# liuQuan98/APR

Measured on AMD Instinct MI355X. Metric: point-cloud pairs/sec (120k-pt KITTI frame, FCGF encode+match+SVD), higher is better.
Workload: dtype f32

## Files before the change

apr_amd/_lib.py:

```python
from __future__ import annotations

import ctypes as C
import os

import torch

_HERE = os.path.dirname(os.path.abspath(__file__))
LIB_PATH = os.path.join(_HERE, "lib", "libapr_hip.so")

_p = C.c_void_p
_i32, _i64, _u64, _f32, _f64, _sz = C.c_int32, C.c_int64, C.c_uint64, C.c_float, C.c_double, C.c_size_t

class PairDesc(C.Structure):
    _fields_ = [("f0", C.c_void_p), ("n0", C.c_int64), ("f1", C.c_void_p), ("n1", C.c_int64),
                ("xyz0", C.c_void_p), ("xyz1", C.c_void_p), ("seed", C.c_uint64)]


class SpconvDesc(C.Structure):
    _fields_ = [("inp", C.c_void_p), ("ldi", C.c_int64), ("nbr", C.c_void_p), ("n_out", C.c_int64),
                ("K", C.c_int32), ("cin", C.c_int32), ("cout", C.c_int32), ("relu", C.c_int32),
                ("w_packed", C.c_void_p), ("scale", C.c_void_p), ("shift", C.c_void_p),
                ("residual", C.c_void_p), ("ldr", C.c_int64), ("out", C.c_void_p), ("ldo", C.c_int64),
                ("counters", C.c_void_p), ("plist", C.c_void_p), ("prod_scratch", C.c_void_p),
                ("plist_bytes", C.c_int64), ("w_bf3", C.c_void_p),
                ("os_pairs", C.c_void_p), ("os_rows", C.c_int64), ("os_build_bytes", C.c_int64),
                ("os_n_in", C.c_int64), ("l2norm", C.c_int32), ("ws3", C.c_int32)]


class ResunetLayer(C.Structure):
    _fields_ = [("K", C.c_int32), ("cin", C.c_int32), ("cout", C.c_int32), ("relu", C.c_int32),
                ("w_packed", C.c_void_p), ("w_bf3", C.c_void_p), ("scale", C.c_void_p), ("shift", C.c_void_p)]


class ResunetPlan(C.Structure):
    _fields_ = [("layer", ResunetLayer * 23), ("conv1_w", C.c_void_p), ("conv1_ks", C.c_int32), ("normalize", C.c_int32),
                ("ws_conv", C.c_uint32), ("ws_block", C.c_uint32), ("os_block", C.c_uint32),
                ("ws3", C.c_int32), ("ws3_cin128", C.c_int32), ("os_min_rows", C.c_int32), ("occ_kernel_map", C.c_int32),
                ("ws3_max_rows_128", C.c_int64)]


class LevelMap(C.Structure):
    _fields_ = [("coords", C.c_void_p), ("keys", C.c_void_p), ("vals", C.c_void_p), ("cap", C.c_int64), ("n", C.c_int64)]


class Pyramid(C.Structure):
    _fields_ = [("lv", LevelMap * 4), ("first", C.c_void_p), ("pts", C.c_void_p), ("header", C.c_void_p),
                ("header_ints", C.c_int32), ("compact", C.c_int32), ("compact_rows", C.c_int64),
                ("counters", C.c_void_p), ("n_counter_slots", C.c_int32)]


class GcnLayer(C.Structure):
    _fields_ = [("kind", C.c_int32), ("k", C.c_int32), ("heads", C.c_int32),
                ("eps1", C.c_float), ("eps2", C.c_float), ("eps3", C.c_float),
                ("w1", C.c_void_p), ("w2", C.c_void_p), ("w3", C.c_void_p), ("b1", C.c_void_p), ("b2", C.c_void_p),
                ("wq", C.c_void_p), ("wk", C.c_void_p), ("wv", C.c_void_p), ("wm", C.c_void_p),
                ("bq", C.c_void_p), ("bk", C.c_void_p), ("bv", C.c_void_p), ("bm", C.c_void_p)]


class GcnDesc(C.Structure):
    _fields_ = [("n_layers", C.c_int32), ("c", C.c_int32), ("layer", GcnLayer * 8)]


PROTOTYPES = {
    "apr_col_sums": (C.c_int, [_p, _i64, _i64, _i32, _p, _p, _sz, _p]),
    "apr_mha_train_forward": (C.c_int, [_p, _p, _p, _i32, _i32, _i32, _i32, _i32, _p, _p, _p]),
    "apr_mha_train_backward": (C.c_int, [_p, _p, _p, _p, _p, _i32, _i32, _i32, _i32, _i32, _p, _p, _p, _p, _p]),
    "apr_edge_features_backward": (C.c_int, [_p, _i32, _i32, _i32, _p, _i64, _p, _p]),
    "apr_gcn_scratch_bytes": (_sz, [_p, _i32, _i32]),
    "apr_gcn_forward": (C.c_int, [_p, _p, _i32, _p, _i32, _p, _i64, _p, _i64, _p, _i64, _p, _i64, _p, _sz, _p]),
    "apr_voxel_pyramid_scratch_bytes": (_sz, [_i64, _i32]),
    "apr_voxel_pyramid": (C.c_int, [_p, _p, _i32, _f32, _p, _sz, _p, _p]),
    "apr_resunet_encode_supported": (C.c_int, [_p, _p, _p]),
    "apr_resunet_encode_scratch_bytes": (_sz, [_p, _p, _p]),
    "apr_resunet_encode": (C.c_int, [_p, _p, _p, _p, _i32, _p, _sz, _p, _i64, _p]),
    "apr_last_error": (C.c_char_p, []),
    "apr_version": (C.c_int, []),
    "apr_device_count": (C.c_int, []),
    "apr_struct_sizes": (_i32, [_p, _i32]),
    "apr_ransac_set_screen": (C.c_int, [_i32]),
    "apr_ransac_set_option": (C.c_int, [_i32, _i32]),
    "apr_ransac_sampling_launches": (C.c_int, [_p]),
    "apr_event_wait": (C.c_int, [_p, _i32]),
    "apr_event_wait_timeout": (C.c_int, [_p, _i32, _i64]),
    "apr_hash_capacity": (_i64, [_i64]),
    "apr_map_scratch_bytes": (_sz, [_i64]),
    "apr_voxelize": (C.c_int, [_p, _i64, _f32, _i32, _p, _p]),
    "apr_map_build": (C.c_int, [_p, _i64, _p, _i32, _p, _p, _i64, _p, _p, _p, _p, _p, _sz, _p]),
    "apr_kernel_map_transpose": (C.c_int, [_p, _i64, _i32, _i64, _p, _p]),
    "apr_voxelize_segments": (C.c_int, [_p, _i64, C.c_float, _p, _i32, _p, _p]),
    "apr_segment_counts": (C.c_int, [_p, _p, _p, _i32, _p, _p]),
    "apr_kernel_map_same": (C.c_int, [_p, _i64, _p, _p, _i64, _i32, _i32, _p, _p]),
    "apr_kernel_map": (C.c_int, [_p, _i64, _p, _p, _p, _i64, _i32, _i32, _p, _p]),
    "apr_spconv_packed_size": (_i64, [_i32, _i32, _i32]),
    "apr_spconv_pack_weights": (C.c_int, [_p, _i32, _i32, _i32, _p, _p]),
    "apr_spconv_fwd": (C.c_int, [_p, _i64, _p, _i64, _i32, _i32, _i32, _p, _p, _p, _p, _i64, _i32, _p, _i64, _p]),
    "apr_pairlist_counter_ints": (_i32, []),
    "apr_pairlist_bytes": (_sz, [_i64, _i32]),
    "apr_pairlist_build": (C.c_int, [_p, _i64, _i32, _p, _p, _sz, _p]),
    "apr_pairlist3_bytes": (_sz, [_i64]),
    "apr_pairlist3_build": (C.c_int, [_p, _i64, _i32, _p, _p, _sz, _p]),
    "apr_spconv_ws3_supported": (C.c_int, [_i32, _i32, _i32]),
    "apr_spconv_ws3_fwd_bf3": (C.c_int, [_p, _i64, _p, _p, _i64, _i32, _i32, _p, _p, _p, _p, _i64, _i32, _p, _i64, _p, _p]),
    "apr_spconv_ws_fwd": (C.c_int, [_p, _i64, _p, _p, _i64, _i32, _i32, _i32, _p, _p, _p, _p, _i64, _i32, _p, _i64, _p, _p]),
    "apr_spconv_packed_bf3_bytes": (_i64, [_i32, _i32, _i32]),
    "apr_spconv_pack_weights_bf3": (C.c_int, [_p, _i32, _i32, _i32, _p, _p]),
    "apr_spconv_pack_weights_bf3_ex": (C.c_int, [_p, _i32, _i32, _i32, _i32, _i32, _p, _p]),
    "apr_spconv_ws_fwd_bf3": (C.c_int, [_p, _i64, _p, _p, _i64, _i32, _i32, _i32, _p, _p, _p, _p, _p, _i64, _i32, _p, _i64,
                                        _p, _p]),
    "apr_spconv_wgrad_scratch_bytes": (_sz, [_i64, _i32, _i32, _i32]),
    "apr_spconv_wgrad": (C.c_int, [_p, _i64, _p, _i64, _p, _i64, _i32, _i32, _i32, _p, _p, _sz, _p]),
    "apr_spconv_wgrad_same_level": (C.c_int, [_p, _i64, _p, _i64, _p, _i64, _i32, _i32, _i32, _p, _p, _sz, _p]),
    "apr_spconv_fwd_batch": (C.c_int, [_p, _i32, _p]),
    "apr_spconv_fwd_batch_timed": (C.c_int, [_p, _i32, _p, _p]),
    "apr_bn_stats": (C.c_int, [_p, _i64, _i64, _i32, _p, _p, _p, _sz, _p]),
    "apr_norm_params": (C.c_int, [_p, _i64, _i64, _i32, _f32, _p, _p, _p, _sz, _p]),
    "apr_bn_stats_scratch_bytes": (_sz, [_i64, _i32]),
    "apr_instance_norm_act": (C.c_int, [_p, _i64, _i64, _i32, _f32, _p, _i64, _i32, _f32, _p, _i64, _p, _sz, _p]),
    "apr_spconv_os_tile_rows": (_i32, [_i64, _i32, _i32]),
    "apr_spconv_os_pairs_bytes": (_sz, [_i64, _i32, _i32]),
    "apr_spconv_os_pairs_build": (C.c_int, [_p, _i64, _i64, _i32, _i32, _p, _sz, _p]),
    "apr_spconv_os_trace": (C.c_int, [_p, _i32]),
    "apr_spconv_os_set_debug": (C.c_int, [_i32]),
    "apr_spconv_os_fwd": (C.c_int, [_p, _i64, _p, _i64, _i32, _i32, _i32, _i32, _p, _p, _p, _p, _i64, _i32, _p, _i64, _p]),
    "apr_norm_backward_scratch_bytes": (_sz, [_i64, _i32]),
    "apr_norm_backward": (C.c_int, [_p, _i64, _p, _i64, _i64, _i32, _p, _p, _p, _p, _i64, _p, _p, _p, _sz, _p]),
    "apr_bn_train_fwd": (C.c_int, [_p, _i64, _i64, _i32, _p, _p, C.c_float, C.c_float, _p, _p, _p, _i64, _i32, _p, _i64, _p, _p,
                                   _p, _p, _i32, _p, _sz, _p]),
    "apr_bn_train_bwd": (C.c_int, [_p, _i64, _p, _i64, _p, _i64, _i64, _i32, _p, _p, _p, _i32, _p, _i64, _p, _i64, _p, _p,
                                   _p, _i32, _p, _sz, _p]),
    "apr_weights_flip_transpose": (C.c_int, [_p, _i32, _i32, _i32, _i32, _p, _p]),
    "apr_dense_gemm_bf3": (C.c_int, [_p, _i64, _i64, _i32, _i32, _p, _p, _p, _p, _i64, _i32, _p, _i64, _p]),
    "apr_dense_rows_bf3_ok": (_i32, [_i32, _i32]),
    "apr_dense_rows_bf3_route": (_i32, [_i64, _i32, _i32]),
    "apr_dense_rows_bf3": (C.c_int, [_p, _i64, _i64, _i32, _i32, _p, _p, _p, _p, _i64, _i32, _i32, _p, _i64, _p]),
    "apr_dense_gemm_bf3_norm_scratch_bytes": (_sz, [_i64, _i32, _i32]),
    "apr_dense_gemm_bf3_norm_act": (C.c_int, [_p, _i64, _i64, _i32, _i32, _p, _f32, _p, _i64, _i32, _f32, _p, _i64, _p, _i32, _p,
                                              _sz, _p]),
    "apr_weighted_choice_round": (C.c_int64, [_p, _i64, _p, _i64, _i64, _p, _i64, _p, _p, _i32]),
    "apr_instance_norm_act_seg": (C.c_int, [_p, _i64, _i64, _i32, _f32, _p, _i64, _i32, _f32, _p, _i64, _p, _i32, _p, _sz, _p]),
    "apr_affine_act": (C.c_int, [_p, _i64, _i64, _i32, _p, _p, _p, _i64, _i32, _f32, _p, _i64, _p]),
    "apr_act_backward": (C.c_int, [_p, _i64, _p, _i64, _i64, _i32, _i32, _f32, _p, _i64, _p]),
    "apr_l2_normalize": (C.c_int, [_p, _i64, _i64, _i32, _p, _i64, _p]),
    "apr_l2_normalize_backward": (C.c_int, [_p, _i64, _p, _i64, _i64, _i32, _p, _i64, _p]),
    "apr_feature_nn": (C.c_int, [_p, _i64, _p, _i64, _i32, _p, _p]),
    "apr_feature_nn_fast_scratch_bytes": (_sz, [_i64, _i64, _i32]),
    "apr_feature_nn_fast": (C.c_int, [_p, _i64, _p, _i64, _i32, _p, _p, _sz, _p]),
    "apr_nn_unpack": (C.c_int, [_p, _i64, _p, _p, _p]),
    "apr_ransac_scratch_bytes": (_sz, [_i64, _i64]),
    "apr_ransac_pose": (C.c_int, [_p, _i64, _p, _i64, _p, _f64, _f64, _i64, _u64, _p, _sz, _p, _p]),
    "apr_ransac_geometric_scratch_bytes": (_sz, [_i64, _i64, _i64]),
    "apr_ransac_pose_geometric": (C.c_int, [_p, _i64, _p, _i64, _p, _f64, _f64, _i64, _i64, _u64, _p, _sz, _p, _p]),
    "apr_ransac_raw_bytes": (_sz, []),
    "apr_ransac_pose_geometric_async": (C.c_int, [_p, _i64, _p, _i64, _p, _f64, _f64, _i64, _i64, _u64, _p, _sz, _p, _p]),
    "apr_ransac_decode": (C.c_int, [_p, _p]),
    "apr_irls_pose": (C.c_int, [_p, _p, _p, _i64, _p, _p, _sz, _p]),
    "apr_match_pose_batch_scratch_bytes": (_sz, [_i32, _i64, _i64, _i32, _i64]),
    "apr_match_pose_batch": (C.c_int, [_p, _i32, _i32, C.c_double, C.c_double, _i64, _p, _sz, _p, _p]),
    "apr_match_pose_batch_slot_bytes": (_sz, [_i32]),
    "apr_match_pose_set_lanes": (C.c_int, [_i32]),
    "apr_match_pose_batch_enqueue": (C.c_int, [_p, _i32, _i32, C.c_double, C.c_double, _i64, _p, _sz, _p, _p]),
    "apr_match_pose_batch_finish": (C.c_int, [_p, _i32, _i32, C.c_double, C.c_double, _i64, _p, _sz, _p, _p, _p]),
    "apr_irls_scratch_bytes": (_sz, [_i64]),
    "apr_valid_pair": (C.c_int, [_p, _i64, _p, _i64, _p, _p, _i64, _i64, _p, _p, _f32, _p, _i64, _i64, _p, _sz, _p]),
    "apr_valid_pair_scratch_bytes": (_sz, [_i64]),
    "apr_contrastive_reduce": (C.c_int, [_p, _p, _i32, _i32, _p, _p, _p, _p, _p, _p, _p, _i32, _i64, _f32, _f32, _p, _p]),
    "apr_grid_subsample_scratch_bytes": (_sz, [_i64]),
    "apr_grid_subsample": (C.c_int, [_p, _i64, _p, _i32, _f32, _p, _i32, _p, _p, _p, _p, _sz, _p]),
    "apr_grid_subsample_async": (C.c_int, [_p, _i64, _p, _i32, _f32, _p, _i32, _p, _p, _p, _p, _sz, _p]),
    "apr_voxel_down_sample_scratch_bytes": (_sz, [_i64]),
    "apr_voxel_down_sample": (C.c_int, [_p, _i64, _p, _i32, _f64, _p, _p, _p, _p, _p, _p, _p, _sz, _p]),
    "apr_sample_augment": (C.c_int, [_p, _p, _i64, _f64, _p, _f64, _p, _p, _p]),
    "apr_cloud_mean": (C.c_int, [_p, _i64, _p, _p]),
    "apr_radius_scratch_bytes": (_sz, [_i64, _i64]),
    "apr_radius_neighbors_async": (C.c_int, [_p, _i64, _p, _i64, _p, _p, _i32, _f32, _i32, _p, _i64, _p, _p, _sz, _p]),
    "apr_radius_neighbors_regrid_async": (C.c_int, [_p, _i64, _p, _i64, _p, _p, _i32, _f32, _i32, _p, _i64, _p, _p, _sz, _p]),
    "apr_radius_neighbors": (C.c_int, [_p, _i64, _p, _i64, _p, _p, _i32, _f32, _i32, _p, _i64, _p, _p, _sz, _p]),
    "apr_knn": (C.c_int, [_p, _i32, _i32, _i32, _p, _p]),
    "apr_row_sums": (C.c_int, [_p, _i64, _i64, _i32, _p, _p]),
    "apr_kpconv_weighted": (C.c_int, [_p, _i64, _p, _i64, _p, _i32, _p, _i64, _i32, _p, _i32, _f32, _p, _p, _i64, _p]),
    "apr_kpconv_dfeat": (C.c_int, [_p, _i64, _p, _i64, _p, _i32, _p, _i64, _i32, _p, _i32, _f32, _p, _p, _i64, _p]),
    "apr_kpconv_dfeat_contrib": (C.c_int, [_p, _i64, _p, _i64, _p, _i32, _p, _i64, _i32, _p, _i32, _f32, _p, _p, _p]),
    "apr_reverse_table_scratch_bytes": (_sz, [_i64, _i32, _i64]),
    "apr_reverse_table_build": (C.c_int, [_p, _i64, _i32, _i64, _p, _p, _p, _sz, _p]),
    "apr_reverse_gather": (C.c_int, [_p, _i32, _p, _p, _i64, _p, _i64, _p]),
    "apr_reverse_gather_range": (C.c_int, [_p, _i32, _p, _p, _i64, _i64, _i64, _i32, _p, _i64, _p]),
    "apr_gather_pool": (C.c_int, [_p, _i64, _i64, _i32, _p, _i32, _i64, _i32, _p, _i64, _p]),
    "apr_gather_pool_argmax": (C.c_int, [_p, _i64, _i64, _i32, _p, _i32, _i64, _p, _i64, _p, _p]),
    "apr_gather_pool_backward": (C.c_int, [_p, _i64, _i32, _p, _p, _i64, _i32, _p, _i32, _p, _i64, _p]),
    "apr_edge_features": (C.c_int, [_p, _i64, _i32, _i32, _p, _i32, _p, _p]),
    "apr_group_max": (C.c_int, [_p, _i64, _i32, _i32, _i32, _p, _p, _f32, _p, _i64, _p]),
    "apr_coords_bbox": (C.c_int, [_p, _i64, _p, _p]),
    "apr_kp_resnet_scratch_bytes": (_sz, [_p]),
    "apr_kp_resnet_block": (C.c_int, [_p, _p]),
    "apr_voxelize_frames": (C.c_int, [_p, _p, _i32, _f32, _p, _p, _p]),
    "apr_gather_frame_points": (C.c_int, [_p, _p, _i32, _p, _p, _i64, _p, _p]),
    "apr_pack_i32": (C.c_int, [_p, _p, _i32, _p, _p, _i64, _p]),
    "apr_fill_bytes": (C.c_int, [_p, _i32, _sz, _p]),
    "apr_kernel_map_transpose_prefilled": (C.c_int, [_p, _i64, _i32, _i64, _p, _p]),
    "apr_occ_conv_scratch_bytes": (_sz, [_p, _i32]),
    "apr_occ_conv_pays": (C.c_int, [_p, _i32, _i64]),
    "apr_occ_conv": (C.c_int, [_p, _i64, _p, _i32, _p, _i32, _p, _p, _p, _i64, _i32, _p, _i64, _p, _sz, _p]),
    "apr_kernel_map_occ": (C.c_int, [_p, _i64, _p, _p, _p, _i64, _i32, _i32, _p, _i32, _p, _p, _p]),
    "apr_mha": (C.c_int, [_p, _p, _p, _i32, _i32, _i32, _i32, _p, _p]),
    "apr_mha_headmajor": (C.c_int, [_p, _p, _p, _i32, _i32, _i32, _i32, _p, _p]),
    "apr_softmax_matvec": (C.c_int, [_p, _p, _p, _i32, _i32, _i32, _f32, _p, _p]),
    "apr_softmax_matvec_bt": (C.c_int, [_p, _p, _p, _i32, _i32, _i32, _f32, _p, _p]),
    "apr_softmax_matvec_mfma": (C.c_int, [_p, _p, _p, _i32, _i32, _i32, _f32, _p, _p]),
    "apr_score_head": (C.c_int, [_p, _i64, _i64, _p, _p]),
    "apr_transform_points": (C.c_int, [_p, _i64, _p, _p, _p]),
    "apr_crop_scratch_bytes": (_sz, [_i64]),
    "apr_crop_to_radius": (C.c_int, [_p, _i64, _p, _i64, _p, _p, _p, _sz, _p]),
    "apr_chamfer_sum": (C.c_int, [_p, _i64, _p, _i64, _p, _p, _sz, _p]),
    "apr_nn3_scratch_bytes": (_sz, [_i64, _i64]),
    "apr_nn3": (C.c_int, [_p, _i64, _p, _i64, C.c_float, _p, _p, _p, _sz, _p]),
    "apr_nn3_batch": (C.c_int, [_p, _p, _p, _p, _i32, C.c_float, _p, _p, _p, _p, _sz, _p]),
    "apr_overlap_labels": (C.c_int, [_p, _i64, _i64, _i64, _p, _p, _p, _p, _p]),
    "apr_weighted_bce_scratch_bytes": (_sz, []),
    "apr_weighted_bce_forward": (C.c_int, [_p, _p, _i64, _p, _p, _p, _sz, _p]),
    "apr_weighted_bce_backward": (C.c_int, [_p, _p, _i64, _p, _p, _p, _p, _p, _p]),
    "apr_gathered_argmax": (C.c_int, [_p, _p, _p, _i64, _p, _p, _p, _i64, _i32, _p, _p, _p]),
    "apr_saliency_labels": (C.c_int, [_p, _p, _p, _p, _p, _p, _p, _p, _p, _p, _i64, _i64, _f32, _p, _p, _p, _p, _p]),
    "apr_circle_select": (C.c_int, [_p, _i64, _p, _i64, _p, _i64, _p, _p, _f32, _p, _p, _p]),
    "apr_circle_gather": (C.c_int, [_p, _p, _p, _p, _i32, _p, _p, _p, _p, _i32, _p, _p, _p, _p, _p, _p, _p, _p, _p]),
    "apr_circle_forward": (C.c_int, [_p, _p, _p, _i32, _p, _p, _p, _i32, _p, _p, _p, _p, _p, _p, _p, _p]),
    "apr_circle_backward": (C.c_int, [_p, _p, _p, _i32, _p, _p, _p, _i32, _p, _p, _p, _p, _p, _p, _p, _p, _p, _p, _p]),
    "apr_circle_scatter": (C.c_int, [_p, _p, _i32, _i32, _p, _i64, _p]),
    "apr_icp_scratch_bytes": (_sz, [_i64, _i64, _i32]),
    "apr_icp_batch": (C.c_int, [_p, _p, _p, _p, _i32, _p, _i32, _p, _f64, _i32, _f64, _f64, _p, _p, _p, _sz, _p]),
    "apr_mutual_select": (C.c_int, [_p, _p, _i64, _p, _p, _i64, _p, _p, _p]),
    "apr_inlier_ratio": (C.c_int, [_p, _i64, _p, _i64, _p, _p, _p, _p, _p, _i64, _f32, _p, _p, _p, _p]),
    "apr_dense_argmax": (C.c_int, [_p, _i64, _i64, _p, _p, _p]),
    "apr_ransac_pairs_geometric_scratch_bytes": (_sz, [_i64, _i64, _i64, _i64, _i64]),
    "apr_ransac_pose_pairs_geometric": (C.c_int, [_p, _i64, _p, _i64, _p, _i64, _f64, _i64, _i64, _u64, _p, _sz, _p, _p]),
    "apr_information_scratch_bytes": (_sz, [_i64, _i64, _i32]),
    "apr_information_batch": (C.c_int, [_p, _p, _p, _p, _i32, _p, _i32, _p, _i64, _f64, _p, _p, _p, _p, _sz, _p]),
    "apr_posegraph_optimize": (C.c_int, [_p, _p, _i32, _p, _p, _i64, _p, _p, _f64, _f64, _f64, _p, _p, _p, _p, _p, _p]),
}

class KpResnetDesc(C.Structure):
    _fields_ = [("x", _p), ("ldx", _i64), ("n_in", _i64),
                ("in_dim", _i32), ("mid", _i32), ("out_dim", _i32), ("strided", _i32),
                ("q_pts", _p), ("s_pts", _p), ("n_out", _i64),
                ("nbr", _p), ("H", _i32), ("n_kp", _i32),
                ("kernel_points", _p), ("extent", _f32), ("eps", _f32), ("slope", _f32), ("nseg", _i32),
                ("w_unary1", _p), ("w_kpconv", _p), ("w_unary2", _p), ("w_shortcut", _p),
                ("seg_in", _p), ("seg_out", _p),
                ("out", _p), ("ldo", _i64),
                ("scratch", _p), ("scratch_bytes", _sz)]


_lib = None


class AprHipError(RuntimeError):
    pass


def load():
    global _lib
    if _lib is not None:
        return _lib
    if not os.path.exists(LIB_PATH):
        raise AprHipError(
            f"{LIB_PATH} is missing: build it with `python -m apr_amd.build` "
            "(hipcc --offload-arch=gfx950). There is no CPU fallback.")
    lib = C.CDLL(LIB_PATH)
    for name, (res, args) in PROTOTYPES.items():
        fn = getattr(lib, name)
        fn.restype = res
        fn.argtypes = args
    _lib = lib
    return lib


def check(rc: int):
    if rc != 0:
        msg = load().apr_last_error().decode()
        raise AprHipError(f"libapr_hip error {rc}: {msg}")


def ptr(t):
    if t is None:
        return None
    return C.c_void_p(t.data_ptr())


def stream():
    return C.c_void_p(torch._C._cuda_getCurrentRawStream(torch.cuda.current_device()))


def require_gpu_tensor(t, dtype, name):
    if not t.is_cuda:
        raise AprHipError(f"{name}: expected a GPU tensor (the HIP path has no CPU fallback)")
    if t.dtype != dtype:
        raise AprHipError(f"{name}: expected dtype {dtype}, got {t.dtype}")
    if not t.is_contiguous():
        raise AprHipError(f"{name}: tensor must be contiguous")
    return t
```

apr_amd/csrc/common.h:

```cpp
#pragma once
#include <hip/hip_runtime.h>
#include <stdint.h>
#include <stdio.h>
#include <stdlib.h>
#include <string.h>

#include "../../include/apr_hip.h"

static inline int env_int(const char* name, int dflt) {
  const char* v = getenv(name);
  return v ? atoi(v) : dflt;
}

#define APR_API extern "C" __attribute__((visibility("default")))

void apr_set_error(const char* fmt, ...);

#define APR_CHECK_ARG(cond, ...)      \
  do {                                \
    if (!(cond)) {                    \
      apr_set_error(__VA_ARGS__);     \
      return APR_EINVAL;              \
    }                                 \
  } while (0)

#define APR_HIP(call)                                                            \
  do {                                                                           \
    hipError_t e_ = (call);                                                      \
    if (e_ != hipSuccess) {                                                      \
      apr_set_error("%s:%d %s -> %s", __FILE__, __LINE__, #call, hipGetErrorString(e_)); \
      return APR_EHIP;                                                           \
    }                                                                            \
  } while (0)

#define APR_LAUNCH_CHECK() APR_HIP(hipGetLastError())

static inline int64_t cdiv64(int64_t a, int64_t b) { return (a + b - 1) / b; }

__host__ __device__ static inline size_t apr_align256(size_t x) { return (x + 255) & ~(size_t)255; }

struct AprArena {
  char* base;
  size_t off = 0;
  explicit AprArena(void* scratch) : base((char*)apr_align256((size_t)scratch)) {}
  template <typename T>
  T* take(size_t count) {
    T* p = base ? (T*)(base + off) : nullptr;
    off += apr_align256(count * sizeof(T));
    return p;
  }
  size_t bytes() const { return off + 256; }
  bool fits(size_t scratch_bytes) const { return scratch_bytes >= bytes(); }
};

int apr_internal_nn_brute(const float* f0, int64_t n0, const float* f1, int64_t n1, int32_t c, uint64_t* best,
                          const unsigned* run_if, void* stream);

int apr_internal_fill(void* ptr, int32_t byte_value, size_t bytes, hipStream_t st);

bool apr_internal_dense_ok(int64_t M, int32_t cin, int32_t cout);
bool apr_internal_dense_rows_route(int64_t M, int32_t cin, int32_t cout);
int apr_internal_dense_gemm(const float* in, int64_t ldi, int64_t M, int32_t cin, int32_t cout, const float* wp,
                            const float* scale, const float* shift, const float* residual, int64_t ldr, int32_t relu,
                            float* out, int64_t ldo, hipStream_t st);

int apr_internal_norm_apply_partials(const float* x, int64_t ldx, int32_t c, const int64_t* seg_row0, const int* seg_blk0,
                                     int32_t nseg, const double* partial, float eps, const float* residual, int64_t ldr,
                                     int32_t act_mode, float negative_slope, float* y, int64_t ldy, hipStream_t st);

#ifdef __HIPCC__
__device__ inline int apr_wave_incl_scan(int x) {
  x += __builtin_amdgcn_update_dpp(0, x, 0x111, 0xf, 0xf, true);
  x += __builtin_amdgcn_update_dpp(0, x, 0x112, 0xf, 0xf, true);
  x += __builtin_amdgcn_update_dpp(0, x, 0x114, 0xf, 0xf, true);
  x += __builtin_amdgcn_update_dpp(0, x, 0x118, 0xf, 0xf, true);
  x += __builtin_amdgcn_update_dpp(0, x, 0x142, 0xa, 0xf, true);
  x += __builtin_amdgcn_update_dpp(0, x, 0x143, 0xc, 0xf, true);
  return x;
}
#endif

#define APR_KEY_EMPTY 0xFFFFFFFFFFFFFFFFull
#define APR_AXIS_BIAS (1 << 17)
#define APR_AXIS_RANGE (1 << 18)

__host__ __device__ static inline bool apr_key_in_range(int b, int x, int y, int z) {
  return (unsigned)b < 1023u && (unsigned)(x + APR_AXIS_BIAS) < (unsigned)APR_AXIS_RANGE &&
         (unsigned)(y + APR_AXIS_BIAS) < (unsigned)APR_AXIS_RANGE &&
         (unsigned)(z + APR_AXIS_BIAS) < (unsigned)APR_AXIS_RANGE;
}

__host__ __device__ static inline uint64_t apr_pack_key(int b, int x, int y, int z) {
  return ((((uint64_t)(unsigned)b << 18 | (uint64_t)(unsigned)(x + APR_AXIS_BIAS)) << 18 |
           (uint64_t)(unsigned)(y + APR_AXIS_BIAS))
          << 18) |
         (uint64_t)(unsigned)(z + APR_AXIS_BIAS);
}

__host__ __device__ static inline uint32_t apr_hash_u64(uint64_t k) {
  k ^= k >> 33;
  k *= 0xff51afd7ed558ccdull;
  k ^= k >> 33;
  k *= 0xc4ceb9fe1a85ec53ull;
  k ^= k >> 33;
  return (uint32_t)k;
}

__host__ __device__ static inline int apr_floor_to(int v, int m) {
  int q = v / m;
  if ((v % m) != 0 && v < 0) --q;
  return q * m;
}

struct AprSearchGrid {
  const unsigned long long* keys;
  const int* vals;
  uint32_t mask;
  const int* start;
  const int* sorted;
  const float* mins;
  float cell;
  const int4* cell_coords;
  const int* n_cells;
  const int* status;
};
#define APR_GRID_MARGIN_CELLS 40960
size_t apr_internal_grid_bytes(int64_t n);
int apr_internal_search_grid(const float* pts, int64_t n, float cell, void* scratch, AprSearchGrid* out,
                             hipStream_t st);
int apr_internal_search_grid_batch(const float* pts, int64_t n, const int32_t* lengths_host, int32_t nb, float cell, void* scratch,
                                   AprSearchGrid* out, hipStream_t st);
struct AprCellBuckets {
  int4* coords;
  const int* starts;
  const float* mins;
  const int4* cell_coords;
  const int* n_cells;
  const int* status;
  const int* start;
  int* sorted;
  int* big_count;
  int* big_list;
  int* spare;
};
int apr_internal_buckets_begin(const float* pts, int64_t n, const int32_t* lengths_host, int32_t nb, void* scratch,
                               AprCellBuckets* out, hipStream_t st);
int apr_internal_buckets_finish(int64_t n, void* scratch, int64_t* first, hipStream_t st);
int apr_internal_icp_pack(const float* tgt, int64_t m, AprSearchGrid g, float4* rows, hipStream_t st);

__device__ static inline int apr_table_lookup(const unsigned long long* __restrict__ keys,
                                              const int* __restrict__ vals, uint32_t mask,
                                              unsigned long long key) {
  uint32_t slot = apr_hash_u64(key) & mask;
  for (uint32_t probe = 0; probe <= mask; ++probe) {
    unsigned long long k = keys[slot];
    if (k == key) return vals[slot];
    if (k == APR_KEY_EMPTY) return -1;
    slot = (slot + 1) & mask;
  }
  return -1;
}
```

apr_amd/csrc/encoder.hip:

```cpp
#include "common.h"

namespace {

constexpr int kLevels = 4, kStages = 7, kMaps = 10, kMaxLists = 24;

inline bool ws_shape_ok(int K, int cin, int cout) { return K <= 27 && cin % 64 == 0 && cin <= 512 && cout % 64 == 0; }

struct ListSlot {
  int map, kind, rows;
  void* blob;
  size_t bytes;
  int32_t* counters;
  bool built;
};

struct Enc {
  const apr_resunet_plan& P;
  const apr_level_map* lv;
  const int32_t* bbox;
  AprArena arena;
  const bool dry;
  hipStream_t st;
  int rc = APR_OK;

  int32_t* kmap[kMaps] = {};
  ListSlot lists[kMaxLists];
  int nlists = 0, ncounter = 0;
  int32_t* counters = nullptr;
  int n_counter_slots = 0;
  void* occ = nullptr;
  size_t occ_bytes = 0;
  int32_t* tpool[3] = {};
  bool tpool_ready = false;
  float* prod = nullptr;
  size_t prod_bytes = 0;

  apr_spconv_desc descs[4];
  int ndesc = 0;

  Enc(const apr_resunet_plan& p, const apr_level_map* l, const int32_t* b, void* scratch, hipStream_t s)
      : P(p), lv(l), bbox(b), arena(scratch), dry(scratch == nullptr), st(s) {}

  float* rows(int64_t n, int c) { return arena.take<float>((size_t)n * c); }
  size_t need() const { return arena.bytes() + apr_align256(prod_bytes); }
  bool ok() const { return rc == APR_OK; }
  void run(int r) {
    if (rc == APR_OK && r != APR_OK) rc = r;
  }

  int64_t map_rows(int m) const { return m < 4 ? lv[m].n : m < 7 ? lv[m - 4 + 1].n : lv[m - 7].n; }
  int64_t map_in_rows(int m) const { return m < 4 ? lv[m].n : m < 7 ? lv[m - 4].n : lv[m - 7 + 1].n; }

  int32_t* kernel_map(int m) {
    if (kmap[m] || (dry && kmap_sized[m])) return kmap[m];
    kmap_sized[m] = true;
    const int64_t n_out = map_rows(m);
    if (m >= 7) {
      const int l = m - 7;
      int32_t* fwd = kernel_map(4 + l);
      if (!tpool_ready) {
        size_t ints = 0;
        for (int a = 0; a < 3; ++a) ints += (size_t)lv[a].n * 27;
        ints = (ints + 63) / 64 * 64 + 64;
        int32_t* buf = arena.take<int32_t>(ints);
        size_t pos = 0;
        for (int a = 0; a < 3; ++a) {
          tpool[a] = dry ? nullptr : buf + pos;
          pos += (size_t)lv[a].n * 27;
        }
        if (!dry) run(apr_fill_bytes(buf, 0xFF, ints * 4, st));
        tpool_ready = true;
      }
      kmap[m] = tpool[l];
      if (!dry) run(apr_kernel_map_transpose_prefilled(fwd, lv[l + 1].n, 27, lv[l].n, kmap[m], st));
      return kmap[m];
    }
    kmap[m] = arena.take<int32_t>((size_t)n_out * 27);
    if (dry) return kmap[m];
    const int lin = m < 4 ? m : m - 4, lout = m < 4 ? m : m - 4 + 1;
    const apr_level_map& in = lv[lin];
    const apr_level_map& outm = lv[lout];
    if (lin == 0 && P.occ_kernel_map && occ)
      run(apr_kernel_map_occ(outm.coords, outm.n, nullptr, in.keys, in.vals, in.cap, 3, 1, bbox, P.conv1_ks, occ, kmap[m], st));
    else
      run(apr_kernel_map(outm.coords, outm.n, nullptr, in.keys, in.vals, in.cap, 3, 1 << lin, kmap[m], st));
    return kmap[m];
  }
  bool kmap_sized[kMaps] = {};

  ListSlot* find_list(int m, int kind, int rws) {
    for (int i = 0; i < nlists; ++i)
      if (lists[i].map == m && lists[i].kind == kind && lists[i].rows == rws) return &lists[i];
    return nullptr;
  }

  ListSlot* ws_list(const apr_resunet_layer& L, int m, bool same_level) {
    bool tri = P.ws3 && L.w_bf3 && apr_spconv_ws3_supported(L.K, L.cin, L.cout);
    if (tri && L.cin == 128 && ((same_level && map_rows(m) > P.ws3_max_rows_128) || !P.ws3_cin128)) tri = false;
    const int kind = tri ? 1 : 0;
    ListSlot* s = find_list(m, kind, 0);
    if (s) return s;
    if (nlists >= kMaxLists) {
      apr_set_error("apr_resunet_encode: more than %d pair lists", kMaxLists);
      run(APR_EINVAL);
      return nullptr;
    }
    s = &lists[nlists++];
    s->map = m;
    s->kind = kind;
    s->rows = 0;
    s->bytes = tri ? apr_pairlist3_bytes(map_rows(m)) : apr_pairlist_bytes(map_rows(m), 27);
    s->blob = arena.take<char>(s->bytes);
    s->built = false;
    s->counters = nullptr;
    if (!dry) {
      if (ncounter >= n_counter_slots) {
        apr_set_error("apr_resunet_encode: more than %d pair lists need a counter block", n_counter_slots);
        run(APR_EINVAL);
        return nullptr;
      }
      s->counters = counters + (size_t)ncounter * apr_pairlist_counter_ints();
    }
    ++ncounter;
    return s;
  }

  ListSlot* os_list(const apr_resunet_layer& L, int m) {
    const int64_t n_out = map_rows(m), n_in = map_in_rows(m);
    const int rws = n_in < (1ll << 23) ? apr_spconv_os_tile_rows(n_out, L.cin, L.cout) : 0;
    if (rws <= 0) return nullptr;
    ListSlot* s = find_list(m, 2, rws);
    if (s) return s;
    if (nlists >= kMaxLists) {
      apr_set_error("apr_resunet_encode: more than %d pair lists", kMaxLists);
      run(APR_EINVAL);
      return nullptr;
    }
    s = &lists[nlists++];
    s->map = m;
    s->kind = 2;
    s->rows = rws;
    s->bytes = apr_spconv_os_pairs_bytes(n_out, 27, rws);
    s->blob = arena.take<char>(s->bytes);
    s->built = false;
    s->counters = nullptr;
    return s;
  }

  float* prod_rows(size_t floats) {
    if (dry) {
      if (floats * 4 > prod_bytes) prod_bytes = floats * 4;
      return nullptr;
    }
    return prod;
  }

  void conv(const apr_resunet_layer& L, const float* in, int64_t ldi, int m, int64_t n_out, ListSlot* list, const float* residual,
            int64_t ldr, float* out, int64_t ldo, bool l2norm) {
    if (!ok()) return;
    int32_t* nbr = m >= 0 ? kernel_map(m) : nullptr;
    apr_spconv_desc d;
    memset(&d, 0, sizeof(d));
    d.in = in; d.ldi = ldi; d.nbr = nbr; d.n_out = n_out;
    d.K = L.K; d.cin = L.cin; d.cout = L.cout; d.relu = L.relu;
    d.w_packed = L.w_packed; d.scale = L.scale; d.shift = L.shift;
    d.residual = residual; d.ldr = residual ? ldr : 0;
    d.out = out; d.ldo = ldo;
    d.l2norm = l2norm ? 1 : 0;
    if (list && list->kind == 2 && L.w_bf3 && m >= 0) {
      d.os_pairs = list->blob; d.os_rows = list->rows; d.os_n_in = map_in_rows(m); d.w_bf3 = L.w_bf3;
      if (!list->built) {
        d.os_build_bytes = (int64_t)list->bytes;
        list->built = true;
      }
    } else if (list && list->kind != 2 && m >= 0 && ws_shape_ok(L.K, L.cin, L.cout)) {
      const bool is3 = list->kind == 1;
      d.prod_scratch = prod_rows((size_t)n_out * (is3 ? 9 : 27) * L.cout);
      d.counters = list->counters; d.plist = list->blob; d.ws3 = is3 ? 1 : 0;
      d.w_bf3 = L.w_bf3;
      if (!list->built) {
        d.plist_bytes = (int64_t)list->bytes;
        list->built = true;
      }
    } else if (m < 0 && L.K == 1 && L.w_bf3 && ((L.cin % 64 == 0 && L.cout % 64 == 0) || apr_dense_rows_bf3_ok(L.cin, L.cout)) &&
               ldi % 4 == 0 && ldo % 4 == 0 &&
               (dry || (((uintptr_t)in | (uintptr_t)out) % 16 == 0 && (!residual || (ldr % 4 == 0 && (uintptr_t)residual % 16 == 0)) &&
                        (!L.scale || (uintptr_t)L.scale % 16 == 0) && (!L.shift || (uintptr_t)L.shift % 16 == 0)))) {
      d.w_bf3 = L.w_bf3;
    }
    if (!dry) descs[ndesc++] = d;
  }
  void flush() {
    if (!dry && ok() && ndesc > 0) run(apr_spconv_fwd_batch(descs, ndesc, st));
    ndesc = 0;
  }

  void walk(float* out, int64_t ldo) {
    const apr_resunet_layer* L = P.layer;
    const int64_t n[4] = {lv[0].n, lv[1].n, lv[2].n, lv[3].n};
    occ_bytes = apr_occ_conv_scratch_bytes(bbox, P.conv1_ks);
    occ = arena.take<char>(occ_bytes + 256);
    if (!counters) {
      n_counter_slots = 16;
      counters = arena.take<int32_t>((size_t)n_counter_slots * apr_pairlist_counter_ints());
      if (!dry) run(apr_fill_bytes(counters, 0, (size_t)n_counter_slots * apr_pairlist_counter_ints() * 4, st));
    }
    if (!dry) prod = (float*)arena.take<char>(prod_bytes_live);

    const int ch1 = L[0].cout, ch2 = L[3].cout, ch3 = L[6].cout, ch4 = L[9].cout;
    const int tr4 = L[12].cout, tr3 = L[15].cout, tr2 = L[18].cout;
    const int w1 = tr2 + ch1, w2 = tr3 + ch2, w3 = tr4 + ch3;
    float* cat1 = rows(n[0], w1);
    float* cat2 = rows(n[1], w2);
    float* cat3 = rows(n[2], w3);
    float* s8 = rows(n[3], ch4);
    int64_t amax = 0;
    {
      const int64_t c[kStages] = {n[0] * ch1, n[1] * ch2, n[2] * ch3, n[3] * ch4, n[2] * tr4, n[1] * tr3, n[0] * tr2};
      for (int s = 0; s < kStages; ++s) amax = c[s] > amax ? c[s] : amax;
    }
    float* A = arena.take<float>((size_t)amax);
    float* H = arena.take<float>((size_t)amax);
    float* h1 = rows(n[0], L[21].cout);

    struct StageIo {
      const float* in; int64_t ldi; int cmap, bmap, lout; float* out; int64_t ldo;
    };
    const StageIo io[kStages] = {
        {nullptr, 0, -1, 0, 0, cat1 + tr2, w1},
        {cat1 + tr2, w1, 4, 1, 1, cat2 + tr3, w2},
        {cat2 + tr3, w2, 5, 2, 2, cat3 + tr4, w3},
        {cat3 + tr4, w3, 6, 3, 3, s8, ch4},
        {s8, ch4, 9, 2, 2, cat3, w3},
        {cat3, w3, 8, 1, 1, cat2, w2},
        {cat2, w2, 7, 0, 0, cat1, w1},
    };
    for (int s = 0; s < kStages && ok(); ++s) {
      const apr_resunet_layer &C = L[3 * s], &B1 = L[3 * s + 1], &B2 = L[3 * s + 2];
      const StageIo& q = io[s];
      const int64_t n_out = n[q.lout];
      if (s == 0) {
        if (!dry)
          run(apr_occ_conv(lv[0].coords, n_out, bbox, P.conv1_ks, P.conv1_w, C.cout, C.scale, C.shift, nullptr, 0, C.relu, A,
                           C.cout, occ, occ_bytes + 256, st));
      } else {
        ListSlot* cl = ((P.ws_conv >> s) & 1u) && ws_shape_ok(C.K, C.cin, C.cout) ? ws_list(C, q.cmap, false) : nullptr;
        conv(C, q.in, q.ldi, q.cmap, n_out, cl, nullptr, 0, A, C.cout, false);
      }
      ListSlot* bl = nullptr;
      if (((P.os_block >> s) & 1u) && B1.cin == 64 && B1.w_bf3 && n_out >= P.os_min_rows) bl = os_list(B1, q.bmap);
      if (!bl && ((P.ws_block >> s) & 1u) && ws_shape_ok(B1.K, B1.cin, B1.cout)) bl = ws_list(B1, q.bmap, true);
      conv(B1, A, B1.cin, q.bmap, n_out, bl, nullptr, 0, H, B1.cout, false);
      conv(B2, H, B2.cin, q.bmap, n_out, bl, A, B1.cin, q.out, q.ldo, false);
      flush();
    }
    conv(L[21], cat1, w1, -1, n[0], nullptr, nullptr, 0, h1, L[21].cout, false);
    conv(L[22], h1, L[21].cout, -1, n[0], nullptr, nullptr, 0, out, ldo, P.normalize != 0);
    flush();
  }
  size_t prod_bytes_live = 0;
};

bool plan_ok(const apr_resunet_plan* p, const apr_level_map* lv, const int32_t* bbox) {
  if (!p || !lv || !bbox || !p->conv1_w) return false;
  for (int l = 0; l < kLevels; ++l)
    if (lv[l].n <= 0 || !lv[l].coords || !lv[l].keys || !lv[l].vals || lv[l].cap <= 0 || (lv[l].cap & (lv[l].cap - 1))) return false;
  for (int i = 0; i < 23; ++i)
    if (!p->layer[i].w_packed || p->layer[i].cin <= 0 || p->layer[i].cout <= 0) return false;
  for (int i = 1; i < 21; ++i)
    if (p->layer[i].K != 27) return false;
  if (p->layer[21].K != 1 || p->layer[22].K != 1) return false;
  const apr_resunet_layer* L = p->layer;
  for (int s = 0; s < kStages; ++s)
    if (L[3 * s + 1].cin != L[3 * s].cout || L[3 * s + 1].cout != L[3 * s].cout || L[3 * s + 2].cin != L[3 * s].cout ||
        L[3 * s + 2].cout != L[3 * s].cout)
      return false;
  if (L[3].cin != L[0].cout || L[6].cin != L[3].cout || L[9].cin != L[6].cout || L[12].cin != L[9].cout ||
      L[15].cin != L[12].cout + L[6].cout || L[18].cin != L[15].cout + L[3].cout || L[21].cin != L[18].cout + L[0].cout ||
      L[22].cin != L[21].cout)
    return false;
  if (L[0].cin != 1 || L[0].K != p->conv1_ks * p->conv1_ks * p->conv1_ks || L[0].cout % 8 != 0) return false;
  if (p->conv1_ks != 3 && p->conv1_ks != 5 && p->conv1_ks != 7) return false;
  return true;
}

}

APR_API int apr_resunet_encode_supported(const apr_resunet_plan* plan, const apr_level_map* lv, const int32_t* bbox_host) {
  if (!plan_ok(plan, lv, bbox_host)) return 0;
  return apr_occ_conv_pays(bbox_host, plan->conv1_ks, lv[0].n) ? 1 : 0;
}

APR_API size_t apr_resunet_encode_scratch_bytes(const apr_resunet_plan* plan, const apr_level_map* lv, const int32_t* bbox_host) {
  if (!apr_resunet_encode_supported(plan, lv, bbox_host)) return 0;
  Enc e(*plan, lv, bbox_host, nullptr, nullptr);
  e.walk(nullptr, plan->layer[22].cout);
  return e.need();
}

APR_API int apr_resunet_encode(const apr_resunet_plan* plan, const apr_level_map* lv, const int32_t* bbox_host, int32_t* counters,
                               int32_t n_counter_slots, void* scratch, size_t scratch_bytes, float* out, int64_t ldo,
                               void* stream) {
  APR_CHECK_ARG(apr_resunet_encode_supported(plan, lv, bbox_host),
                "apr_resunet_encode: plan / maps / box not covered (apr_resunet_encode_supported)");
  APR_CHECK_ARG(scratch && out && ldo >= plan->layer[22].cout && (!counters || n_counter_slots > 0),
                "apr_resunet_encode: bad arguments");
  Enc dry(*plan, lv, bbox_host, nullptr, nullptr);
  dry.walk(nullptr, ldo);
  APR_CHECK_ARG(scratch_bytes >= dry.need(), "apr_resunet_encode: scratch too small");
  Enc e(*plan, lv, bbox_host, scratch, (hipStream_t)stream);
  e.counters = counters;
  e.n_counter_slots = counters ? n_counter_slots : 0;
  e.prod_bytes_live = dry.prod_bytes;
  e.walk(out, ldo);
  return e.rc;
}

namespace {

struct MapBufs {
  uint64_t* keys; int32_t* vals; int64_t cap; int32_t* coords; int64_t* first; int32_t *n_dev, *status; void* scratch;
  size_t scratch_bytes; int64_t rows;
};

MapBufs take_map(AprArena& f, int64_t rows, bool want_first, int32_t* hdr_slot, void* shared_scratch, size_t shared_bytes) {
  MapBufs m;
  m.rows = rows;
  m.cap = apr_hash_capacity(rows);
  m.keys = f.take<uint64_t>((size_t)m.cap);
  m.vals = f.take<int32_t>((size_t)m.cap);
  m.coords = f.take<int32_t>((size_t)rows * 4);
  m.first = want_first ? f.take<int64_t>((size_t)rows) : nullptr;
  m.scratch_bytes = shared_bytes;
  m.scratch = shared_scratch;
  m.n_dev = hdr_slot;
  m.status = hdr_slot ? hdr_slot + 1 : nullptr;
  return m;
}

inline int64_t compact_rows_for(int64_t n_points) { return n_points > 4 * 65536 ? (n_points / 4 > 65536 ? n_points / 4 : 65536) : 0; }

int front_walk(AprArena& f, const float* const* frames, const int64_t* offs, int32_t nseg, float vs, apr_pyramid* out,
               hipStream_t st) {
  const int64_t N = offs ? offs[nseg] : 0;
  const int64_t R = compact_rows_for(N);
  const int hints = 10 + nseg + 8;
  const bool dry = f.base == nullptr;
  int32_t* hdr = f.take<int32_t>((size_t)hints);
  int32_t* counters = f.take<int32_t>((size_t)16 * apr_pairlist_counter_ints());
  int32_t* raw = f.take<int32_t>((size_t)N * 4);
  int64_t* offs_dev = f.take<int64_t>((size_t)(nseg + 1));
  float* pts = f.take<float>((size_t)N * 3);
  const size_t sbytes = apr_map_scratch_bytes(N);
  void* const sc = f.take<char>(sbytes);
  MapBufs dedup = take_map(f, N, true, dry ? nullptr : hdr + (R ? 8 : 0), sc, sbytes);
  MapBufs lvl[4];
  if (R) lvl[0] = take_map(f, R, false, dry ? nullptr : hdr, sc, sbytes);
  else lvl[0] = dedup;
  const int64_t rows = R ? R : N;
  for (int l = 1; l < 4; ++l) lvl[l] = take_map(f, rows, false, dry ? nullptr : hdr + 2 * l, sc, sbytes);
  if (dry) return APR_OK;

  int rc;
  const size_t clear = (size_t)((char*)counters - (char*)hdr) + (size_t)16 * apr_pairlist_counter_ints() * 4;
  if ((rc = apr_pack_i32(nullptr, nullptr, 0, nullptr, hdr, (int64_t)(clear / 4), st)) != APR_OK) return rc;
  if ((rc = apr_voxelize_frames(frames, offs, nseg, vs, raw, offs_dev, st)) != APR_OK) return rc;
  if ((rc = apr_map_build(raw, N, nullptr, 0, dedup.keys, dedup.vals, dedup.cap, dedup.coords, dedup.first, dedup.n_dev,
                          dedup.status, dedup.scratch, dedup.scratch_bytes, st)) != APR_OK)
    return rc;
  if ((rc = apr_segment_counts(dedup.first, dedup.n_dev, offs_dev, nseg, hdr + 10, st)) != APR_OK) return rc;
  if ((rc = apr_coords_bbox(raw, N, hdr + 10 + nseg, st)) != APR_OK) return rc;
  if ((rc = apr_gather_frame_points(frames, offs, nseg, dedup.first, dedup.n_dev, N, pts, st)) != APR_OK) return rc;
  if (R &&
      (rc = apr_map_build(dedup.coords, R, dedup.n_dev, 0, lvl[0].keys, lvl[0].vals, lvl[0].cap, lvl[0].coords, nullptr,
                          lvl[0].n_dev, lvl[0].status, lvl[0].scratch, lvl[0].scratch_bytes, st)) != APR_OK)
    return rc;
  for (int l = 1; l < 4; ++l)
    if ((rc = apr_map_build(lvl[l - 1].coords, rows, lvl[l - 1].n_dev, 1 << l, lvl[l].keys, lvl[l].vals, lvl[l].cap, lvl[l].coords,
                            nullptr, lvl[l].n_dev, lvl[l].status, lvl[l].scratch, lvl[l].scratch_bytes, st)) != APR_OK)
      return rc;
  for (int l = 0; l < 4; ++l) {
    out->lv[l].coords = lvl[l].coords; out->lv[l].keys = lvl[l].keys; out->lv[l].vals = lvl[l].vals;
    out->lv[l].cap = lvl[l].cap; out->lv[l].n = lvl[l].rows;
  }
  out->first = dedup.first;
  out->pts = pts;
  out->header = hdr;
  out->header_ints = hints;
  out->compact = R ? 1 : 0;
  out->compact_rows = R;
  out->counters = counters;
  out->n_counter_slots = 16;
  return APR_OK;
}

}

APR_API size_t apr_voxel_pyramid_scratch_bytes(int64_t n_points, int32_t nseg) {
  if (n_points <= 0 || nseg <= 0 || nseg > APR_MAX_FRAMES) return 0;
  AprArena f(nullptr);
  int64_t offs[APR_MAX_FRAMES + 1] = {};
  offs[nseg] = n_points;
  (void)front_walk(f, nullptr, offs, nseg, 1.f, nullptr, nullptr);
  return f.bytes();
}

APR_API int apr_voxel_pyramid(const float* const* frames_host, const int64_t* offsets_host, int32_t nseg, float voxel_size,
                              void* arena, size_t arena_bytes, apr_pyramid* out, void* stream) {
  APR_CHECK_ARG(frames_host && offsets_host && nseg >= 1 && nseg <= APR_MAX_FRAMES && arena && out && voxel_size > 0.f,
                "apr_voxel_pyramid: bad arguments (1 .. %d frames)", APR_MAX_FRAMES);
  APR_CHECK_ARG(offsets_host[0] == 0 && offsets_host[nseg] > 0, "apr_voxel_pyramid: offsets must run 0 .. total points > 0");
  APR_CHECK_ARG(arena_bytes >= apr_voxel_pyramid_scratch_bytes(offsets_host[nseg], nseg), "apr_voxel_pyramid: arena too small");
  AprArena f(arena);
  return front_walk(f, frames_host, offsets_host, nseg, voxel_size, out, (hipStream_t)stream);
}
```

apr_amd/csrc/hash.hip:

```cpp
#include "common.h"

namespace {

constexpr int kBlock = 256;

__global__ void k_voxelize(const float* __restrict__ xyz, int64_t n, float vs, int batch,
                           int4* __restrict__ coords) {
  int64_t i = (int64_t)blockIdx.x * blockDim.x + threadIdx.x;
  if (i >= n) return;
  float x = xyz[3 * i + 0] / vs, y = xyz[3 * i + 1] / vs, z = xyz[3 * i + 2] / vs;
  coords[i] = make_int4(batch, (int)floorf(x), (int)floorf(y), (int)floorf(z));
}

__global__ void k_voxelize_segments(const float* __restrict__ xyz, int64_t n, float vs,
                                    const long long* __restrict__ offsets, int nseg, int4* __restrict__ coords) {
  int64_t i = (int64_t)blockIdx.x * blockDim.x + threadIdx.x;
  if (i >= n) return;
  int b = 0;
  while (b + 1 < nseg && i >= offsets[b + 1]) ++b;
  float x = xyz[3 * i + 0] / vs, y = xyz[3 * i + 1] / vs, z = xyz[3 * i + 2] / vs;
  coords[i] = make_int4(b, (int)floorf(x), (int)floorf(y), (int)floorf(z));
}

__device__ inline int4 load_coord(const int4* coords, int64_t i, int floor_to) {
  int4 c = coords[i];
  if (floor_to > 0) {
    c.y = apr_floor_to(c.y, floor_to);
    c.z = apr_floor_to(c.z, floor_to);
    c.w = apr_floor_to(c.w, floor_to);
  }
  return c;
}

__global__ void k_insert(const int4* __restrict__ coords, int64_t n, const int* __restrict__ n_dev,
                         int floor_to, unsigned long long* __restrict__ keys, int* __restrict__ vals,
                         uint32_t mask, int* __restrict__ slot_of, int* __restrict__ status) {
  const int64_t i = (int64_t)blockIdx.x * blockDim.x + threadIdx.x;
  const int lane = threadIdx.x & 63;
  if (n_dev) n = min((long long)n, (long long)*n_dev);
  const bool live = i < n;
  unsigned long long key = APR_KEY_EMPTY;
  bool ok = false;
  if (live) {
    const int4 c = load_coord(coords, i, floor_to);
    ok = apr_key_in_range(c.x, c.y, c.z, c.w);
    if (ok) key = apr_pack_key(c.x, c.y, c.z, c.w);
    else *status = 1;
  }
  const unsigned long long prev = __shfl_up(key, 1);
  const bool head = lane == 0 || key != prev || !ok;
  const unsigned long long heads = __ballot(head);
  const int leader = 63 - __clzll((long long)(heads & ((2ull << lane) - 1ull)));
  int slot = -1;
  if (head && ok) {
    uint32_t sl = apr_hash_u64(key) & mask;
    for (uint32_t probe = 0; probe <= mask; ++probe) {
      unsigned long long p = keys[sl];
      if (p != key) {
        if (p != APR_KEY_EMPTY) {
          sl = (sl + 1) & mask;
          continue;
        }
        p = atomicCAS(&keys[sl], APR_KEY_EMPTY, key);
        if (p != APR_KEY_EMPTY && p != key) {
          sl = (sl + 1) & mask;
          continue;
        }
      }
      atomicMin(&vals[sl], (int)i);
      slot = (int)sl;
      break;
    }
    if (slot < 0) *status = 2;
  }
  slot = __shfl(slot, leader);
  if (live) slot_of[i] = ok ? slot : -1;
}

__global__ void k_flag_count(const int* __restrict__ vals, const int* __restrict__ slot_of,
                             int64_t n, const int* __restrict__ n_dev, uint8_t* __restrict__ flags,
                             int* __restrict__ block_counts) {
  __shared__ int wave_cnt[kBlock / 64];
  int64_t i = (int64_t)blockIdx.x * blockDim.x + threadIdx.x;
  if (n_dev) n = min((long long)n, (long long)*n_dev);
  bool f = false;
  if (i < n) {
    int s = slot_of[i];
    f = (s >= 0) && (vals[s] == (int)i);
    flags[i] = f;
  }
  unsigned long long b = __ballot(f);
  if ((threadIdx.x & 63) == 0) wave_cnt[threadIdx.x >> 6] = __popcll(b);
  __syncthreads();
  if (threadIdx.x == 0) {
    int s = 0;
    for (int w = 0; w < kBlock / 64; ++w) s += wave_cnt[w];
    block_counts[blockIdx.x] = s;
  }
}

__global__ void k_scan_blocks(const int* __restrict__ counts, int nblk, int* __restrict__ offsets,
                              int* __restrict__ n_out) {
  __shared__ int wave_sum[16];
  __shared__ int carry_s;
  if (threadIdx.x == 0) carry_s = 0;
  __syncthreads();
  const int lane = threadIdx.x & 63, wave = threadIdx.x >> 6;
  for (int base = 0; base < nblk; base += blockDim.x) {
    int idx = base + threadIdx.x;
    int v = idx < nblk ? counts[idx] : 0;
    int incl = v;
    for (int d = 1; d < 64; d <<= 1) {
      int t = __shfl_up(incl, d);
      if (lane >= d) incl += t;
    }
    if (lane == 63) wave_sum[wave] = incl;
    __syncthreads();
    int woff = 0;
    for (int w = 0; w < wave; ++w) woff += wave_sum[w];
    int carry = carry_s;
    if (idx < nblk) offsets[idx] = carry + woff + incl - v;
    __syncthreads();
    if (threadIdx.x == blockDim.x - 1) carry_s = carry + woff + incl;
    __syncthreads();
  }
  if (threadIdx.x == 0) *n_out = carry_s;
}

__global__ void k_compact(const int4* __restrict__ coords, int64_t n, const int* __restrict__ n_dev,
                          int floor_to, const uint8_t* __restrict__ flags,
                          const int* __restrict__ block_offsets, const int* __restrict__ slot_of,
                          int* __restrict__ vals, int4* __restrict__ out_coords,
                          long long* __restrict__ out_first) {
  __shared__ int wave_cnt[kBlock / 64];
  int64_t i = (int64_t)blockIdx.x * blockDim.x + threadIdx.x;
  if (n_dev) n = min((long long)n, (long long)*n_dev);
  bool f = (i < n) && flags[i];
  unsigned long long b = __ballot(f);
  const int lane = threadIdx.x & 63, wave = threadIdx.x >> 6;
  if (lane == 0) wave_cnt[wave] = __popcll(b);
  __syncthreads();
  if (!f) return;
  int pos = block_offsets[blockIdx.x] + __popcll(b & ((1ull << lane) - 1ull));
  for (int w = 0; w < wave; ++w) pos += wave_cnt[w];
  out_coords[pos] = load_coord(coords, i, floor_to);
  if (out_first) out_first[pos] = (long long)i;
  vals[slot_of[i]] = pos;
}

__device__ inline int table_lookup(const unsigned long long* __restrict__ keys,
                                   const int* __restrict__ vals, uint32_t mask,
                                   unsigned long long key) {
  uint32_t slot = apr_hash_u64(key) & mask;
  for (uint32_t probe = 0; probe <= mask; ++probe) {
    unsigned long long k = keys[slot];
    if (k == key) return vals[slot];
    if (k == APR_KEY_EMPTY) return -1;
    slot = (slot + 1) & mask;
  }
  return -1;
}

__global__ void k_table_init(unsigned long long* __restrict__ keys, int* __restrict__ vals, int64_t cap,
                             int* __restrict__ status, int* __restrict__ n_out) {
  const int64_t i = (int64_t)blockIdx.x * blockDim.x + threadIdx.x;
  if (i < cap) {
    keys[i] = ~0ull;
    vals[i] = 0x7F7F7F7F;
  }
  if (i == 0) {
    *status = 0;
    if (n_out) *n_out = 0;
  }
}

__global__ void k_segment_counts(const long long* __restrict__ first, const int* __restrict__ n_dev,
                                 const long long* __restrict__ offsets, int nseg, int* __restrict__ counts) {
  const int b = blockIdx.x * blockDim.x + threadIdx.x;
  if (b >= nseg) return;
  const int n = *n_dev;
  auto lower = [&](long long v) {
    int lo = 0, hi = n;
    while (lo < hi) {
      const int mid = (lo + hi) >> 1;
      if (first[mid] < v) lo = mid + 1; else hi = mid;
    }
    return lo;
  };
  counts[b] = lower(offsets[b + 1]) - lower(offsets[b]);
}

__global__ void k_kernel_map(const int4* __restrict__ out_coords, int64_t n_out,
                             const int* __restrict__ n_out_dev,
                             const unsigned long long* __restrict__ keys,
                             const int* __restrict__ vals, uint32_t mask, int ks, int scale,
                             int* __restrict__ nbr) {
  const int K = ks * ks * ks, h = ks / 2;
  int64_t total = n_out * K;
  if (n_out_dev) total = (int64_t)min((long long)n_out, (long long)*n_out_dev) * K;
  for (int64_t t = (int64_t)blockIdx.x * blockDim.x + threadIdx.x; t < total;
       t += (int64_t)gridDim.x * blockDim.x) {
    int64_t j = t / K;
    int o = (int)(t - j * K);
    int ox = o % ks - h, oy = (o / ks) % ks - h, oz = o / (ks * ks) - h;
    int4 c = out_coords[j];
    int x = c.y + ox * scale, y = c.z + oy * scale, z = c.w + oz * scale;
    int r = -1;
    if (apr_key_in_range(c.x, x, y, z)) r = table_lookup(keys, vals, mask, apr_pack_key(c.x, x, y, z));
    nbr[t] = r;
  }
}

__global__ void k_kernel_map_sym(const int4* __restrict__ coords, int64_t n, const unsigned long long* __restrict__ keys,
                                 const int* __restrict__ vals, uint32_t mask, int ks, int scale,
                                 int* __restrict__ nbr) {
  const int K = ks * ks * ks, h = ks / 2, half = K / 2;
  const int64_t total = n * (half + 1);
  for (int64_t t = (int64_t)blockIdx.x * blockDim.x + threadIdx.x; t < total;
       t += (int64_t)gridDim.x * blockDim.x) {
    const int64_t j = t / (half + 1);
    const int o = (int)(t - j * (half + 1));
    if (o == half) {
      nbr[j * K + o] = (int)j;
      continue;
    }
    const int ox = o % ks - h, oy = (o / ks) % ks - h, oz = o / (ks * ks) - h;
    const int4 c = coords[j];
    const int x = c.y + ox * scale, y = c.z + oy * scale, z = c.w + oz * scale;
    int r = -1;
    if (apr_key_in_range(c.x, x, y, z)) r = table_lookup(keys, vals, mask, apr_pack_key(c.x, x, y, z));
    nbr[j * K + o] = r;
    if (r >= 0) nbr[(int64_t)r * K + (K - 1 - o)] = (int)j;
  }
}

__global__ void k_fill_upper(int* __restrict__ nbr, int64_t n, int K, int half) {
  const int64_t total = n * half;
  for (int64_t t = (int64_t)blockIdx.x * blockDim.x + threadIdx.x; t < total; t += (int64_t)gridDim.x * blockDim.x) {
    const int64_t j = t / half;
    nbr[j * K + half + 1 + (int)(t - j * half)] = -1;
  }
}

__global__ void k_map_transpose(const int* __restrict__ nbr, int64_t total, int K, int* __restrict__ nbr_t) {
  const int64_t t = (int64_t)blockIdx.x * blockDim.x + threadIdx.x;
  if (t >= total) return;
  const int i = nbr[t];
  if (i >= 0) nbr_t[(int64_t)i * K + (int)(t % K)] = (int)(t / K);
}

constexpr int kMaxFrames = APR_MAX_FRAMES;
struct FrameTable {
  const float* ptr[kMaxFrames];
  long long off[kMaxFrames + 1];
  int nseg;
};

__device__ inline int frame_of(const FrameTable& ft, long long i) {
  int b = 0;
  while (b + 1 < ft.nseg && i >= ft.off[b + 1]) ++b;
  return b;
}

__global__ void k_voxelize_frames(FrameTable ft, int64_t n, float vs, int4* __restrict__ coords,
                                  long long* __restrict__ offsets_out) {
  int64_t i = (int64_t)blockIdx.x * blockDim.x + threadIdx.x;
  if (blockIdx.x == 0 && threadIdx.x <= ft.nseg && offsets_out) offsets_out[threadIdx.x] = ft.off[threadIdx.x];
  if (i >= n) return;
  const int b = frame_of(ft, i);
  const float* p = ft.ptr[b] + 3 * (i - ft.off[b]);
  float x = p[0] / vs, y = p[1] / vs, z = p[2] / vs;
  coords[i] = make_int4(b, (int)floorf(x), (int)floorf(y), (int)floorf(z));
}

__global__ void k_gather_frame_points(FrameTable ft, const long long* __restrict__ first, const int* __restrict__ n_dev,
                                      float* __restrict__ pts) {
  const int64_t r = (int64_t)blockIdx.x * blockDim.x + threadIdx.x;
  if (r >= *n_dev) return;
  const long long i = first[r];
  const int b = frame_of(ft, i);
  const float* p = ft.ptr[b] + 3 * (i - ft.off[b]);
  pts[3 * r + 0] = p[0];
  pts[3 * r + 1] = p[1];
  pts[3 * r + 2] = p[2];
}

constexpr int kMaxPack = APR_MAX_PACK;
struct PackTable {
  const int* src[kMaxPack];
  int begin[kMaxPack + 1];
  int nsrc;
};
__global__ void k_pack_i32(PackTable pt, int* __restrict__ dst, int* __restrict__ zero_ptr, long long zero_words) {
  for (int s = 0; s < pt.nsrc; ++s) {
    const int n = pt.begin[s + 1] - pt.begin[s];
    for (int e = blockIdx.x * blockDim.x + threadIdx.x; e < n; e += gridDim.x * blockDim.x) dst[pt.begin[s] + e] = pt.src[s][e];
  }
  for (long long e = (long long)blockIdx.x * blockDim.x + threadIdx.x; e < zero_words; e += (long long)gridDim.x * blockDim.x)
    zero_ptr[e] = 0;
}

}

APR_API int64_t apr_hash_capacity(int64_t n) {
  int64_t cap = 1024;
  while (cap < 2 * n) cap <<= 1;
  return cap;
}

namespace {
struct MapScratch {
  int* slot_of;
  uint8_t* flags;
  int *blk_cnt, *blk_off;
};
MapScratch walk_map(AprArena& a, int64_t n) {
  const size_t nblk = (size_t)cdiv64(n > 0 ? n : 1, kBlock);
  MapScratch m;
  m.slot_of = a.take<int>(n);
  m.flags = a.take<uint8_t>(n);
  m.blk_cnt = a.take<int>(nblk);
  m.blk_off = a.take<int>(nblk);
  return m;
}
}

APR_API size_t apr_map_scratch_bytes(int64_t n) {
  AprArena a(nullptr);
  walk_map(a, n);
  return a.bytes();
}

APR_API int apr_voxelize(const float* xyz, int64_t n, float voxel_size, int32_t batch,
                         int32_t* coords, void* stream) {
  APR_CHECK_ARG(n >= 0 && voxel_size > 0.f, "apr_voxelize: bad n=%lld or voxel_size", (long long)n);
  APR_CHECK_ARG(batch >= 0 && batch < 1023, "apr_voxelize: batch index %d outside [0,1023)", batch);
  if (n == 0) return APR_OK;
  hipLaunchKernelGGL(k_voxelize, dim3((unsigned)cdiv64(n, kBlock)), dim3(kBlock), 0, (hipStream_t)stream,
                     xyz, n, voxel_size, batch, (int4*)coords);
  APR_LAUNCH_CHECK();
  return APR_OK;
}

APR_API int apr_map_build(const int32_t* coords_in, int64_t n, const int32_t* n_dev, int32_t floor_to,
                          uint64_t* keys,
                          int32_t* vals, int64_t cap, int32_t* out_coords, int64_t* out_first,
                          int32_t* n_out, int32_t* status, void* scratch, size_t scratch_bytes,
                          void* stream) {
  hipStream_t st = (hipStream_t)stream;
  APR_CHECK_ARG(n >= 0 && n < (1ll << 31), "apr_map_build: n=%lld out of range", (long long)n);
  APR_CHECK_ARG(cap >= 2 * n && (cap & (cap - 1)) == 0, "apr_map_build: cap=%lld must be a power of two >= 2n",
                (long long)cap);
  AprArena arena(scratch);
  const MapScratch m = walk_map(arena, n);
  APR_CHECK_ARG(arena.fits(scratch_bytes), "apr_map_build: scratch too small");
  APR_CHECK_ARG(floor_to >= 0, "apr_map_build: floor_to < 0");
  hipLaunchKernelGGL(k_table_init, dim3((unsigned)cdiv64(cap, 256)), dim3(256), 0, st, (unsigned long long*)keys, vals,
                     cap, status, n == 0 ? n_out : (int*)nullptr);
  if (n == 0) {
    APR_LAUNCH_CHECK();
    return APR_OK;
  }
  const int nblk = (int)cdiv64(n, kBlock);
  const uint32_t mask = (uint32_t)(cap - 1);
  hipLaunchKernelGGL(k_insert, dim3(nblk), dim3(kBlock), 0, st, (const int4*)coords_in, n, n_dev,
                     floor_to, (unsigned long long*)keys, vals, mask, m.slot_of, status);
  hipLaunchKernelGGL(k_flag_count, dim3(nblk), dim3(kBlock), 0, st, vals, m.slot_of, n, n_dev, m.flags, m.blk_cnt);
  hipLaunchKernelGGL(k_scan_blocks, dim3(1), dim3(1024), 0, st, m.blk_cnt, nblk, m.blk_off, n_out);
  hipLaunchKernelGGL(k_compact, dim3(nblk), dim3(kBlock), 0, st, (const int4*)coords_in, n, n_dev, floor_to,
                     m.flags, m.blk_off, m.slot_of, vals, (int4*)out_coords, (long long*)out_first);
  APR_LAUNCH_CHECK();
  return APR_OK;
}

static int map_transpose(const int32_t* nbr, int64_t n_out, int32_t K, int64_t n_in, int32_t* nbr_t, bool prefilled,
                         void* stream) {
  APR_CHECK_ARG(n_out >= 0 && n_in >= 0 && K >= 1 && (nbr || n_out == 0) && (nbr_t || n_in == 0),
                "apr_kernel_map_transpose: bad arguments");
  hipStream_t st = (hipStream_t)stream;
  if (n_in > 0 && !prefilled) {
    if (int rcf = apr_internal_fill(nbr_t, 0xFF, (size_t)n_in * K * 4, st)) return rcf;
  }
  if (n_out > 0)
    hipLaunchKernelGGL(k_map_transpose, dim3((unsigned)cdiv64(n_out * K, kBlock)), dim3(kBlock), 0, st, nbr,
                       n_out * (int64_t)K, K, nbr_t);
  APR_LAUNCH_CHECK();
  return APR_OK;
}

APR_API int apr_kernel_map_transpose(const int32_t* nbr, int64_t n_out, int32_t K, int64_t n_in, int32_t* nbr_t,
                                     void* stream) {
  return map_transpose(nbr, n_out, K, n_in, nbr_t, false, stream);
}

APR_API int apr_kernel_map_transpose_prefilled(const int32_t* nbr, int64_t n_out, int32_t K, int64_t n_in, int32_t* nbr_t,
                                               void* stream) {
  return map_transpose(nbr, n_out, K, n_in, nbr_t, true, stream);
}

static __global__ __launch_bounds__(256) void k_fill_bytes(unsigned char* __restrict__ p, unsigned v32, unsigned long long head,
                                              unsigned long long n16, unsigned long long tail) {
  uint4* const q = (uint4*)(p + head);
  const uint4 v = make_uint4(v32, v32, v32, v32);
  for (unsigned long long i = (unsigned long long)blockIdx.x * blockDim.x + threadIdx.x; i < n16;
       i += (unsigned long long)gridDim.x * blockDim.x)
    q[i] = v;
  if (blockIdx.x == 0) {
    if (threadIdx.x < head) p[threadIdx.x] = (unsigned char)v32;
    if (threadIdx.x < tail) p[head + n16 * 16 + threadIdx.x] = (unsigned char)v32;
  }
}

int apr_internal_fill(void* ptr, int32_t byte_value, size_t bytes, hipStream_t st) {
  static const int s_kernel = env_int("APR_FILL_KERNEL", 1);
  if (bytes == 0) return APR_OK;
  if (!s_kernel) {
    APR_HIP(hipMemsetAsync(ptr, byte_value, bytes, st));
    return APR_OK;
  }
  const unsigned b = (unsigned)byte_value & 0xFFu;
  const unsigned v32 = b * 0x01010101u;
  size_t head = (16 - ((uintptr_t)ptr & 15)) & 15;
  if (head > bytes) head = bytes;
  const size_t n16 = (bytes - head) / 16, tail = bytes - head - n16 * 16;
  int64_t nblk = cdiv64((int64_t)n16, 256 * 8);
  nblk = nblk < 1 ? 1 : (nblk > 2048 ? 2048 : nblk);
  hipLaunchKernelGGL(k_fill_bytes, dim3((unsigned)nblk), dim3(256), 0, st, (unsigned char*)ptr, v32, (unsigned long long)head,
                     (unsigned long long)n16, (unsigned long long)tail);
  APR_LAUNCH_CHECK();
  return APR_OK;
}

APR_API int apr_fill_bytes(void* ptr, int32_t byte_value, size_t bytes, void* stream) {
  APR_CHECK_ARG(ptr || bytes == 0, "apr_fill_bytes: null pointer");
  return apr_internal_fill(ptr, byte_value, bytes, (hipStream_t)stream);
}

APR_API int apr_voxelize_segments(const float* xyz, int64_t n, float voxel_size, const int64_t* offsets, int32_t nseg,
                                  int32_t* coords, void* stream) {
  APR_CHECK_ARG(n >= 0 && voxel_size > 0.f && nseg >= 1 && nseg <= 1023 && offsets, "apr_voxelize_segments: bad arguments");
  if (n == 0) return APR_OK;
  hipLaunchKernelGGL(k_voxelize_segments, dim3((unsigned)cdiv64(n, kBlock)), dim3(kBlock), 0, (hipStream_t)stream, xyz, n,
                     voxel_size, (const long long*)offsets, nseg, (int4*)coords);
  APR_LAUNCH_CHECK();
  return APR_OK;
}


static int fill_frame_table(FrameTable& ft, const float* const* frames, const int64_t* offsets, int32_t nseg) {
  APR_CHECK_ARG(frames && offsets && nseg >= 1 && nseg <= kMaxFrames, "frame table: 1 <= frames <= %d", kMaxFrames);
  APR_CHECK_ARG(offsets[0] == 0, "frame table: offsets[0] must be 0");
  for (int b = 0; b < nseg; ++b) {
    APR_CHECK_ARG(offsets[b + 1] >= offsets[b] && (frames[b] || offsets[b + 1] == offsets[b]), "frame table: bad frame %d", b);
    ft.ptr[b] = frames[b];
    ft.off[b] = offsets[b];
  }
  ft.off[nseg] = offsets[nseg];
  ft.nseg = nseg;
  return APR_OK;
}

APR_API int apr_voxelize_frames(const float* const* frames_host, const int64_t* offsets_host, int32_t nseg, float voxel_size,
                                int32_t* coords, int64_t* offsets_dev, void* stream) {
  FrameTable ft;
  if (int rc = fill_frame_table(ft, frames_host, offsets_host, nseg)) return rc;
  APR_CHECK_ARG(voxel_size > 0.f && coords, "apr_voxelize_frames: bad arguments");
  const int64_t n = offsets_host[nseg];
  hipLaunchKernelGGL(k_voxelize_frames, dim3((unsigned)(n > 0 ? cdiv64(n, kBlock) : 1)), dim3(kBlock), 0, (hipStream_t)stream, ft,
                     n, voxel_size, (int4*)coords, (long long*)offsets_dev);
  APR_LAUNCH_CHECK();
  return APR_OK;
}

APR_API int apr_gather_frame_points(const float* const* frames_host, const int64_t* offsets_host, int32_t nseg,
                                    const int64_t* first, const int32_t* n_dev, int64_t n_max, float* pts, void* stream) {
  FrameTable ft;
  if (int rc = fill_frame_table(ft, frames_host, offsets_host, nseg)) return rc;
  APR_CHECK_ARG(first && n_dev && pts && n_max >= 0, "apr_gather_frame_points: bad arguments");
  if (n_max == 0) return APR_OK;
  hipLaunchKernelGGL(k_gather_frame_points, dim3((unsigned)cdiv64(n_max, kBlock)), dim3(kBlock), 0, (hipStream_t)stream, ft,
                     (const long long*)first, n_dev, pts);
  APR_LAUNCH_CHECK();
  return APR_OK;
}

APR_API int apr_pack_i32(const int32_t* const* srcs_host, const int32_t* counts_host, int32_t nsrc, int32_t* dst,
                         int32_t* zero_ptr, int64_t zero_words, void* stream) {
  APR_CHECK_ARG(nsrc >= 0 && nsrc <= kMaxPack && (nsrc == 0 || (srcs_host && counts_host && dst)) && zero_words >= 0 &&
                    (zero_words == 0 || zero_ptr),
                "apr_pack_i32: bad arguments (at most %d sources)", kMaxPack);
  PackTable pt;
  pt.nsrc = nsrc;
  pt.begin[0] = 0;
  int64_t words = 0;
  for (int s = 0; s < nsrc; ++s) {
    APR_CHECK_ARG(counts_host[s] >= 0 && (srcs_host[s] || counts_host[s] == 0), "apr_pack_i32: bad source %d", s);
    pt.src[s] = srcs_host[s];
    words += counts_host[s];
    APR_CHECK_ARG(words < (1 << 30), "apr_pack_i32: too many words");
    pt.begin[s + 1] = (int)words;
  }
  if (nsrc == 0 && zero_words == 0) return APR_OK;
  int64_t nblk = cdiv64(zero_words > words ? zero_words : words, 256 * 8);
  nblk = nblk < 1 ? 1 : (nblk > 64 ? 64 : nblk);
  hipLaunchKernelGGL(k_pack_i32, dim3((unsigned)nblk), dim3(256), 0, (hipStream_t)stream, pt, dst, zero_ptr, (long long)zero_words);
  APR_LAUNCH_CHECK();
  return APR_OK;
}

APR_API int apr_segment_counts(const int64_t* first, const int32_t* n_dev, const int64_t* offsets, int32_t nseg,
                               int32_t* counts, void* stream) {
  APR_CHECK_ARG(nseg >= 0 && first && n_dev && offsets && counts, "apr_segment_counts: bad arguments");
  if (nseg == 0) return APR_OK;
  hipLaunchKernelGGL(k_segment_counts, dim3((unsigned)cdiv64(nseg, 64)), dim3(64), 0, (hipStream_t)stream,
                     (const long long*)first, n_dev, (const long long*)offsets, nseg, counts);
  APR_LAUNCH_CHECK();
  return APR_OK;
}

APR_API int apr_kernel_map_same(const int32_t* coords, int64_t n, const uint64_t* keys, const int32_t* vals, int64_t cap,
                                int32_t kernel_size, int32_t scale, int32_t* nbr, void* stream) {
  APR_CHECK_ARG(kernel_size >= 3 && (kernel_size & 1) && kernel_size <= 7,
                "apr_kernel_map_same: kernel_size=%d must be odd, 3 ... 7", kernel_size);
  APR_CHECK_ARG((cap & (cap - 1)) == 0 && cap > 0, "apr_kernel_map_same: cap must be a power of two");
  APR_CHECK_ARG(n >= 0 && n < (1ll << 31), "apr_kernel_map_same: bad n");
  if (n == 0) return APR_OK;
  hipStream_t st = (hipStream_t)stream;
  const int K = kernel_size * kernel_size * kernel_size, half = K / 2;
  int64_t fblk = cdiv64(n * half, kBlock);
  if (fblk > 16384) fblk = 16384;
  hipLaunchKernelGGL(k_fill_upper, dim3((unsigned)fblk), dim3(kBlock), 0, st, nbr, n, K, half);
  int64_t nblk = cdiv64(n * (half + 1), kBlock);
  if (nblk > 65536) nblk = 65536;
  hipLaunchKernelGGL(k_kernel_map_sym, dim3((unsigned)nblk), dim3(kBlock), 0, st, (const int4*)coords, n,
                     (const unsigned long long*)keys, vals, (uint32_t)(cap - 1), kernel_size, scale, nbr);
  APR_LAUNCH_CHECK();
  return APR_OK;
}

APR_API int apr_kernel_map(const int32_t* out_coords, int64_t n_out, const int32_t* n_out_dev,
                           const uint64_t* in_keys, const int32_t* in_vals, int64_t cap,
                           int32_t kernel_size, int32_t scale, int32_t* nbr, void* stream) {
  APR_CHECK_ARG(kernel_size >= 1 && (kernel_size & 1) && kernel_size <= 7,
                "apr_kernel_map: kernel_size=%d must be odd and <= 7", kernel_size);
  APR_CHECK_ARG((cap & (cap - 1)) == 0 && cap > 0, "apr_kernel_map: cap must be a power of two");
  APR_CHECK_ARG(n_out >= 0, "apr_kernel_map: n_out < 0");
  if (n_out == 0) return APR_OK;
  const int K = kernel_size * kernel_size * kernel_size;
  int64_t total = n_out * K;
  int64_t nblk = cdiv64(total, kBlock);
  if (nblk > 65536) nblk = 65536;
  hipLaunchKernelGGL(k_kernel_map, dim3((unsigned)nblk), dim3(kBlock), 0, (hipStream_t)stream,
                     (const int4*)out_coords, n_out, n_out_dev, (const unsigned long long*)in_keys, in_vals,
                     (uint32_t)(cap - 1), kernel_size, scale, nbr);
  APR_LAUNCH_CHECK();
  return APR_OK;
}
```

apr_amd/csrc/occ.hip:

```cpp
#include <climits>

#include "common.h"

namespace {

struct OccGrid {
  int minx, miny, minz;
  int dy, dz, wx;
  int nx, nb;
};

__device__ inline bool occ_inside(const OccGrid& g, const int4& c, int h) {
  const int x = c.y - g.minx, y = c.z - g.miny, z = c.w - g.minz;
  return c.x >= 0 && c.x < g.nb && x >= h && x < g.nx - h && y >= h && y < g.dy - h && z >= h && z < g.dz - h;
}

__device__ inline int64_t occ_word(const OccGrid& g, int b, int x, int y, int z) {
  return (((int64_t)b * g.dz + (z - g.minz)) * g.dy + (y - g.miny)) * g.wx + ((x - g.minx) >> 5);
}

__global__ void k_bbox_init(int* __restrict__ bbox) {
  if (threadIdx.x < 3) bbox[threadIdx.x] = INT_MAX;
  else if (threadIdx.x < 7) bbox[threadIdx.x] = INT_MIN;
  else if (threadIdx.x == 7) bbox[7] = 0;
}

constexpr int kBboxThreads = 1024, kBboxBlocks = 128;
__global__ __launch_bounds__(kBboxThreads) void k_bbox(const int4* __restrict__ coords, int64_t n, int* __restrict__ bbox) {
  __shared__ int s_red[kBboxThreads / 64][8];
  int lo[3] = {INT_MAX, INT_MAX, INT_MAX}, hi[4] = {INT_MIN, INT_MIN, INT_MIN, INT_MIN};
  for (int64_t i = (int64_t)blockIdx.x * blockDim.x + threadIdx.x; i < n; i += (int64_t)gridDim.x * blockDim.x) {
    const int4 c = coords[i];
    lo[0] = min(lo[0], c.y); lo[1] = min(lo[1], c.z); lo[2] = min(lo[2], c.w);
    hi[0] = max(hi[0], c.y); hi[1] = max(hi[1], c.z); hi[2] = max(hi[2], c.w); hi[3] = max(hi[3], c.x);
  }
#pragma unroll
  for (int d = 32; d >= 1; d >>= 1) {
#pragma unroll
    for (int a = 0; a < 3; ++a) lo[a] = min(lo[a], __shfl_xor(lo[a], d));
#pragma unroll
    for (int a = 0; a < 4; ++a) hi[a] = max(hi[a], __shfl_xor(hi[a], d));
  }
  const int wave = threadIdx.x >> 6;
  if ((threadIdx.x & 63) == 0) {
#pragma unroll
    for (int a = 0; a < 3; ++a) s_red[wave][a] = lo[a];
#pragma unroll
    for (int a = 0; a < 4; ++a) s_red[wave][3 + a] = hi[a];
  }
  __syncthreads();
  if (threadIdx.x < 7) {
    const int a = threadIdx.x;
    int v = s_red[0][a];
    for (int w = 1; w < kBboxThreads / 64; ++w) v = a < 3 ? min(v, s_red[w][a]) : max(v, s_red[w][a]);
    if (a < 3) atomicMin(&bbox[a], v);
    else atomicMax(&bbox[a], v);
  }
}

__global__ void k_occ_set(const int4* __restrict__ coords, int n, OccGrid g, int h, unsigned* __restrict__ bm) {
  const int i = blockIdx.x * blockDim.x + threadIdx.x;
  if (i >= n) return;
  const int4 c = coords[i];
  if (!occ_inside(g, c, h)) return;
  atomicOr(&bm[occ_word(g, c.x, c.y, c.z, c.w)], 1u << ((c.y - g.minx) & 31));
}

template <int KS>
__global__ __launch_bounds__(256) void k_occ_conv(const int4* __restrict__ coords, int n, OccGrid g,
                                                  const unsigned* __restrict__ bm, const float* __restrict__ w,
                                                  int cout, const float* __restrict__ scale,
                                                  const float* __restrict__ shift, const float* __restrict__ residual,
                                                  int64_t ldr, int relu, float* __restrict__ out, int64_t ldo) {
  constexpr int H = KS / 2, K = KS * KS * KS, MW = (K + 31) / 32;
  __shared__ unsigned s_mask[64][MW + 1];
  const int tid = threadIdx.x;
  const int r = tid >> 2, cg = tid & 3;
  const int row = blockIdx.x * 64 + r;
  for (int t = tid; t < 64 * (MW + 1); t += 256) (&s_mask[0][0])[t] = 0u;
  __syncthreads();
  bool inside = false;
  if (row < n) {
    const int4 c = coords[row];
    inside = occ_inside(g, c, H);
  }
  if (inside) {
    const int4 c = coords[row];
    const int x0 = c.y - H - g.minx;
    const int sh = x0 & 31;
    const unsigned* base = bm + occ_word(g, c.x, c.y - H, c.z, c.w);
    for (int p = cg; p < KS * KS; p += 4) {
      const int oy = p % KS - H, oz = p / KS - H;
      const unsigned* q = base + ((int64_t)oz * g.dy + oy) * g.wx;
      const unsigned long long win = (unsigned long long)q[0] | ((unsigned long long)q[1] << 32);
      const unsigned bits = (unsigned)(win >> sh) & ((1u << KS) - 1u);
      if (bits) {
        const int k0 = KS * p;
        atomicOr(&s_mask[r][k0 >> 5], bits << (k0 & 31));
        if ((k0 & 31) + KS > 32) atomicOr(&s_mask[r][(k0 >> 5) + 1], bits >> (32 - (k0 & 31)));
      }
    }
  }
  __syncthreads();
  if (row >= n) return;
  if (!inside) {
    for (int c = cg; c < cout; c += 4) out[(int64_t)row * ldo + c] = __int_as_float(0x7fc00000);
    return;
  }
  typedef float f32x4 __attribute__((ext_vector_type(4)));
  for (int c0 = cg * 8; c0 < cout; c0 += 32) {
    float acc[8] = {0.f, 0.f, 0.f, 0.f, 0.f, 0.f, 0.f, 0.f};
#pragma unroll
    for (int mw = 0; mw < MW; ++mw) {
      unsigned m = s_mask[r][mw];
      while (m) {
        const int k = mw * 32 + __ffs((int)m) - 1;
        m &= m - 1;
        const f32x4 w0 = *reinterpret_cast<const f32x4*>(w + (int64_t)k * cout + c0);
        const f32x4 w1 = *reinterpret_cast<const f32x4*>(w + (int64_t)k * cout + c0 + 4);
        acc[0] += w0[0]; acc[1] += w0[1]; acc[2] += w0[2]; acc[3] += w0[3];
        acc[4] += w1[0]; acc[5] += w1[1]; acc[6] += w1[2]; acc[7] += w1[3];
      }
    }
#pragma unroll
    for (int i = 0; i < 8; ++i) {
      const int c = c0 + i;
      float v = acc[i] * (scale ? scale[c] : 1.f) + (shift ? shift[c] : 0.f);
      if (residual) v += residual[(int64_t)row * ldr + c];
      if (relu) v = fmaxf(v, 0.f);
      out[(int64_t)row * ldo + c] = v;
    }
  }
}

struct OccLayout {
  OccGrid g;
  int64_t words;
  bool ok;
};

OccLayout occ_layout(const int32_t* bbox, int32_t ks) {
  OccLayout L;
  L.ok = false;
  L.words = 0;
  const int h = ks / 2;
  for (int a = 0; a < 3; ++a)
    if (bbox[3 + a] < bbox[a]) return L;
  if (bbox[6] < 0) return L;
  const int64_t dx = (int64_t)bbox[3] - bbox[0] + 1 + 2 * h, dy = (int64_t)bbox[4] - bbox[1] + 1 + 2 * h,
                dz = (int64_t)bbox[5] - bbox[2] + 1 + 2 * h;
  const int64_t wx = (dx + 31) / 32 + 1;
  const int64_t words = ((int64_t)bbox[6] + 1) * dz * dy * wx;
  if (dx > (1 << 24) || dy > (1 << 24) || dz > (1 << 24) || words > (1ll << 29)) return L;
  L.g.minx = bbox[0] - h;
  L.g.miny = bbox[1] - h;
  L.g.minz = bbox[2] - h;
  L.g.dy = (int)dy;
  L.g.dz = (int)dz;
  L.g.wx = (int)wx;
  L.g.nx = (int)dx;
  L.g.nb = bbox[6] + 1;
  L.words = words;
  L.ok = true;
  return L;
}

__global__ void k_kernel_map_occ(const int4* __restrict__ out_coords, int64_t n_out, const int* __restrict__ n_out_dev,
                                 const unsigned long long* __restrict__ keys, const int* __restrict__ vals, uint32_t mask,
                                 int ks, int scale, OccGrid g, int pad, const unsigned* __restrict__ bm, int* __restrict__ nbr) {
  const int K = ks * ks * ks, h = ks / 2;
  int64_t total = n_out * K;
  if (n_out_dev) total = (int64_t)min((long long)n_out, (long long)*n_out_dev) * K;
  for (int64_t t = (int64_t)blockIdx.x * blockDim.x + threadIdx.x; t < total; t += (int64_t)gridDim.x * blockDim.x) {
    const int64_t j = t / K;
    const int o = (int)(t - j * K);
    const int ox = o % ks - h, oy = (o / ks) % ks - h, oz = o / (ks * ks) - h;
    const int4 c = out_coords[j];
    const int x = c.y + ox * scale, y = c.z + oy * scale, z = c.w + oz * scale;
    int r = -1;
    if (apr_key_in_range(c.x, x, y, z)) {
      const int4 cell = make_int4(c.x, x, y, z);
      const bool maybe = !occ_inside(g, cell, pad) || ((bm[occ_word(g, c.x, x, y, z)] >> ((x - g.minx) & 31)) & 1u);
      if (maybe) r = apr_table_lookup(keys, vals, mask, apr_pack_key(c.x, x, y, z));
    }
    nbr[t] = r;
  }
}

}

APR_API int apr_kernel_map_occ(const int32_t* out_coords, int64_t n_out, const int32_t* n_out_dev, const uint64_t* in_keys,
                               const int32_t* in_vals, int64_t cap, int32_t kernel_size, int32_t scale,
                               const int32_t* bbox_host, int32_t bitmap_kernel_size, const void* occ_scratch, int32_t* nbr,
                               void* stream) {
  APR_CHECK_ARG(kernel_size >= 1 && (kernel_size & 1) && kernel_size <= 7, "apr_kernel_map_occ: kernel_size=%d must be odd and <= 7",
                kernel_size);
  APR_CHECK_ARG((cap & (cap - 1)) == 0 && cap > 0 && n_out >= 0 && bbox_host && occ_scratch && nbr,
                "apr_kernel_map_occ: bad arguments");
  if (n_out == 0) return APR_OK;
  const OccLayout L = occ_layout(bbox_host, bitmap_kernel_size);
  APR_CHECK_ARG(L.ok, "apr_kernel_map_occ: empty or oversized bounding box");
  const unsigned* bm = (const unsigned*)(((uintptr_t)occ_scratch + 255) & ~(uintptr_t)255);
  const int K = kernel_size * kernel_size * kernel_size;
  int64_t nblk = cdiv64(n_out * K, 256);
  if (nblk > 65536) nblk = 65536;
  hipLaunchKernelGGL(k_kernel_map_occ, dim3((unsigned)nblk), dim3(256), 0, (hipStream_t)stream, (const int4*)out_coords, n_out,
                     n_out_dev, (const unsigned long long*)in_keys, in_vals, (uint32_t)(cap - 1), kernel_size, scale, L.g,
                     bitmap_kernel_size / 2, bm, nbr);
  APR_LAUNCH_CHECK();
  return APR_OK;
}

APR_API int apr_coords_bbox(const int32_t* coords, int64_t n, int32_t* bbox_dev, void* stream) {
  APR_CHECK_ARG(n >= 0 && bbox_dev && (n == 0 || coords), "apr_coords_bbox: bad arguments");
  hipStream_t st = (hipStream_t)stream;
  hipLaunchKernelGGL(k_bbox_init, dim3(1), dim3(64), 0, st, bbox_dev);
  if (n > 0) {
    int64_t nblk = cdiv64(n, kBboxThreads * 4);
    if (nblk > kBboxBlocks) nblk = kBboxBlocks;
    hipLaunchKernelGGL(k_bbox, dim3((unsigned)nblk), dim3(kBboxThreads), 0, st, (const int4*)coords, n, bbox_dev);
  }
  APR_LAUNCH_CHECK();
  return APR_OK;
}

APR_API size_t apr_occ_conv_scratch_bytes(const int32_t* bbox_host, int32_t kernel_size) {
  if (!bbox_host || kernel_size < 1 || !(kernel_size & 1)) return 0;
  const OccLayout L = occ_layout(bbox_host, kernel_size);
  return L.ok ? (size_t)L.words * 4 + 256 : 0;
}

APR_API int apr_occ_conv_pays(const int32_t* bbox_host, int32_t kernel_size, int64_t n) {
  const size_t b = apr_occ_conv_scratch_bytes(bbox_host, kernel_size);
  return b > 0 && n > 0 && b <= (size_t)n * 1024 + ((size_t)4 << 20);
}

APR_API int apr_occ_conv(const int32_t* coords, int64_t n, const int32_t* bbox_host, int32_t kernel_size,
                         const float* w, int32_t cout, const float* scale, const float* shift, const float* residual,
                         int64_t ldr, int32_t relu, float* out, int64_t ldo, void* scratch, size_t scratch_bytes,
                         void* stream) {
  APR_CHECK_ARG(n >= 0 && n < (1ll << 31) && bbox_host && w && out && scratch, "apr_occ_conv: bad arguments");
  APR_CHECK_ARG(kernel_size == 3 || kernel_size == 5 || kernel_size == 7, "apr_occ_conv: kernel_size %d, supported: 3, 5, 7",
                kernel_size);
  APR_CHECK_ARG(cout > 0 && cout % 8 == 0 && ldo >= cout && (!residual || ldr >= cout), "apr_occ_conv: cout %% 8 != 0 or short rows");
  APR_CHECK_ARG((((uintptr_t)w) & 15) == 0, "apr_occ_conv: weights must be 16-byte aligned");
  if (n == 0) return APR_OK;
  const OccLayout L = occ_layout(bbox_host, kernel_size);
  APR_CHECK_ARG(L.ok, "apr_occ_conv: empty or oversized bounding box");
  APR_CHECK_ARG(scratch_bytes >= (size_t)L.words * 4 + 256, "apr_occ_conv: scratch too small");
  hipStream_t st = (hipStream_t)stream;
  unsigned* bm = (unsigned*)(((uintptr_t)scratch + 255) & ~(uintptr_t)255);
  if (int rcf = apr_internal_fill(bm, 0, (size_t)L.words * 4, st)) return rcf;
  hipLaunchKernelGGL(k_occ_set, dim3((unsigned)cdiv64(n, 256)), dim3(256), 0, st, (const int4*)coords, (int)n, L.g,
                     kernel_size / 2, bm);
  const dim3 grid((unsigned)cdiv64(n, 64));
  if (kernel_size == 3)
    hipLaunchKernelGGL(k_occ_conv<3>, grid, dim3(256), 0, st, (const int4*)coords, (int)n, L.g, bm, w, cout, scale, shift,
                       residual, ldr, relu, out, ldo);
  else if (kernel_size == 5)
    hipLaunchKernelGGL(k_occ_conv<5>, grid, dim3(256), 0, st, (const int4*)coords, (int)n, L.g, bm, w, cout, scale, shift,
                       residual, ldr, relu, out, ldo);
  else
    hipLaunchKernelGGL(k_occ_conv<7>, grid, dim3(256), 0, st, (const int4*)coords, (int)n, L.g, bm, w, cout, scale, shift,
                       residual, ldr, relu, out, ldo);
  APR_LAUNCH_CHECK();
  return APR_OK;
}
```

apr_amd/ops.py:

```python
from __future__ import annotations

import ctypes as C
import os

import numpy as np
import torch

from . import _lib
from ._lib import check, ptr, stream


def _lib_():
    return _lib.load()


def _f32(t, name):
    if not t.is_cuda or t.dtype != torch.float32:
        raise _lib.AprHipError(f"{name}: need a float32 GPU tensor (no CPU fallback), got {t.dtype} on {t.device}")
    return t


def _rows(t, name):
    _f32(t, name)
    if t.dim() != 2 or (t.shape[1] > 1 and t.stride(1) != 1):
# ... 1017 lines not shown
    @staticmethod
    def backward(ctx, dy):
        (x,) = ctx.saved_tensors
        dy = dy.contiguous()
        n, c = x.shape
        dx = torch.empty_like(x)
        check(_lib_().apr_l2_normalize_backward(ptr(x), c, ptr(dy), c, n, c, ptr(dx), c, stream()))
        return dx



def feature_nn(f0, f1, return_distance=False, impl=None):
    f0 = _f32(f0, "feature_nn.f0").contiguous()
    f1 = _f32(f1, "feature_nn.f1").contiguous()
    if f0.shape[1] != f1.shape[1]:
        raise _lib.AprHipError("feature_nn: channel mismatch")
    n0, c = f0.shape
    n1 = f1.shape[0]
    lib = _lib_()
    best = torch.empty(n0, dtype=torch.int64, device=f0.device)
    if impl is None:
        impl = os.environ.get("APR_NN_IMPL", "fast")
    if impl not in ("brute", "fast"):
        raise _lib.AprHipError(f"feature_nn: unknown impl {impl!r}")
    if impl == "fast" and c in (32, 64, 128):
        sb = int(lib.apr_feature_nn_fast_scratch_bytes(n0, n1, c))
        scratch = torch.empty(sb, dtype=torch.uint8, device=f0.device)
        check(lib.apr_feature_nn_fast(ptr(f0), n0, ptr(f1), n1, c, ptr(best), ptr(scratch), sb, stream()))
    else:
        check(lib.apr_feature_nn(ptr(f0), n0, ptr(f1), n1, c, ptr(best), stream()))
    idx = torch.empty(n0, dtype=torch.int64, device=f0.device)
    d2 = torch.empty(n0, dtype=torch.float32, device=f0.device) if return_distance else None
    check(lib.apr_nn_unpack(ptr(best), n0, ptr(idx), ptr(d2), stream()))
    return (idx, d2) if return_distance else idx



def _dev(t, dtype, name):
    if not torch.is_tensor(t) or not t.is_cuda or t.dtype != dtype:
        raise _lib.AprHipError(f"{name}: need a {dtype} GPU tensor (no CPU fallback), got "
                               f"{getattr(t, 'dtype', type(t))} on {getattr(t, 'device', 'the host')}")
    return t.contiguous()


def overlap_labels(correspondence, n_src, n_tgt):
    corr = _dev(correspondence, torch.int64, "overlap_labels.correspondence")
    dev = corr.device
    gt = torch.empty(n_src + n_tgt, dtype=torch.float32, device=dev)
    src_idx = torch.empty(n_src, dtype=torch.int32, device=dev)
    tgt_idx = torch.empty(n_tgt, dtype=torch.int32, device=dev)
    counts = torch.empty(3, dtype=torch.int32, device=dev)
    check(_lib_().apr_overlap_labels(ptr(corr), corr.shape[0], n_src, n_tgt, ptr(gt), ptr(src_idx), ptr(tgt_idx), ptr(counts),
                                     stream()))
    return gt, src_idx, tgt_idx, counts


def weighted_bce(pred, gt, n_dev=None):
    pred, gt = _dev(pred, torch.float32, "weighted_bce.pred"), _dev(gt, torch.float32, "weighted_bce.gt")
    if pred.dim() != 1 or pred.shape != gt.shape:
        raise _lib.AprHipError("weighted_bce: prediction and gt must be vectors of one length")
    lib = _lib_()
    sb = int(lib.apr_weighted_bce_scratch_bytes())
    scratch = torch.empty(sb, dtype=torch.uint8, device=pred.device)
    out = torch.empty(8, dtype=torch.float32, device=pred.device)
    check(lib.apr_weighted_bce_forward(ptr(pred), ptr(gt), pred.shape[0], ptr(n_dev), ptr(out), ptr(scratch), sb, stream()))
    return out


def weighted_bce_backward(pred, gt, out8, grad_out, n_dev=None, scatter_pos=None, dpred=None):
    pred, gt = _dev(pred, torch.float32, "weighted_bce_backward.pred"), _dev(gt, torch.float32, "weighted_bce_backward.gt")
    out8, grad_out = _dev(out8, torch.float32, "weighted_bce_backward.out8"), _dev(grad_out, torch.float32, "weighted_bce_backward.grad_out")
    if dpred is None:
        dpred = torch.zeros_like(pred)
    check(_lib_().apr_weighted_bce_backward(ptr(pred), ptr(gt), pred.shape[0], ptr(n_dev), ptr(out8), ptr(grad_out),
                                            ptr(scatter_pos), ptr(dpred), stream()))
    return dpred


def gathered_argmax(a, a_idx, na_dev, b, b_idx, nb_dev):
    a, b = _dev(a, torch.float32, "gathered_argmax.a"), _dev(b, torch.float32, "gathered_argmax.b")
    a_idx, b_idx = _dev(a_idx, torch.int32, "gathered_argmax.a_idx"), _dev(b_idx, torch.int32, "gathered_argmax.b_idx")
    if a.dim() != 2 or b.dim() != 2 or a.shape[1] != b.shape[1]:
        raise _lib.AprHipError("gathered_argmax: channel mismatch")
    row_arg = torch.zeros(a_idx.shape[0], dtype=torch.int32, device=a.device)
    col_arg = torch.zeros(b_idx.shape[0], dtype=torch.int32, device=a.device)
    check(_lib_().apr_gathered_argmax(ptr(a), ptr(a_idx), ptr(na_dev), a_idx.shape[0], ptr(b), ptr(b_idx), ptr(nb_dev),
                                      b_idx.shape[0], a.shape[1], ptr(row_arg), ptr(col_arg), stream()))
    return row_arg, col_arg


def saliency_labels(src_pcd, tgt_pcd, rot, trans, src_idx, tgt_idx, counts, row_arg, col_arg, scores_saliency, radius):
    src_pcd, tgt_pcd = _dev(src_pcd, torch.float32, "saliency_labels.src_pcd"), _dev(tgt_pcd, torch.float32, "saliency_labels.tgt_pcd")
    rot, trans = _dev(rot, torch.float32, "saliency_labels.rot"), _dev(trans, torch.float32, "saliency_labels.trans")
    scores_saliency = _dev(scores_saliency, torch.float32, "saliency_labels.scores_saliency")
    for name, t in (("src_idx", src_idx), ("tgt_idx", tgt_idx), ("counts", counts), ("row_arg", row_arg), ("col_arg", col_arg)):
        _dev(t, torch.int32, "saliency_labels." + name)
    n_src, n_tgt = src_pcd.shape[0], tgt_pcd.shape[0]
    if scores_saliency.shape[0] != n_src + n_tgt or src_idx.shape[0] != n_src or tgt_idx.shape[0] != n_tgt:
        raise _lib.AprHipError("saliency_labels: vector lengths do not match the clouds")
    dev = src_pcd.device
    labels = torch.zeros(n_src + n_tgt, dtype=torch.float32, device=dev)
    sel = torch.full((n_src + n_tgt,), 0.5, dtype=torch.float32, device=dev)
    pos = torch.zeros(n_src + n_tgt, dtype=torch.int32, device=dev)
    dist = torch.zeros(n_src + n_tgt, dtype=torch.float32, device=dev)
    check(_lib_().apr_saliency_labels(ptr(src_pcd), ptr(tgt_pcd), ptr(rot), ptr(trans), ptr(src_idx), ptr(tgt_idx),
                                      ptr(counts), ptr(row_arg), ptr(col_arg), ptr(scores_saliency), n_src, n_tgt,
                                      float(radius), ptr(labels), ptr(sel), ptr(pos), ptr(dist), stream()))
    return labels, sel, pos, dist


def circle_select(correspondence, src_pcd, tgt_pcd, rot, trans, thresh):
    corr = _dev(correspondence, torch.int64, "circle_select.correspondence")
    src_pcd, tgt_pcd = _dev(src_pcd, torch.float32, "circle_select.src_pcd"), _dev(tgt_pcd, torch.float32, "circle_select.tgt_pcd")
    rot, trans = _dev(rot, torch.float32, "circle_select.rot"), _dev(trans, torch.float32, "circle_select.trans")
    filt = torch.empty(max(int(corr.shape[0]), 1), dtype=torch.int32, device=corr.device)
    count = torch.empty(1, dtype=torch.int32, device=corr.device)
    check(_lib_().apr_circle_select(ptr(corr), corr.shape[0], ptr(src_pcd), src_pcd.shape[0], ptr(tgt_pcd), tgt_pcd.shape[0],
                                    ptr(rot), ptr(trans), float(thresh), ptr(filt), ptr(count), stream()))
    return filt, count


def circle_gather(correspondence, filt, count, choice, src_pcd, tgt_pcd, src_feats, tgt_feats, rot, trans):
    correspondence, choice = _dev(correspondence, torch.int64, "circle_gather.correspondence"), _dev(choice, torch.int64, "circle_gather.choice")
    filt, count = _dev(filt, torch.int32, "circle_gather.filt"), _dev(count, torch.int32, "circle_gather.count")
    src_pcd, tgt_pcd = _dev(src_pcd, torch.float32, "circle_gather.src_pcd"), _dev(tgt_pcd, torch.float32, "circle_gather.tgt_pcd")
    src_feats, tgt_feats = _dev(src_feats, torch.float32, "circle_gather.src_feats"), _dev(tgt_feats, torch.float32, "circle_gather.tgt_feats")
    rot, trans = _dev(rot, torch.float32, "circle_gather.rot"), _dev(trans, torch.float32, "circle_gather.trans")
    P, D, dev = int(choice.shape[0]), int(src_feats.shape[1]), src_feats.device
    g = {"a_row": torch.empty(P, dtype=torch.int32, device=dev), "b_row": torch.empty(P, dtype=torch.int32, device=dev),
         "a_pts": torch.empty((P, 3), dtype=torch.float32, device=dev), "b_pts": torch.empty((P, 3), dtype=torch.float32, device=dev),
         "a_feats": torch.empty((P, D), dtype=torch.float32, device=dev),
         "b_feats": torch.empty((P, D), dtype=torch.float32, device=dev)}
    check(_lib_().apr_circle_gather(ptr(correspondence), ptr(filt), ptr(count), ptr(choice), P, ptr(src_pcd), ptr(tgt_pcd),
                                    ptr(src_feats), ptr(tgt_feats), D, ptr(rot), ptr(trans), ptr(g["a_row"]), ptr(g["b_row"]),
                                    ptr(g["a_pts"]), ptr(g["b_pts"]), ptr(g["a_feats"]), ptr(g["b_feats"]), stream()))
    return g


def _circle_params(params):
    return (C.c_float * 7)(*[float(v) for v in params])


def circle_forward(params, anchors=None, coords_dist=None, feats_dist=None):
    g = anchors or {}
    for name, t in list(g.items()) + [("coords_dist", coords_dist), ("feats_dist", feats_dist)]:
        if t is not None and name in ("a_row", "b_row", "a_pts", "b_pts", "a_feats", "b_feats", "coords_dist", "feats_dist"):
            _dev(t, torch.int32 if name.endswith("_row") else torch.float32, "circle_forward." + name)
    if anchors is None and (coords_dist is None or feats_dist is None or coords_dist.shape != feats_dist.shape):
        raise _lib.AprHipError("circle_forward: give the anchors or two distance matrices of one shape")
    if anchors is not None:
        na = nb = int(g["a_row"].shape[0])
        dev = g["a_row"].device
    else:
        na, nb = (int(v) for v in coords_dist.shape)
        dev = coords_dist.device
    st_a = torch.empty((na, 8), dtype=torch.float32, device=dev)
    st_b = torch.empty((nb, 8), dtype=torch.float32, device=dev)
    out = torch.empty(4, dtype=torch.float32, device=dev)
    nn = torch.empty(na, dtype=torch.int32, device=dev)
    check(_lib_().apr_circle_forward(ptr(g.get("a_feats")), ptr(g.get("a_pts")), ptr(g.get("a_row")), na, ptr(g.get("b_feats")),
                                     ptr(g.get("b_pts")), ptr(g.get("b_row")), nb, ptr(coords_dist), ptr(feats_dist),
                                     _circle_params(params), ptr(st_a), ptr(st_b), ptr(out), ptr(nn), stream()))
    return out, st_a, st_b, nn


def circle_backward(params, st_a, st_b, out4, grad_out, anchors=None, coords_dist=None, feats_dist=None):
    g = anchors or {}
    for name, t in (("st_a", st_a), ("st_b", st_b), ("out4", out4), ("grad_out", grad_out)):
        _dev(t, torch.float32, "circle_backward." + name)
    grad_out = grad_out.contiguous()
    na, nb = int(st_a.shape[0]), int(st_b.shape[0])
    d_a = d_b = d_fd = None
    if anchors is not None:
        d_a, d_b = torch.empty_like(g["a_feats"]), torch.empty_like(g["b_feats"])
    else:
        d_fd = torch.empty_like(feats_dist)
    check(_lib_().apr_circle_backward(ptr(g.get("a_feats")), ptr(g.get("a_pts")), ptr(g.get("a_row")), na, ptr(g.get("b_feats")),
                                      ptr(g.get("b_pts")), ptr(g.get("b_row")), nb, ptr(coords_dist), ptr(feats_dist),
                                      _circle_params(params), ptr(st_a), ptr(st_b), ptr(out4), ptr(grad_out), ptr(d_a), ptr(d_b),
                                      ptr(d_fd), stream()))
    return (d_a, d_b) if anchors is not None else d_fd


def circle_scatter(d_anchor, row, n_rows):
    d_anchor, row = _dev(d_anchor, torch.float32, "circle_scatter.d_anchor"), _dev(row, torch.int32, "circle_scatter.row")
    P, D = d_anchor.shape
    out = torch.zeros((n_rows, D), dtype=torch.float32, device=d_anchor.device)
    check(_lib_().apr_circle_scatter(ptr(d_anchor), ptr(row), P, D, ptr(out), n_rows, stream()))
    return out


def ransac_pose(xyz0, xyz1, corr, max_dist, edge_ratio=0.9, max_iter=4000000, seed=0):
    xyz0 = _f32(xyz0, "ransac.xyz0").contiguous()
    xyz1 = _f32(xyz1, "ransac.xyz1").contiguous()
    if corr.dtype != torch.int64 or not corr.is_cuda:
        raise _lib.AprHipError("ransac_pose: corr must be an int64 GPU tensor")
    corr = corr.contiguous()
    n0, n1 = xyz0.shape[0], xyz1.shape[0]
    if corr.shape[0] != n0:
        raise _lib.AprHipError("ransac_pose: one correspondence per source point expected")
    lib = _lib_()
    sb = int(lib.apr_ransac_scratch_bytes(n0, int(max_iter)))
    scratch = torch.empty(sb, dtype=torch.uint8, device=xyz0.device)
    res = (C.c_double * 20)()
    check(lib.apr_ransac_pose(ptr(xyz0), n0, ptr(xyz1), n1, ptr(corr), float(max_dist), float(edge_ratio),
                              int(max_iter), int(seed) & 0xFFFFFFFFFFFFFFFF, ptr(scratch), sb, res, stream()))
    r = np.array(list(res), dtype=np.float64)
    T = r[:16].reshape(4, 4).copy()
    info = dict(inliers=int(r[16]), rmse=float(r[17]), best_iteration=int(r[18]), n_valid=int(r[19]),
                fitness=float(r[16]) / max(n0, 1))
    return T, info


def match_pose_batch(feats0, feats1, pts0, pts1, max_dist, edge_ratio=0.9, max_iter=4000000, seeds=None):
    B = len(feats0)
    if not (B == len(feats1) == len(pts0) == len(pts1)) or B == 0:
        raise _lib.AprHipError("match_pose_batch: need the same (non-zero) number of entries in every list")
    if seeds is None:
        seeds = range(B)
    lib = _lib_()
    descs = (_lib.PairDesc * B)()
    keep = []
    c = feats0[0].shape[1]
    n0m = n1m = 0
    for i in range(B):
        f0 = _f32(feats0[i], "match_pose_batch.feats0").contiguous()
        f1 = _f32(feats1[i], "match_pose_batch.feats1").contiguous()
        p0 = _f32(pts0[i], "match_pose_batch.pts0").contiguous()
        p1 = _f32(pts1[i], "match_pose_batch.pts1").contiguous()
        if f0.shape[1] != c or f1.shape[1] != c or p0.shape != (f0.shape[0], 3) or p1.shape != (f1.shape[0], 3):
            raise _lib.AprHipError("match_pose_batch: inconsistent shapes in pair %d" % i)
        keep += [f0, f1, p0, p1]
        d = descs[i]
        d.f0, d.n0, d.f1, d.n1 = f0.data_ptr(), f0.shape[0], f1.data_ptr(), f1.shape[0]
        d.xyz0, d.xyz1, d.seed = p0.data_ptr(), p1.data_ptr(), int(seeds[i]) & 0xFFFFFFFFFFFFFFFF
        n0m, n1m = max(n0m, f0.shape[0]), max(n1m, f1.shape[0])
    sb = int(lib.apr_match_pose_batch_scratch_bytes(B, n0m, n1m, c, int(max_iter)))
    scratch = torch.empty(sb, dtype=torch.uint8, device=keep[0].device)
    res = (C.c_double * (20 * B))()
    check(lib.apr_match_pose_batch(descs, B, c, float(max_dist), float(edge_ratio), int(max_iter), ptr(scratch), sb, res,
                                   stream()))
    r = np.array(list(res), dtype=np.float64).reshape(B, 20)
    out = []
    for i in range(B):
        n0 = descs[i].n0
        out.append((r[i, :16].reshape(4, 4).copy(),
                    dict(inliers=int(r[i, 16]), rmse=float(r[i, 17]), best_iteration=int(r[i, 18]),
                         n_valid=int(r[i, 19]), fitness=float(r[i, 16]) / max(n0, 1))))
    return out


def coords_bbox(coords):
    if coords.dtype != torch.int32 or coords.dim() != 2 or coords.shape[1] != 4 or not coords.is_contiguous():
        raise _lib.AprHipError("coords_bbox: coords must be contiguous int32 [n, 4]")
    bbox = torch.empty(8, dtype=torch.int32, device=coords.device)
    check(_lib_().apr_coords_bbox(ptr(coords), coords.shape[0], ptr(bbox), stream()))
    return bbox


def occ_conv_supported(bbox, kernel_size, cout, n=None):
    if bbox is None or kernel_size not in (3, 5, 7) or cout % 8 != 0:
        return False
    box = (C.c_int32 * 8)(*[int(v) for v in bbox])
    if n is not None:
        return bool(_lib_().apr_occ_conv_pays(box, int(kernel_size), int(n)))
    return int(_lib_().apr_occ_conv_scratch_bytes(box, int(kernel_size))) > 0


def occ_conv(coords, n, bbox, kernel_size, w, scale=None, shift=None, relu=False, residual=None, out=None, keep=None):
    lib = _lib_()
    w = _f32(w, "occ_conv.w").contiguous()
    K, cout = w.shape
    if K != kernel_size ** 3:
        raise _lib.AprHipError("occ_conv: w must be [kernel_size^3, cout]")
    box = (C.c_int32 * 8)(*[int(v) for v in bbox])
    sb = int(lib.apr_occ_conv_scratch_bytes(box, int(kernel_size)))
    if sb == 0:
        raise _lib.AprHipError("occ_conv: empty or oversized bounding box (use occ_conv_supported)")
    if out is None:
        out = torch.empty((n, cout), dtype=torch.float32, device=coords.device)
    out, ldo = _rows(out, "occ_conv.out")
    ldr = 0
    if residual is not None:
        residual, ldr = _rows(residual, "occ_conv.residual")
    scratch = torch.empty(sb, dtype=torch.uint8, device=coords.device)
    check(lib.apr_occ_conv(ptr(coords), int(n), box, int(kernel_size), ptr(w), cout, ptr(scale), ptr(shift), ptr(residual),
                           ldr, int(bool(relu)), ptr(out), ldo, ptr(scratch), sb, stream()))
    if keep is not None:
        keep.append((scratch, tuple(int(v) for v in bbox), int(kernel_size), int(n), coords.data_ptr()))
    return out


def kernel_map_occ(out_map: CoordMap, in_map: CoordMap, kernel_size: int, scale: int, occ) -> torch.Tensor:
    scratch, bbox, bks = occ[:3]
    if len(occ) < 5 or in_map.n is None or occ[3] != in_map.n or occ[4] != in_map.coords.data_ptr():
        return kernel_map(out_map, in_map, kernel_size, scale)
    nbr = torch.empty((out_map.n, kernel_size ** 3), dtype=torch.int32, device=out_map.coords.device)
    box = (C.c_int32 * 8)(*bbox)
    check(_lib_().apr_kernel_map_occ(ptr(out_map.coords), out_map.n, None, ptr(in_map.keys), ptr(in_map.vals), in_map.cap,
                                     int(kernel_size), int(scale), box, int(bks), ptr(scratch), ptr(nbr), stream()))
    return nbr


def set_ransac_screen(mode):
    check(_lib_().apr_ransac_set_screen(-1 if mode is None else int(bool(mode))))


_RANSAC_OPTIONS = {"screen": 0, "count": 1, "prune": 2, "force_rounds": 3}


def set_ransac_option(name, value):
    check(_lib_().apr_ransac_set_option(_RANSAC_OPTIONS[name], -1 if value is None else int(bool(value))))


class ransac_options:

    def __init__(self, **kw):
        self.kw = kw

    def __enter__(self):
        for k, v in self.kw.items():
            set_ransac_option(k, v)

    def __exit__(self, *exc):
        for k in self.kw:
            set_ransac_option(k, None)


def ransac_sampling_launches():
    out = (C.c_int64 * 2)()
    check(_lib_().apr_ransac_sampling_launches(out))
    return int(out[0]), int(out[1])


def set_match_lanes(lanes):
    check(_lib_().apr_match_pose_set_lanes(int(lanes)))


def match_pose_batch_async(feats0, feats1, pts0, pts1, max_dist, edge_ratio=0.9, max_iter=4000000, seeds=None):
    B = len(feats0)
    if not (B == len(feats1) == len(pts0) == len(pts1)) or B == 0:
        raise _lib.AprHipError("match_pose_batch: need the same (non-zero) number of entries in every list")
    if seeds is None:
        seeds = range(B)
    lib = _lib_()
    descs = (_lib.PairDesc * B)()
    keep = []
    c = feats0[0].shape[1]
    n0m = n1m = 0
    for i in range(B):
        f0 = _f32(feats0[i], "match_pose_batch.feats0").contiguous()
        f1 = _f32(feats1[i], "match_pose_batch.feats1").contiguous()
        p0 = _f32(pts0[i], "match_pose_batch.pts0").contiguous()
        p1 = _f32(pts1[i], "match_pose_batch.pts1").contiguous()
        if f0.shape[1] != c or f1.shape[1] != c or p0.shape != (f0.shape[0], 3) or p1.shape != (f1.shape[0], 3):
            raise _lib.AprHipError("match_pose_batch: inconsistent shapes in pair %d" % i)
        keep += [f0, f1, p0, p1]
        d = descs[i]
        d.f0, d.n0, d.f1, d.n1 = f0.data_ptr(), f0.shape[0], f1.data_ptr(), f1.shape[0]
        d.xyz0, d.xyz1, d.seed = p0.data_ptr(), p1.data_ptr(), int(seeds[i]) & 0xFFFFFFFFFFFFFFFF
        n0m, n1m = max(n0m, f0.shape[0]), max(n1m, f1.shape[0])
    sb = int(lib.apr_match_pose_batch_scratch_bytes(B, n0m, n1m, c, int(max_iter)))
    scratch = torch.empty(sb, dtype=torch.uint8, device=keep[0].device)
    slots = torch.empty(int(lib.apr_match_pose_batch_slot_bytes(B)), dtype=torch.uint8, pin_memory=True)
    st = stream()
    check(lib.apr_match_pose_batch_enqueue(descs, B, c, float(max_dist), float(edge_ratio), int(max_iter), ptr(scratch),
                                           sb, C.c_void_p(slots.data_ptr()), st))
    pf = PendingFetch.__new__(PendingFetch)
    pf._host = slots
    pf.event = fetch_event()
    pf.event.record()
    pf._keep = (keep, scratch, descs)

    def then(_):
        res = (C.c_double * (20 * B))()
        check(lib.apr_match_pose_batch_finish(descs, B, c, float(max_dist), float(edge_ratio), int(max_iter),
                                              ptr(scratch), sb, C.c_void_p(slots.data_ptr()), res, st))
        r = np.array(list(res), dtype=np.float64).reshape(B, 20)
        return [(r[i, :16].reshape(4, 4).copy(),
                 dict(inliers=int(r[i, 16]), rmse=float(r[i, 17]), best_iteration=int(r[i, 18]), n_valid=int(r[i, 19]),
                      fitness=float(r[i, 16]) / max(descs[i].n0, 1))) for i in range(B)]

    pf._then = then
    return pf


def ransac_pose_geometric(xyz0, xyz1, corr, max_dist, edge_ratio=0.9, max_iter=50000, max_validation=1000, seed=0):
    xyz0 = _f32(xyz0, "ransac.xyz0").contiguous()
    xyz1 = _f32(xyz1, "ransac.xyz1").contiguous()
    if corr.dtype != torch.int64 or not corr.is_cuda or corr.shape[0] != xyz0.shape[0]:
        raise _lib.AprHipError("ransac_pose_geometric: corr must be an int64 GPU tensor, one entry per source point")
    corr = corr.contiguous()
    n0, n1 = xyz0.shape[0], xyz1.shape[0]
    lib = _lib_()
    sb = int(lib.apr_ransac_geometric_scratch_bytes(n0, n1, int(max_iter)))
    scratch = torch.empty(sb, dtype=torch.uint8, device=xyz0.device)
    res = (C.c_double * 20)()
    check(lib.apr_ransac_pose_geometric(ptr(xyz0), n0, ptr(xyz1), n1, ptr(corr), float(max_dist), float(edge_ratio),
                                        int(max_iter), int(max_validation), int(seed) & 0xFFFFFFFFFFFFFFFF,
                                        ptr(scratch), sb, res, stream()))
    r = np.array(list(res), dtype=np.float64)
    info = dict(inliers=int(r[16]), rmse=float(r[17]), best_iteration=int(r[18]), n_valid=int(r[19]),
                fitness=float(r[16]) / max(n0, 1))
    return r[:16].reshape(4, 4).copy(), info


MUTUAL_FEATURE_WIDTH = 32


def score_argmax(a, b):
    a, b = _dev(a, torch.float32, "score_argmax.a"), _dev(b, torch.float32, "score_argmax.b")
    if a.dim() != 2 or b.dim() != 2 or a.shape[1] != b.shape[1]:
        raise _lib.AprHipError("score_argmax: need two [n, d] matrices of one width")
    if a.shape[1] != MUTUAL_FEATURE_WIDTH:
        raise _lib.AprHipError(f"score_argmax: feature width {a.shape[1]} is not covered (the arg-max kernel is limited to "
                               f"d = {MUTUAL_FEATURE_WIDTH})")
    if a.shape[0] == 0 or b.shape[0] == 0:
        raise _lib.AprHipError("score_argmax: empty cloud")
    dev = a.device
    ia = torch.arange(a.shape[0], dtype=torch.int32, device=dev)
    ib = torch.arange(b.shape[0], dtype=torch.int32, device=dev)
    n = torch.tensor([a.shape[0], b.shape[0]], dtype=torch.int32, device=dev)
    return gathered_argmax(a, ia, n[0:1], b, ib, n[1:2])


def dense_argmax(scores):
    scores = _dev(scores, torch.float32, "dense_argmax.scores")
    if scores.dim() != 2 or scores.shape[0] == 0 or scores.shape[1] == 0:
        raise _lib.AprHipError("dense_argmax: need a non-empty [n, m] matrix")
    n, m = scores.shape
    row_arg = torch.empty(n, dtype=torch.int32, device=scores.device)
    col_arg = torch.empty(m, dtype=torch.int32, device=scores.device)
    check(_lib_().apr_dense_argmax(ptr(scores), n, m, ptr(row_arg), ptr(col_arg), stream()))
    return row_arg, col_arg


def mutual_select(row_arg, col_arg, n_src_dev=None, n_tgt_dev=None):
    row_arg, col_arg = _dev(row_arg, torch.int32, "mutual_select.row_arg"), _dev(col_arg, torch.int32, "mutual_select.col_arg")
    if row_arg.dim() != 1 or col_arg.dim() != 1 or row_arg.shape[0] == 0 or col_arg.shape[0] == 0:
        raise _lib.AprHipError("mutual_select: need two non-empty vectors")
    for name, t in (("n_src_dev", n_src_dev), ("n_tgt_dev", n_tgt_dev)):
        if t is not None:
            _dev(t, torch.int32, "mutual_select." + name)
    n_src, n_tgt = row_arg.shape[0], col_arg.shape[0]
    pairs = torch.zeros((min(n_src, n_tgt), 2), dtype=torch.int32, device=row_arg.device)
    count = torch.zeros(1, dtype=torch.int32, device=row_arg.device)
    check(_lib_().apr_mutual_select(ptr(row_arg), ptr(n_src_dev), n_src, ptr(col_arg), ptr(n_tgt_dev), n_tgt, ptr(pairs),
                                    ptr(count), stream()))
    return pairs, count


def inlier_ratio(src_pcd, tgt_pcd, rot, trans, row_arg, pairs, count, threshold):
    src_pcd, tgt_pcd = _dev(src_pcd, torch.float32, "inlier_ratio.src_pcd"), _dev(tgt_pcd, torch.float32, "inlier_ratio.tgt_pcd")
    rot, trans = _dev(rot, torch.float32, "inlier_ratio.rot"), _dev(trans, torch.float32, "inlier_ratio.trans")
    row_arg, pairs = _dev(row_arg, torch.int32, "inlier_ratio.row_arg"), _dev(pairs, torch.int32, "inlier_ratio.pairs")
    count = _dev(count, torch.int32, "inlier_ratio.count")
    if src_pcd.dim() != 2 or src_pcd.shape[1] != 3 or tgt_pcd.dim() != 2 or tgt_pcd.shape[1] != 3:
        raise _lib.AprHipError("inlier_ratio: the clouds must be [n, 3]")
    if rot.numel() != 9 or trans.numel() != 3 or row_arg.shape[0] != src_pcd.shape[0] or pairs.dim() != 2 or pairs.shape[1] != 2:
        raise _lib.AprHipError("inlier_ratio: need rot [3,3], trans [3,1], one row_arg per source point and pairs [k, 2]")
    n_src, n_tgt, cap = src_pcd.shape[0], tgt_pcd.shape[0], pairs.shape[0]
    dev = src_pcd.device
    dist_wo = torch.empty(n_src, dtype=torch.float32, device=dev)
    dist_w = torch.zeros(cap, dtype=torch.float32, device=dev)
    out = torch.empty(8, dtype=torch.float32, device=dev)
    check(_lib_().apr_inlier_ratio(ptr(src_pcd), n_src, ptr(tgt_pcd), n_tgt, ptr(rot), ptr(trans), ptr(row_arg), ptr(pairs),
                                   ptr(count), cap, float(threshold), ptr(dist_wo), ptr(dist_w), ptr(out), stream()))
    return dist_wo, dist_w, out


def ransac_pose_pairs_geometric(xyz0, xyz1, pairs, n_pairs, max_dist, max_iter=50000, max_validation=1000, seed=0):
    xyz0 = _f32(xyz0, "ransac_pairs.xyz0").contiguous()
    xyz1 = _f32(xyz1, "ransac_pairs.xyz1").contiguous()
    pairs = _dev(pairs, torch.int32, "ransac_pairs.pairs")
    n_pairs = int(n_pairs)
    if pairs.dim() != 2 or pairs.shape[1] != 2 or not 0 <= n_pairs <= pairs.shape[0]:
        raise _lib.AprHipError("ransac_pose_pairs_geometric: pairs must be int32 [k, 2] with 0 <= n_pairs <= k")
    n0, n1 = xyz0.shape[0], xyz1.shape[0]
    lib = _lib_()
    sb = int(lib.apr_ransac_pairs_geometric_scratch_bytes(n0, n1, n_pairs, int(max_iter), int(max_validation)))
    scratch = torch.empty(max(sb, 256), dtype=torch.uint8, device=xyz0.device)
    res = (C.c_double * 20)()
    check(lib.apr_ransac_pose_pairs_geometric(ptr(xyz0), n0, ptr(xyz1), n1, ptr(pairs), n_pairs, float(max_dist),
                                              int(max_iter), int(max_validation), int(seed) & 0xFFFFFFFFFFFFFFFF,
                                              ptr(scratch), sb, res, stream()))
    r = np.array(list(res), dtype=np.float64)
    info = dict(inliers=int(r[16]), rmse=float(r[17]), best_iteration=int(r[18]), n_valid=int(r[19]),
                fitness=float(r[16]) / max(n0, 1), n_pairs=n_pairs)
    return r[:16].reshape(4, 4).copy(), info


def ransac_pose_geometric_async(xyz0, xyz1, corr, max_dist, edge_ratio=0.9, max_iter=50000, max_validation=1000, seed=0):
    xyz0 = _f32(xyz0, "ransac.xyz0").contiguous()
    xyz1 = _f32(xyz1, "ransac.xyz1").contiguous()
    if corr.dtype != torch.int64 or not corr.is_cuda or corr.shape[0] != xyz0.shape[0]:
        raise _lib.AprHipError("ransac_pose_geometric: corr must be an int64 GPU tensor, one entry per source point")
    corr = corr.contiguous()
    n0, n1 = xyz0.shape[0], xyz1.shape[0]
    lib = _lib_()
    sb = int(lib.apr_ransac_geometric_scratch_bytes(n0, n1, int(max_iter)))
    scratch = torch.empty(sb, dtype=torch.uint8, device=xyz0.device)
    raw = torch.empty(int(lib.apr_ransac_raw_bytes()), dtype=torch.uint8, device=xyz0.device)
    check(lib.apr_ransac_pose_geometric_async(ptr(xyz0), n0, ptr(xyz1), n1, ptr(corr), float(max_dist),
                                              float(edge_ratio), int(max_iter), int(max_validation),
                                              int(seed) & 0xFFFFFFFFFFFFFFFF, ptr(scratch), sb, ptr(raw), stream()))
    return raw


def ransac_decode(raw_host, n0):
    res = (C.c_double * 20)()
    raw_host = np.ascontiguousarray(raw_host)
    check(_lib_().apr_ransac_decode(raw_host.ctypes.data, res))
    r = np.array(list(res), dtype=np.float64)
    info = dict(inliers=int(r[16]), rmse=float(r[17]), best_iteration=int(r[18]), n_valid=int(r[19]),
                fitness=float(r[16]) / max(n0, 1))
    return r[:16].reshape(4, 4).copy(), info


def irls_pose(pts0, pts1, weight=None):
    pts0 = _f32(pts0, "irls.pts0").contiguous()
    pts1 = _f32(pts1, "irls.pts1").contiguous()
    n = pts0.shape[0]
    if weight is not None:
        weight = _f32(weight, "irls.weight").contiguous().view(-1)
    lib = _lib_()
    sb = int(lib.apr_irls_scratch_bytes(n))
    scratch = torch.empty(sb, dtype=torch.uint8, device=pts0.device)
    T = (C.c_float * 16)()
    check(lib.apr_irls_pose(ptr(pts0), ptr(pts1), ptr(weight), n, T, ptr(scratch), sb, stream()))
    return torch.tensor(list(T), dtype=torch.float32).view(4, 4)


VALID_RECORD_FLOATS = 24
VALID_CORR_DIST, VALID_RTE, VALID_RRE, VALID_HIT_RATIO, VALID_N_CORR, VALID_T_EST = 0, 1, 2, 3, 4, 5
VALID_CHAMFER, VALID_REG, VALID_N_HIT = 21, 22, 23


def valid_pair(xyz0, xyz1, nn, T_gt, records, slot, sel0=None, sel1=None, hit_thresh=0.1):
    xyz0 = _f32(xyz0, "valid_pair.xyz0").contiguous()
    xyz1 = _f32(xyz1, "valid_pair.xyz1").contiguous()
    T_gt = _f32(T_gt, "valid_pair.T_gt").contiguous()
    if T_gt.numel() != 16:
        raise _lib.AprHipError("valid_pair: T_gt must hold 16 floats")
    _lib.require_gpu_tensor(records, torch.float32, "valid_pair.records")
    if records.dim() != 2 or records.shape[1] != VALID_RECORD_FLOATS:
        raise _lib.AprHipError(f"valid_pair: records must be [pairs, {VALID_RECORD_FLOATS}]")
    idx = [None if t is None else _lib.require_gpu_tensor(t, torch.int64, name)
           for t, name in ((sel0, "valid_pair.sel0"), (sel1, "valid_pair.sel1"), (nn, "valid_pair.nn"))]
    m0 = xyz0.shape[0] if sel0 is None else sel0.shape[0]
    m1 = xyz1.shape[0] if sel1 is None else sel1.shape[0]
    if nn.shape[0] != m0:
        raise _lib.AprHipError(f"valid_pair: nn has {nn.shape[0]} rows for {m0} source rows")
    lib = _lib_()
    sb = int(lib.apr_valid_pair_scratch_bytes(m0))
    scratch = torch.empty(sb, dtype=torch.uint8, device=xyz0.device)
    check(lib.apr_valid_pair(ptr(xyz0), xyz0.shape[0], ptr(xyz1), xyz1.shape[0], ptr(idx[0]), ptr(idx[1]), m0, m1,
                             ptr(idx[2]), ptr(T_gt), float(hit_thresh), ptr(records), records.shape[0], int(slot),
                             ptr(scratch), sb, stream()))


ICP_RECORD_DOUBLES = 20
ICP_FITNESS, ICP_RMSE, ICP_N_CORR, ICP_ITERATIONS = 16, 17, 18, 19


def icp_batch(src, src_offsets, tgt, tgt_offsets, init, max_dist, max_iteration=30, relative_fitness=1e-6,
              relative_rmse=1e-6, tgt_of_problem=None, want_corr=False):
    src = _f32(src, "icp_batch.src").contiguous()
    tgt = _f32(tgt, "icp_batch.tgt").contiguous()
    if src.dim() != 2 or src.shape[1] != 3 or tgt.dim() != 2 or tgt.shape[1] != 3:
        raise _lib.AprHipError("icp_batch: src and tgt must be [rows, 3]")
    so = np.ascontiguousarray(np.asarray(src_offsets, dtype=np.int64))
    to = np.ascontiguousarray(np.asarray(tgt_offsets, dtype=np.int64))
    nb, n_tgt = len(so) - 1, len(to) - 1
    if nb < 1 or n_tgt < 1 or so[-1] != src.shape[0] or to[-1] != tgt.shape[0]:
        raise _lib.AprHipError("icp_batch: the offsets must cover the rows of src / tgt")
    top = None
    if tgt_of_problem is not None:
        top = np.ascontiguousarray(np.asarray(tgt_of_problem, dtype=np.int32))
        if len(top) != nb:
            raise _lib.AprHipError("icp_batch: one target segment per problem expected")
    if not torch.is_tensor(init):
        init = torch.from_numpy(np.ascontiguousarray(np.asarray(init, dtype=np.float64)))
    init = init.to(device=src.device, dtype=torch.float64).contiguous()
    if init.numel() != nb * 16:
        raise _lib.AprHipError(f"icp_batch: init must hold {nb} 4x4 transforms")
    lib = _lib_()
    rec = torch.empty((nb, ICP_RECORD_DOUBLES), dtype=torch.float64, device=src.device)
    corr = torch.empty(src.shape[0], dtype=torch.int32, device=src.device) if want_corr else None
    sb = int(lib.apr_icp_scratch_bytes(src.shape[0], tgt.shape[0], nb))
    scratch = torch.empty(sb, dtype=torch.uint8, device=src.device)
    check(lib.apr_icp_batch(ptr(src), so.ctypes.data_as(C.c_void_p), ptr(tgt), to.ctypes.data_as(C.c_void_p), n_tgt,
                            None if top is None else top.ctypes.data_as(C.c_void_p), nb, ptr(init), float(max_dist),
                            int(max_iteration), float(relative_fitness), float(relative_rmse), ptr(rec), ptr(corr),
                            ptr(scratch), sb, stream()))
    return rec, corr


INFORMATION_SUMS = 10
POSEGRAPH_MAX_NODES = 8
POSEGRAPH_OK, POSEGRAPH_NO_WEIGHT, POSEGRAPH_NO_WEIGHT_PRUNED, POSEGRAPH_NOT_POSITIVE, POSEGRAPH_MALFORMED = 0, 1, 2, 3, 4


def _transform_rows(T, nb, name):
    if not torch.is_tensor(T):
        T = torch.from_numpy(np.ascontiguousarray(np.asarray(T, dtype=np.float64)))
    T = T.to(device=torch.device('cuda', torch.cuda.current_device()), dtype=torch.float64).contiguous()
# ... 152 lines not shown
```

include/apr_hip.h:

```cpp
#ifndef APR_HIP_H
#define APR_HIP_H

#include <stddef.h>
#include <stdint.h>

#ifdef __cplusplus
extern "C" {
#endif

#define APR_OK 0
#define APR_EINVAL (-1)
#define APR_EHIP (-2)
#define APR_ETIMEOUT (-3)
#define APR_ERANGE (-3)

const char* apr_last_error(void);
int apr_version(void);
int apr_device_count(void);
int32_t apr_struct_sizes(int32_t* out, int32_t n);
int apr_event_wait(void* event, int32_t poll_us);
int apr_event_wait_timeout(void* event, int32_t poll_us, int64_t timeout_us);


int64_t apr_hash_capacity(int64_t n);

size_t apr_map_scratch_bytes(int64_t n);

int apr_voxelize(const float* xyz, int64_t n, float voxel_size, int32_t batch,
                 int32_t* coords, void* stream);

int apr_map_build(const int32_t* coords_in, int64_t n, const int32_t* n_dev, int32_t floor_to,
                  uint64_t* keys, int32_t* vals, int64_t cap,
                  int32_t* out_coords, int64_t* out_first, int32_t* n_out,
                  int32_t* status, void* scratch, size_t scratch_bytes, void* stream);

int apr_kernel_map_transpose(const int32_t* nbr, int64_t n_out, int32_t K, int64_t n_in, int32_t* nbr_t, void* stream);

int apr_voxelize_segments(const float* xyz, int64_t n, float voxel_size, const int64_t* offsets, int32_t nseg,
                          int32_t* coords, void* stream);

#define APR_MAX_FRAMES 64
int apr_voxelize_frames(const float* const* frames_host, const int64_t* offsets_host, int32_t nseg, float voxel_size,
                        int32_t* coords, int64_t* offsets_dev, void* stream);
int apr_gather_frame_points(const float* const* frames_host, const int64_t* offsets_host, int32_t nseg,
                            const int64_t* out_first, const int32_t* n_dev, int64_t n_max, float* pts, void* stream);

#define APR_MAX_PACK 96
int apr_pack_i32(const int32_t* const* srcs_host, const int32_t* counts_host, int32_t nsrc, int32_t* dst,
                 int32_t* zero_ptr, int64_t zero_words, void* stream);
int apr_fill_bytes(void* ptr, int32_t byte_value, size_t bytes, void* stream);
int apr_kernel_map_transpose_prefilled(const int32_t* nbr, int64_t n_out, int32_t K, int64_t n_in, int32_t* nbr_t,
                                       void* stream);

int apr_segment_counts(const int64_t* out_first, const int32_t* n_dev, const int64_t* offsets, int32_t nseg,
                       int32_t* counts, void* stream);

int apr_kernel_map_same(const int32_t* coords, int64_t n, const uint64_t* keys, const int32_t* vals, int64_t cap,
                        int32_t kernel_size, int32_t scale, int32_t* nbr, void* stream);
int apr_kernel_map(const int32_t* out_coords, int64_t n_out, const int32_t* n_out_dev,
                   const uint64_t* in_keys, const int32_t* in_vals, int64_t cap,
                   int32_t kernel_size, int32_t scale, int32_t* nbr, void* stream);

int apr_coords_bbox(const int32_t* coords, int64_t n, int32_t* bbox_dev, void* stream);
size_t apr_occ_conv_scratch_bytes(const int32_t* bbox_host, int32_t kernel_size);
int apr_occ_conv_pays(const int32_t* bbox_host, int32_t kernel_size, int64_t n);
int apr_occ_conv(const int32_t* coords, int64_t n, const int32_t* bbox_host, int32_t kernel_size, const float* w,
                 int32_t cout, const float* scale, const float* shift, const float* residual, int64_t ldr,
                 int32_t relu, float* out, int64_t ldo, void* scratch, size_t scratch_bytes, void* stream);
int apr_kernel_map_occ(const int32_t* out_coords, int64_t n_out, const int32_t* n_out_dev, const uint64_t* in_keys,
                       const int32_t* in_vals, int64_t cap, int32_t kernel_size, int32_t scale,
                       const int32_t* bbox_host, int32_t bitmap_kernel_size, const void* occ_scratch, int32_t* nbr,
                       void* stream);


int64_t apr_spconv_packed_size(int32_t K, int32_t cin, int32_t cout);
int apr_spconv_pack_weights(const float* w, int32_t K, int32_t cin, int32_t cout,
                            float* w_packed, void* stream);

int apr_weights_flip_transpose(const float* w, int32_t K, int32_t cin, int32_t cout, int32_t flip, float* wt, void* stream);

int apr_spconv_fwd(const float* in, int64_t ldi, const int32_t* nbr, int64_t n_out,
                   int32_t K, int32_t cin, int32_t cout, const float* w_packed,
                   const float* scale, const float* shift,
                   const float* residual, int64_t ldr, int32_t relu,
                   float* out, int64_t ldo, void* stream);

#define APR_PAIR_COUNTER_STRIDE 64
int32_t apr_pairlist_counter_ints(void);
size_t apr_pairlist_bytes(int64_t n_out, int32_t K);
int apr_pairlist_build(const int32_t* nbr, int64_t n_out, int32_t K, int32_t* counters, void* plist,
                       size_t plist_bytes, void* stream);
int apr_spconv_ws_fwd(const float* in, int64_t ldi, const int32_t* counters, const void* plist, int64_t n_out,
                      int32_t K, int32_t cin,
                      int32_t cout, const float* w_packed, const float* scale, const float* shift,
                      const float* residual, int64_t ldr, int32_t relu, float* out, int64_t ldo,
                      float* prod_scratch, void* stream);
int64_t apr_spconv_packed_bf3_bytes(int32_t K, int32_t cin, int32_t cout);
int apr_spconv_pack_weights_bf3(const float* w, int32_t K, int32_t cin, int32_t cout, void* w_bf3, void* stream);
int apr_spconv_pack_weights_bf3_ex(const float* w, int32_t K, int32_t cin, int32_t cout, int32_t flip, int32_t transposed,
                                   void* w_bf3, void* stream);
int apr_spconv_ws_fwd_bf3(const float* in, int64_t ldi, const int32_t* counters, const void* plist, int64_t n_out,
                          int32_t K, int32_t cin, int32_t cout, const float* w_packed, const void* w_bf3,
                          const float* scale, const float* shift, const float* residual, int64_t ldr, int32_t relu,
                          float* out, int64_t ldo, float* prod_scratch, void* stream);

int32_t apr_spconv_os_tile_rows(int64_t n_out, int32_t cin, int32_t cout);
size_t apr_spconv_os_pairs_bytes(int64_t n_out, int32_t K, int32_t R);
int apr_spconv_os_pairs_build(const int32_t* nbr, int64_t n_out, int64_t n_in, int32_t K, int32_t R, void* os_pairs,
                              size_t os_pairs_bytes, void* stream);
int apr_spconv_os_trace(uint64_t* host_out, int32_t n);
int apr_spconv_os_set_debug(int32_t mode);
int apr_spconv_os_fwd(const float* in, int64_t ldi, const void* os_pairs, int64_t n_out, int32_t K, int32_t R,
                      int32_t cin, int32_t cout, const void* w_bf3, const float* scale, const float* shift,
                      const float* residual, int64_t ldr, int32_t relu, float* out, int64_t ldo, void* stream);

size_t apr_spconv_wgrad_scratch_bytes(int64_t n_out, int32_t K, int32_t cin, int32_t cout);
int apr_spconv_wgrad(const float* in, int64_t ldi, const float* dout, int64_t ldo, const int32_t* nbr, int64_t n_out,
                     int32_t K, int32_t cin, int32_t cout, float* dw, void* scratch, size_t scratch_bytes,
                     void* stream);
int apr_spconv_wgrad_same_level(const float* in, int64_t ldi, const float* dout, int64_t ldo, const int32_t* nbr,
                                int64_t n_out, int32_t K, int32_t cin, int32_t cout, float* dw, void* scratch,
                                size_t scratch_bytes, void* stream);

size_t apr_pairlist3_bytes(int64_t n_out);
int apr_pairlist3_build(const int32_t* nbr, int64_t n_out, int32_t K, int32_t* counters, void* plist3, size_t plist3_bytes,
                        void* stream);
int apr_spconv_ws3_supported(int32_t K, int32_t cin, int32_t cout);
int apr_spconv_ws3_fwd_bf3(const float* in, int64_t ldi, const int32_t* counters, const void* plist3, int64_t n_out,
                           int32_t cin, int32_t cout, const void* w_bf3, const float* scale, const float* shift,
                           const float* residual, int64_t ldr, int32_t relu, float* out, int64_t ldo, float* prod_scratch,
                           void* stream);

typedef struct apr_spconv_desc {
  const float* in; int64_t ldi; const int32_t* nbr; int64_t n_out;
  int32_t K, cin, cout, relu;
  const float* w_packed; const float* scale; const float* shift;
  const float* residual; int64_t ldr;
  float* out; int64_t ldo;
  int32_t* counters;
  void* plist;
  float* prod_scratch;
  int64_t plist_bytes;
  const void* w_bf3;
  void* os_pairs;
  int64_t os_rows;
  int64_t os_build_bytes;
  int64_t os_n_in;
  int32_t l2norm;
  int32_t ws3;
} apr_spconv_desc;
int apr_spconv_fwd_batch(const apr_spconv_desc* descs_host, int32_t n, void* stream);
int apr_spconv_fwd_batch_timed(const apr_spconv_desc* descs, int32_t n, float* layer_ms, void* stream);

typedef struct apr_resunet_layer {
  int32_t K, cin, cout, relu;
  const float* w_packed;
  const void* w_bf3;
  const float* scale; const float* shift;
} apr_resunet_layer;
typedef struct apr_resunet_plan {
  apr_resunet_layer layer[23];
  const float* conv1_w;
  int32_t conv1_ks, normalize;
  uint32_t ws_conv, ws_block, os_block;
  int32_t ws3, ws3_cin128, os_min_rows, occ_kernel_map;
  int64_t ws3_max_rows_128;
} apr_resunet_plan;
typedef struct apr_level_map {
  const int32_t* coords; const uint64_t* keys; const int32_t* vals; int64_t cap; int64_t n;
} apr_level_map;
int apr_resunet_encode_supported(const apr_resunet_plan* plan, const apr_level_map* lv, const int32_t* bbox_host);
size_t apr_resunet_encode_scratch_bytes(const apr_resunet_plan* plan, const apr_level_map* lv, const int32_t* bbox_host);
int apr_resunet_encode(const apr_resunet_plan* plan, const apr_level_map* lv, const int32_t* bbox_host, int32_t* counters,
                       int32_t n_counter_slots, void* scratch, size_t scratch_bytes, float* out, int64_t ldo, void* stream);

typedef struct apr_pyramid {
  apr_level_map lv[4];
  const int64_t* first;
  const float* pts;
  int32_t* header; int32_t header_ints;
  int32_t compact; int64_t compact_rows;
  int32_t* counters; int32_t n_counter_slots;
} apr_pyramid;
size_t apr_voxel_pyramid_scratch_bytes(int64_t n_points, int32_t nseg);
int apr_voxel_pyramid(const float* const* frames_host, const int64_t* offsets_host, int32_t nseg, float voxel_size,
                      void* arena, size_t arena_bytes, apr_pyramid* out, void* stream);


int apr_bn_stats(const float* x, int64_t ld, int64_t n, int32_t c,
                 float* mean, float* var, void* scratch, size_t scratch_bytes, void* stream);
size_t apr_bn_stats_scratch_bytes(int64_t n, int32_t c);

size_t apr_norm_backward_scratch_bytes(int64_t n, int32_t c);
int apr_norm_backward(const float* x, int64_t ldx, const float* dy, int64_t lddy, int64_t n, int32_t c,
                      const float* mean, const float* rstd, const float* gamma, float* dx, int64_t lddx,
                      float* dgamma, float* dbeta, void* scratch, size_t scratch_bytes, void* stream);

int apr_bn_train_fwd(const float* z, int64_t ldz, int64_t n, int32_t c, const float* gamma, const float* beta,
                     float eps, float momentum, float* running_mean, float* running_var, const float* residual,
                     int64_t ldr, int32_t relu, float* y, int64_t ldy, float* save_mean, float* save_rstd,
                     int64_t* num_batches_tracked, const int64_t* seg_offsets_host, int32_t nseg, void* scratch,
                     size_t scratch_bytes, void* stream);
int apr_bn_train_bwd(const float* z, int64_t ldz, const float* y, int64_t ldy, const float* dy, int64_t lddy,
                     int64_t n, int32_t c, const float* mean, const float* rstd, const float* gamma, int32_t relu,
                     float* dx, int64_t lddx, float* dres, int64_t lddres, float* dgamma, float* dbeta,
                     const int64_t* seg_offsets_host, int32_t nseg, void* scratch, size_t scratch_bytes, void* stream);

int apr_col_sums(const float* x, int64_t ld, int64_t n, int32_t c, float* sums, void* scratch, size_t scratch_bytes,
                 void* stream);

int apr_norm_params(const float* x, int64_t ld, int64_t n, int32_t c, float eps, float* scale, float* shift,
                    void* scratch, size_t scratch_bytes, void* stream);

int apr_instance_norm_act(const float* x, int64_t ldx, int64_t n, int32_t c, float eps, const float* residual,
                          int64_t ldr, int32_t relu, float negative_slope, float* y, int64_t ldy, void* scratch,
                          size_t scratch_bytes, void* stream);
int apr_instance_norm_act_seg(const float* x, int64_t ldx, int64_t n, int32_t c, float eps, const float* residual,
                              int64_t ldr, int32_t relu, float negative_slope, float* y, int64_t ldy,
                              const int64_t* seg_offsets_host, int32_t nseg, void* scratch, size_t scratch_bytes,
                              void* stream);

int apr_affine_act(const float* x, int64_t ldx, int64_t n, int32_t c,
                   const float* scale, const float* shift,
                   const float* residual, int64_t ldr, int32_t relu, float negative_slope,
                   float* y, int64_t ldy, void* stream);
int apr_act_backward(const float* dy, int64_t lddy, const float* y, int64_t ldy, int64_t n, int32_t c, int32_t mode,
                     float negative_slope, float* dz, int64_t lddz, void* stream);

int apr_l2_normalize(const float* x, int64_t ldx, int64_t n, int32_t c,
                     float* y, int64_t ldy, void* stream);
int apr_l2_normalize_backward(const float* x, int64_t ldx, const float* dy, int64_t lddy, int64_t n, int32_t c,
                              float* dx, int64_t lddx, void* stream);

int apr_feature_nn(const float* f0, int64_t n0, const float* f1, int64_t n1, int32_t c,
                   uint64_t* best, void* stream);
size_t apr_feature_nn_fast_scratch_bytes(int64_t n0, int64_t n1, int32_t c);
int apr_feature_nn_fast(const float* f0, int64_t n0, const float* f1, int64_t n1, int32_t c, uint64_t* best,
                        void* scratch, size_t scratch_bytes, void* stream);
int apr_nn_unpack(const uint64_t* best, int64_t n, int64_t* idx, float* d2, void* stream);

size_t apr_ransac_scratch_bytes(int64_t n0, int64_t max_iter);
int apr_ransac_pose(const float* xyz0, int64_t n0, const float* xyz1, int64_t n1,
                    const int64_t* corr, double max_dist, double edge_ratio,
                    int64_t max_iter, uint64_t seed,
                    void* scratch, size_t scratch_bytes, double* result_host, void* stream);

size_t apr_ransac_geometric_scratch_bytes(int64_t n0, int64_t n1, int64_t max_iter);
int apr_ransac_pose_geometric(const float* xyz0, int64_t n0, const float* xyz1, int64_t n1,
                              const int64_t* corr, double max_dist, double edge_ratio,
                              int64_t max_iter, int64_t max_validation, uint64_t seed,
                              void* scratch, size_t scratch_bytes, double* result_host, void* stream);
size_t apr_ransac_raw_bytes(void);
int apr_ransac_pose_geometric_async(const float* xyz0, int64_t n0, const float* xyz1, int64_t n1,
                                    const int64_t* corr, double max_dist, double edge_ratio, int64_t max_iter,
                                    int64_t max_validation, uint64_t seed, void* scratch, size_t scratch_bytes,
                                    void* raw_dev, void* stream);
int apr_ransac_decode(const void* raw_host, double* result_host);

typedef struct {
  const float* f0; int64_t n0;
  const float* f1; int64_t n1;
  const float* xyz0;
  const float* xyz1;
  uint64_t seed;
} apr_pair_desc;
size_t apr_match_pose_batch_scratch_bytes(int32_t B, int64_t n0_max, int64_t n1_max, int32_t c, int64_t max_iter);
int apr_match_pose_batch(const apr_pair_desc* pairs, int32_t B, int32_t c, double max_dist, double edge_ratio,
                         int64_t max_iter, void* scratch, size_t scratch_bytes, double* results_host, void* stream);
size_t apr_match_pose_batch_slot_bytes(int32_t B);
int apr_match_pose_batch_enqueue(const apr_pair_desc* pairs, int32_t B, int32_t c, double max_dist, double edge_ratio,
                                 int64_t max_iter, void* scratch, size_t scratch_bytes, void* slots_host, void* stream);
int apr_match_pose_batch_finish(const apr_pair_desc* pairs, int32_t B, int32_t c, double max_dist, double edge_ratio,
                                int64_t max_iter, void* scratch, size_t scratch_bytes, const void* slots_host,
                                double* results_host, void* stream);

int apr_ransac_set_screen(int32_t mode);
int apr_ransac_set_option(int32_t option, int32_t value);
int apr_ransac_sampling_launches(int64_t* out2);

int apr_match_pose_set_lanes(int32_t lanes);

int apr_irls_pose(const float* pts0, const float* pts1, const float* weight, int64_t n,
                  float* T_host, void* scratch, size_t scratch_bytes, void* stream);
size_t apr_irls_scratch_bytes(int64_t n);

#define APR_VALID_RECORD_FLOATS 24
int apr_valid_pair(const float* xyz0, int64_t n0, const float* xyz1, int64_t n1, const int64_t* sel0,
                   const int64_t* sel1, int64_t m0, int64_t m1, const int64_t* nn, const float* T_gt,
                   float hit_thresh, float* records, int64_t n_slots, int64_t slot, void* scratch,
                   size_t scratch_bytes, void* stream);
size_t apr_valid_pair_scratch_bytes(int64_t m0);

int apr_contrastive_reduce(const float* pos_f0, const float* pos_f1, int32_t p, int32_t c,
                           const uint64_t* nn01, const uint64_t* nn10, const int64_t* sel0, const int64_t* sel1,
                           const int64_t* pos_ind0, const int64_t* pos_ind1, const int64_t* sorted_pos_keys,
                           int32_t n_keys, int64_t hash_seed, float pos_thresh, float neg_thresh,
                           double* out6, void* stream);


size_t apr_grid_subsample_scratch_bytes(int64_t n);
int apr_grid_subsample(const float* pts, int64_t n, const int32_t* lengths_host, int32_t nb, float dl,
                       const float* feats, int32_t fdim, float* out_pts, float* out_feats,
                       int32_t* out_lengths_host, void* scratch, size_t scratch_bytes, void* stream);
int apr_grid_subsample_async(const float* pts, int64_t n, const int32_t* lengths_host, int32_t nb, float dl,
                             const float* feats, int32_t fdim, float* out_pts, float* out_feats,
                             int32_t* lengths_status_dev, void* scratch, size_t scratch_bytes, void* stream);

size_t apr_voxel_down_sample_scratch_bytes(int64_t n);
int apr_voxel_down_sample(const float* pts, int64_t n, const int32_t* lengths_host, int32_t nb, double voxel_size,
                          double* centroid, float* centroid32, int32_t* count, int32_t* first, int32_t* index,
                          int32_t* out_lengths_host, void* scratch, size_t scratch_bytes, void* stream);

int apr_sample_augment(const double* pts, const double* u, int64_t n, double noise, const double* rot_host,
                       double scale, const double* shift_host, float* out, void* stream);

int apr_cloud_mean(const float* pts, int64_t n, double* mean, void* stream);

size_t apr_radius_scratch_bytes(int64_t nq, int64_t ns);
int apr_radius_neighbors(const float* queries, int64_t nq, const float* supports, int64_t ns,
                         const int32_t* q_lengths_host, const int32_t* s_lengths_host, int32_t nb, float radius,
                         int32_t limit, int32_t* out, int64_t out_ld, int32_t* width_host,
                         void* scratch, size_t scratch_bytes, void* stream);

int apr_radius_neighbors_async(const float* queries, int64_t nq, const float* supports, int64_t ns,
                               const int32_t* q_lengths_host, const int32_t* s_lengths_host, int32_t nb, float radius,
                               int32_t limit, int32_t* out, int64_t out_ld, int32_t* flags_dev,
                               void* scratch, size_t scratch_bytes, void* stream);
int apr_radius_neighbors_regrid_async(const float* queries, int64_t nq, const float* supports, int64_t ns,
                               const int32_t* q_lengths_host, const int32_t* s_lengths_host, int32_t nb, float radius,
                               int32_t limit, int32_t* out, int64_t out_ld, int32_t* flags_dev,
                               void* scratch, size_t scratch_bytes, void* stream);

int apr_knn(const float* pts, int32_t n, int32_t k, int32_t skip_first, int32_t* out, void* stream);


int apr_dense_gemm_bf3(const float* in, int64_t ldi, int64_t M, int32_t cin, int32_t cout, const void* w_bf3,
                       const float* scale, const float* shift, const float* residual, int64_t ldr, int32_t relu,
                       float* out, int64_t ldo, void* stream);
int32_t apr_dense_rows_bf3_ok(int32_t cin, int32_t cout);
int32_t apr_dense_rows_bf3_route(int64_t M, int32_t cin, int32_t cout);
int apr_dense_rows_bf3(const float* in, int64_t ldi, int64_t M, int32_t cin, int32_t cout, const void* w_bf3,
                       const float* scale, const float* shift, const float* residual, int64_t ldr, int32_t relu,
                       int32_t l2norm, float* out, int64_t ldo, void* stream);
size_t apr_dense_gemm_bf3_norm_scratch_bytes(int64_t M, int32_t cout, int32_t nseg);
int apr_dense_gemm_bf3_norm_act(const float* in, int64_t ldi, int64_t M, int32_t cin, int32_t cout, const void* w_bf3,
                                float eps, const float* residual, int64_t ldr, int32_t act_mode, float negative_slope,
                                float* out, int64_t ldo, const int64_t* seg_offsets_host, int32_t nseg, void* scratch,
                                size_t scratch_bytes, void* stream);

typedef struct apr_kp_resnet_desc {
  const float* x; int64_t ldx; int64_t n_in;
  int32_t in_dim, mid, out_dim, strided;
  const float* q_pts; const float* s_pts; int64_t n_out;
  const int32_t* nbr; int32_t H; int32_t n_kp;
  const float* kernel_points; float extent; float eps; float slope; int32_t nseg;
  const void* w_unary1; const void* w_kpconv; const void* w_unary2; const void* w_shortcut;
  const int64_t* seg_in; const int64_t* seg_out;
  float* out; int64_t ldo;
  void* scratch; size_t scratch_bytes;
} apr_kp_resnet_desc;
size_t apr_kp_resnet_scratch_bytes(const apr_kp_resnet_desc* desc);
int apr_kp_resnet_block(const apr_kp_resnet_desc* desc, void* stream);

int64_t apr_weighted_choice_round(double* p, int64_t n, int64_t* found, int64_t n_uniq, int64_t n_new_zeroed,
                                  const double* x, int64_t k, double* cdf, int32_t* stamp, int32_t round_id);

int apr_row_sums(const float* x, int64_t ld, int64_t n, int32_t c, float* out, void* stream);

int apr_kpconv_weighted(const float* q_pts, int64_t nq, const float* s_pts, int64_t ns, const int32_t* nbr,
                        int32_t H, const float* x, int64_t ldx, int32_t cin, const float* kernel_points,
                        int32_t n_kp, float extent, const float* rowsum, float* wf, int64_t ldwf, void* stream);
int apr_kpconv_dfeat(const float* q_pts, int64_t nq, const float* s_pts, int64_t ns, const int32_t* nbr, int32_t H,
                     const float* dwf, int64_t lddwf, int32_t cin, const float* kernel_points, int32_t n_kp,
                     float extent, const float* rowsum, float* dx, int64_t lddx, void* stream);

int apr_kpconv_dfeat_contrib(const float* q_pts, int64_t nq, const float* s_pts, int64_t ns, const int32_t* nbr, int32_t H,
                             const float* dwf, int64_t lddwf, int32_t cin, const float* kernel_points, int32_t n_kp,
                             float extent, const float* rowsum, float* contrib, void* stream);
size_t apr_reverse_table_scratch_bytes(int64_t nq, int32_t H, int64_t ns);
int apr_reverse_table_build(const int32_t* nbr, int64_t nq, int32_t H, int64_t ns, int32_t* rev_t, int32_t* start,
                            void* scratch, size_t scratch_bytes, void* stream);
int apr_reverse_gather(const float* src, int32_t c, const int32_t* rev_t, const int32_t* start, int64_t ns, float* out,
                       int64_t ldo, void* stream);
int apr_reverse_gather_range(const float* src, int32_t c, const int32_t* rev_t, const int32_t* start, int64_t ns,
                             int64_t t_lo, int64_t t_hi, int32_t accumulate, float* out, int64_t ldo, void* stream);

int apr_gather_pool(const float* x, int64_t ldx, int64_t ns, int32_t c, const int32_t* inds, int32_t H,
                    int64_t nq, int32_t mode, float* out, int64_t ldo, void* stream);

int apr_gather_pool_argmax(const float* x, int64_t ldx, int64_t ns, int32_t c, const int32_t* inds, int32_t H, int64_t nq,
                           float* out, int64_t ldo, uint8_t* amax, void* stream);
int apr_gather_pool_backward(const float* dout, int64_t lddo, int32_t c, const int32_t* rev_t, const int32_t* start,
                             int64_t ns, int32_t H, const uint8_t* amax, int32_t mode, float* dx, int64_t lddx, void* stream);

int apr_edge_features(const float* f, int64_t ldf, int32_t n, int32_t c, const int32_t* knn, int32_t k,
                      float* out, void* stream);

int apr_edge_features_backward(const float* de, int32_t n, int32_t c, int32_t k, float* d_center, int64_t ldd,
                               float* contrib, void* stream);

int apr_group_max(const float* y, int64_t ldy, int32_t n, int32_t k, int32_t c, const float* scale,
                  const float* shift, float slope, float* out, int64_t ldo, void* stream);

int apr_mha(const float* q, const float* k, const float* v, int32_t n, int32_t m, int32_t dim, int32_t heads,
            float* out, void* stream);

int apr_mha_train_forward(const float* q, const float* k, const float* v, int32_t n, int32_t m, int32_t dim, int32_t heads,
                          int32_t vdim, float* P, float* out, void* stream);
int apr_mha_train_backward(const float* q, const float* k, const float* v, const float* P, const float* dout, int32_t n,
                           int32_t m, int32_t dim, int32_t heads, int32_t vdim, float* dS, float* dq, float* dk, float* dv,
                           void* stream);

int apr_mha_headmajor(const float* q, const float* k, const float* v, int32_t n, int32_t m, int32_t dim,
                      int32_t heads, float* out, void* stream);

#define APR_GCN_MAX_LAYERS 8
typedef struct apr_gcn_layer {
  int32_t kind;
  int32_t k, heads;
  float eps1, eps2, eps3;
  const void *w1, *w2, *w3;
  const float *b1, *b2;
  const void *wq, *wk, *wv, *wm;
  const float *bq, *bk, *bv, *bm;
} apr_gcn_layer;
typedef struct apr_gcn_desc {
  int32_t n_layers, c;
  apr_gcn_layer layer[APR_GCN_MAX_LAYERS];
} apr_gcn_desc;
size_t apr_gcn_scratch_bytes(const apr_gcn_desc* d, int32_t n0, int32_t n1);
int apr_gcn_forward(const apr_gcn_desc* d, const float* pts0, int32_t n0, const float* pts1, int32_t n1, const float* x0,
                    int64_t ldx0, const float* x1, int64_t ldx1, float* out0, int64_t ldo0, float* out1, int64_t ldo1,
                    void* scratch, size_t scratch_bytes, void* stream);

int apr_softmax_matvec(const float* a, const float* b, const float* w, int32_t n, int32_t m, int32_t c,
                       float temperature, float* out, void* stream);
int apr_softmax_matvec_bt(const float* a, const float* bt, const float* w, int32_t n, int32_t m, int32_t c,
                          float temperature, float* out, void* stream);
int apr_softmax_matvec_mfma(const float* a, const float* b, const float* w, int32_t n, int32_t m, int32_t c,
                            float temperature, float* out, void* stream);

int apr_score_head(const float* x, int64_t ldx, int64_t n, float* y, void* stream);


int apr_transform_points(const float* pts, int64_t n, const float* T16_dev, float* out, void* stream);

size_t apr_crop_scratch_bytes(int64_t n);
int apr_crop_to_radius(const float* key_pts, int64_t n_key, const float* pts, int64_t n, float* out,
                       int32_t* n_out_dev, void* scratch, size_t scratch_bytes, void* stream);

int apr_chamfer_sum(const float* a, int64_t n, const float* b, int64_t m, double* out_dev, void* scratch,
                    size_t scratch_bytes, void* stream);

size_t apr_nn3_scratch_bytes(int64_t n, int64_t m);
int apr_nn3(const float* a, int64_t n, const float* b, int64_t m, float cell, uint64_t* out_packed, double* sum_dev,
            void* scratch, size_t scratch_bytes, void* stream);
int apr_nn3_batch(const float* a, const int64_t* a_offsets_host, const float* b, const int64_t* b_offsets_host, int32_t nb,
                  float cell, uint64_t* out_packed, double* sums_dev, const double* sum_scale_host, void* scratch,
                  size_t scratch_bytes, void* stream);


int apr_overlap_labels(const int64_t* corr, int64_t n_corr, int64_t n_src, int64_t n_tgt, float* gt, int32_t* src_idx,
                       int32_t* tgt_idx, int32_t* counts3, void* stream);

size_t apr_weighted_bce_scratch_bytes(void);
int apr_weighted_bce_forward(const float* pred, const float* gt, int64_t n, const int32_t* n_dev, float* out8, void* scratch,
                             size_t scratch_bytes, void* stream);
int apr_weighted_bce_backward(const float* pred, const float* gt, int64_t n, const int32_t* n_dev, const float* out8,
                              const float* grad_out, const int32_t* scatter_pos, float* dpred, void* stream);

int apr_gathered_argmax(const float* a, const int32_t* a_idx, const int32_t* na_dev, int64_t na_max, const float* b,
                        const int32_t* b_idx, const int32_t* nb_dev, int64_t nb_max, int32_t d, int32_t* row_arg,
                        int32_t* col_arg, void* stream);

int apr_saliency_labels(const float* src_pcd, const float* tgt_pcd, const float* rot9, const float* trans3,
                        const int32_t* src_idx, const int32_t* tgt_idx, const int32_t* counts3, const int32_t* row_arg,
                        const int32_t* col_arg, const float* scores_saliency, int64_t n_src, int64_t n_tgt, float radius,
                        float* labels, float* sel_scores, int32_t* pos, float* dist, void* stream);

int apr_circle_select(const int64_t* corr, int64_t n_corr, const float* src_pcd, int64_t n_src, const float* tgt_pcd,
                      int64_t n_tgt, const float* rot9, const float* trans3, float thresh, int32_t* filt, int32_t* count,
                      void* stream);

int apr_circle_gather(const int64_t* corr, const int32_t* filt, const int32_t* count, const int64_t* choice, int32_t p,
                      const float* src_pcd, const float* tgt_pcd, const float* src_feats, const float* tgt_feats, int32_t d,
                      const float* rot9, const float* trans3, int32_t* a_row, int32_t* b_row, float* a_pts, float* b_pts,
                      float* a_feats, float* b_feats, void* stream);

int apr_circle_forward(const float* a_feats, const float* a_pts, const int32_t* a_row, int32_t na, const float* b_feats,
// ... 53 lines not shown
```

Before: 2730.

## Batch kernel-map and voxel-pyramid builds into fewer multi-map launches

Adds batched kernels that build several kernel maps (hash and occupancy-bitmap variants) and several transposes in a single launch, using a per-block selector over a descriptor table. The encoder now defers all map builds and stage conv batches until the end of its walk, then issues them as grouped launches. The voxel pyramid front end merges per-level insert, count, scan and compact steps into multi-level kernels. The aim is to cut kernel launch count and small-kernel tail overhead. In exchange, builds can no longer overlap with the convs that consume them, and scratch reuse becomes more complex.

```diff
diff --git a/apr_amd/_lib.py b/apr_amd/_lib.py
--- a/apr_amd/_lib.py
+++ b/apr_amd/_lib.py
@@ -47,6 +47,15 @@
     _fields_ = [("lv", LevelMap * 4), ("first", C.c_void_p), ("pts", C.c_void_p), ("header", C.c_void_p),
                 ("header_ints", C.c_int32), ("compact", C.c_int32), ("compact_rows", C.c_int64),
                 ("counters", C.c_void_p), ("n_counter_slots", C.c_int32)]
+
+
+class KmapDesc(C.Structure):
+    _fields_ = [("out_coords", C.c_void_p), ("n_out", C.c_int64), ("in_keys", C.c_void_p), ("in_vals", C.c_void_p),
+                ("cap", C.c_int64), ("kernel_size", C.c_int32), ("scale", C.c_int32), ("nbr", C.c_void_p)]
+
+
+class KmapTransposeDesc(C.Structure):
+    _fields_ = [("nbr", C.c_void_p), ("n_out", C.c_int64), ("K", C.c_int32), ("n_in", C.c_int64), ("nbr_t", C.c_void_p)]
 
 
 class GcnLayer(C.Structure):
@@ -79,6 +88,10 @@
     "apr_struct_sizes": (_i32, [_p, _i32]),
     "apr_ransac_set_screen": (C.c_int, [_i32]),
     "apr_ransac_set_option": (C.c_int, [_i32, _i32]),
+    "apr_set_batched_builds": (C.c_int, [_i32]),
+    "apr_kernel_map_batch": (C.c_int, [_p, _i32, _p]),
+    "apr_kernel_map_occ_batch": (C.c_int, [_p, _i32, _p, _i32, _p, _p]),
+    "apr_kernel_map_transpose_batch": (C.c_int, [_p, _i32, _p]),
     "apr_ransac_sampling_launches": (C.c_int, [_p]),
     "apr_event_wait": (C.c_int, [_p, _i32]),
     "apr_event_wait_timeout": (C.c_int, [_p, _i32, _i64]),
diff --git a/apr_amd/csrc/common.h b/apr_amd/csrc/common.h
--- a/apr_amd/csrc/common.h
+++ b/apr_amd/csrc/common.h
@@ -57,6 +57,65 @@
                           const unsigned* run_if, void* stream);
 
 int apr_internal_fill(void* ptr, int32_t byte_value, size_t bytes, hipStream_t st);
+
+int apr_internal_batched_builds();
+
+struct AprFrontMap {
+  uint64_t* keys;
+  int32_t* vals;
+  int64_t cap;
+  int32_t* coords;
+};
+struct AprFrontEnd {
+  int64_t N, R;
+  int32_t* hdr;
+  int64_t clear_words, bbox_word;
+  int32_t* raw;
+  float* pts;
+  int64_t* first;
+  void* sc;
+  size_t sc_bytes;
+  AprFrontMap dedup, lvl[4];
+};
+int apr_internal_front_batched(const AprFrontEnd& fe, const float* const* frames, const int64_t* offs, int32_t nseg, float vs,
+                               hipStream_t st);
+
+#define APR_KMAP_BATCH_MAX 8
+struct AprKmapBatch {
+  const int4* coords[APR_KMAP_BATCH_MAX];
+  const unsigned long long* keys[APR_KMAP_BATCH_MAX];
+  const int* vals[APR_KMAP_BATCH_MAX];
+  int* nbr[APR_KMAP_BATCH_MAX];
+  long long n_out[APR_KMAP_BATCH_MAX];
+  uint32_t mask[APR_KMAP_BATCH_MAX];
+  int ks[APR_KMAP_BATCH_MAX], scale[APR_KMAP_BATCH_MAX];
+  unsigned blk0[APR_KMAP_BATCH_MAX + 1];
+  int n;
+};
+struct AprKmapOne {
+  const int4* coords;
+  const unsigned long long* keys;
+  const int* vals;
+  int* nbr;
+  long long n_out;
+  uint32_t mask;
+  int ks, scale;
+  unsigned lblk, nblk;
+};
+#ifdef __HIPCC__
+__device__ static inline AprKmapOne apr_kmap_select(const AprKmapBatch& b, unsigned blk) {
+  AprKmapOne o = {b.coords[0], b.keys[0], b.vals[0], b.nbr[0], b.n_out[0], b.mask[0], b.ks[0], b.scale[0], blk, b.blk0[1]};
+#pragma unroll
+  for (int a = 1; a < APR_KMAP_BATCH_MAX; ++a)
+    if (a < b.n && blk >= b.blk0[a]) {
+      o.coords = b.coords[a]; o.keys = b.keys[a]; o.vals = b.vals[a]; o.nbr = b.nbr[a]; o.n_out = b.n_out[a];
+      o.mask = b.mask[a]; o.ks = b.ks[a]; o.scale = b.scale[a];
+      o.lblk = blk - b.blk0[a]; o.nblk = b.blk0[a + 1] - b.blk0[a];
+    }
+  return o;
+}
+#endif
+int apr_internal_kmap_batch_fill(const apr_kmap_desc* maps, int32_t n, AprKmapBatch* b, const char* who);
 
 bool apr_internal_dense_ok(int64_t M, int32_t cin, int32_t cout);
 bool apr_internal_dense_rows_route(int64_t M, int32_t cin, int32_t cout);
diff --git a/apr_amd/csrc/encoder.hip b/apr_amd/csrc/encoder.hip
--- a/apr_amd/csrc/encoder.hip
+++ b/apr_amd/csrc/encoder.hip
@@ -1,4 +1,20 @@
+#include <atomic>
+
 #include "common.h"
+
+static std::atomic<int> g_batched_builds{-1};
+int apr_internal_batched_builds() {
+  const int v = g_batched_builds.load(std::memory_order_relaxed);
+  if (v >= 0) return v;
+  static const int s_env = env_int("APR_BATCHED_BUILDS", 1) != 0;
+  return s_env;
+}
+
+APR_API int apr_set_batched_builds(int32_t value) {
+  APR_CHECK_ARG(value >= -1 && value <= 1, "apr_set_batched_builds: value -1, 0 or 1");
+  g_batched_builds.store(value, std::memory_order_relaxed);
+  return APR_OK;
+}
 
 namespace {
 
@@ -32,11 +48,16 @@
   size_t occ_bytes = 0;
   int32_t* tpool[3] = {};
   bool tpool_ready = false;
+  int32_t* tpool_buf = nullptr;
+  size_t tpool_ints = 0;
+  const bool batched = apr_internal_batched_builds() != 0;
   float* prod = nullptr;
   size_t prod_bytes = 0;
 
-  apr_spconv_desc descs[4];
+  apr_spconv_desc descs[24];
   int ndesc = 0;
+  int stage_end[kStages + 2];
+  int nstage = 0;
 
   Enc(const apr_resunet_plan& p, const apr_level_map* l, const int32_t* b, void* scratch, hipStream_t s)
       : P(p), lv(l), bbox(b), arena(scratch), dry(scratch == nullptr), st(s) {}
@@ -68,15 +89,17 @@
           tpool[a] = dry ? nullptr : buf + pos;
           pos += (size_t)lv[a].n * 27;
         }
-        if (!dry) run(apr_fill_bytes(buf, 0xFF, ints * 4, st));
+        tpool_buf = buf;
+        tpool_ints = ints;
+        if (!dry && !batched) run(apr_fill_bytes(buf, 0xFF, ints * 4, st));
         tpool_ready = true;
       }
       kmap[m] = tpool[l];
-      if (!dry) run(apr_kernel_map_transpose_prefilled(fwd, lv[l + 1].n, 27, lv[l].n, kmap[m], st));
+      if (!dry && !batched) run(apr_kernel_map_transpose_prefilled(fwd, lv[l + 1].n, 27, lv[l].n, kmap[m], st));
       return kmap[m];
     }
     kmap[m] = arena.take<int32_t>((size_t)n_out * 27);
-    if (dry) return kmap[m];
+    if (dry || batched) return kmap[m];
     const int lin = m < 4 ? m : m - 4, lout = m < 4 ? m : m - 4 + 1;
     const apr_level_map& in = lv[lin];
     const apr_level_map& outm = lv[lout];
@@ -191,8 +214,43 @@
     if (!dry) descs[ndesc++] = d;
   }
   void flush() {
+    if (!dry && batched) {
+      stage_end[nstage++] = ndesc;
+      return;
+    }
     if (!dry && ok() && ndesc > 0) run(apr_spconv_fwd_batch(descs, ndesc, st));
     ndesc = 0;
+  }
+
+  void finish_batched() {
+    if (!ok()) return;
+    apr_kmap_desc om[2], hm[kMaps];
+    int no = 0, nh = 0;
+    for (int m = 0; m < 7; ++m) {
+      if (!kmap[m]) continue;
+      const int lin = m < 4 ? m : m - 4, lout = m < 4 ? m : m - 4 + 1;
+      const bool by_occ = lin == 0 && P.occ_kernel_map && occ;
+      apr_kmap_desc& d = by_occ ? om[no++] : hm[nh++];
+      d.out_coords = lv[lout].coords; d.n_out = lv[lout].n;
+      d.in_keys = lv[lin].keys; d.in_vals = lv[lin].vals; d.cap = lv[lin].cap;
+      d.kernel_size = 3; d.scale = by_occ ? 1 : 1 << lin;
+      d.nbr = kmap[m];
+    }
+    if (no) run(apr_kernel_map_occ_batch(om, no, bbox, P.conv1_ks, occ, st));
+    if (nh && ok()) run(apr_kernel_map_batch(hm, nh, st));
+    if (tpool_ready && ok()) {
+      run(apr_fill_bytes(tpool_buf, 0xFF, tpool_ints * 4, st));
+      apr_kmap_transpose_desc tm[3];
+      int nt = 0;
+      for (int l = 0; l < 3; ++l) {
+        if (!kmap[7 + l]) continue;
+        tm[nt].nbr = kmap[4 + l]; tm[nt].n_out = lv[l + 1].n; tm[nt].K = 27; tm[nt].n_in = lv[l].n; tm[nt].nbr_t = kmap[7 + l];
+        ++nt;
+      }
+      if (nt && ok()) run(apr_kernel_map_transpose_batch(tm, nt, st));
+    }
+    for (int s = 0, begin = 0; s < nstage && ok(); begin = stage_end[s], ++s)
+      if (stage_end[s] > begin) run(apr_spconv_fwd_batch(descs + begin, stage_end[s] - begin, st));
   }
 
   void walk(float* out, int64_t ldo) {
@@ -226,11 +284,14 @@
     struct StageIo {
       const float* in; int64_t ldi; int cmap, bmap, lout; float* out; int64_t ldo;
     };
+    float* const skip1 = dry ? nullptr : cat1 + tr2;
+    float* const skip2 = dry ? nullptr : cat2 + tr3;
+    float* const skip3 = dry ? nullptr : cat3 + tr4;
     const StageIo io[kStages] = {
-        {nullptr, 0, -1, 0, 0, cat1 + tr2, w1},
-        {cat1 + tr2, w1, 4, 1, 1, cat2 + tr3, w2},
-        {cat2 + tr3, w2, 5, 2, 2, cat3 + tr4, w3},
-        {cat3 + tr4, w3, 6, 3, 3, s8, ch4},
+        {nullptr, 0, -1, 0, 0, skip1, w1},
+        {skip1, w1, 4, 1, 1, skip2, w2},
+        {skip2, w2, 5, 2, 2, skip3, w3},
+        {skip3, w3, 6, 3, 3, s8, ch4},
         {s8, ch4, 9, 2, 2, cat3, w3},
         {cat3, w3, 8, 1, 1, cat2, w2},
         {cat2, w2, 7, 0, 0, cat1, w1},
@@ -257,6 +318,7 @@
     conv(L[21], cat1, w1, -1, n[0], nullptr, nullptr, 0, h1, L[21].cout, false);
     conv(L[22], h1, L[21].cout, -1, n[0], nullptr, nullptr, 0, out, ldo, P.normalize != 0);
     flush();
+    if (!dry && batched) finish_batched();
   }
   size_t prod_bytes_live = 0;
 };
@@ -361,6 +423,37 @@
   for (int l = 1; l < 4; ++l) lvl[l] = take_map(f, rows, false, dry ? nullptr : hdr + 2 * l, sc, sbytes);
   if (dry) return APR_OK;
 
+  const bool batched = apr_internal_batched_builds() != 0;
+  auto publish = [&]() {
+    for (int l = 0; l < 4; ++l) {
+      out->lv[l].coords = lvl[l].coords; out->lv[l].keys = lvl[l].keys; out->lv[l].vals = lvl[l].vals;
+      out->lv[l].cap = lvl[l].cap; out->lv[l].n = lvl[l].rows;
+    }
+    if (batched && R) out->lv[0].coords = dedup.coords;
+    out->first = dedup.first;
+    out->pts = pts;
+    out->header = hdr;
+    out->header_ints = hints;
+    out->compact = R ? 1 : 0;
+    out->compact_rows = R;
+    out->counters = counters;
+    out->n_counter_slots = 16;
+  };
+  if (batched) {
+    AprFrontEnd fe;
+    fe.N = N; fe.R = R;
+    fe.hdr = hdr;
+    fe.clear_words = (int64_t)(((size_t)((char*)counters - (char*)hdr) + (size_t)16 * apr_pairlist_counter_ints() * 4) / 4);
+    fe.bbox_word = 10 + nseg;
+    fe.raw = raw; fe.pts = pts; fe.first = dedup.first;
+    fe.sc = sc; fe.sc_bytes = sbytes;
+    fe.dedup = AprFrontMap{dedup.keys, dedup.vals, dedup.cap, dedup.coords};
+    for (int l = 0; l < 4; ++l) fe.lvl[l] = AprFrontMap{lvl[l].keys, lvl[l].vals, lvl[l].cap, lvl[l].coords};
+    if (int rcb = apr_internal_front_batched(fe, frames, offs, nseg, vs, st)) return rcb;
+    publish();
+    return APR_OK;
+  }
+
   int rc;
   const size_t clear = (size_t)((char*)counters - (char*)hdr) + (size_t)16 * apr_pairlist_counter_ints() * 4;
   if ((rc = apr_pack_i32(nullptr, nullptr, 0, nullptr, hdr, (int64_t)(clear / 4), st)) != APR_OK) return rc;
@@ -379,18 +472,7 @@
     if ((rc = apr_map_build(lvl[l - 1].coords, rows, lvl[l - 1].n_dev, 1 << l, lvl[l].keys, lvl[l].vals, lvl[l].cap, lvl[l].coords,
                             nullptr, lvl[l].n_dev, lvl[l].status, lvl[l].scratch, lvl[l].scratch_bytes, st)) != APR_OK)
       return rc;
-  for (int l = 0; l < 4; ++l) {
-    out->lv[l].coords = lvl[l].coords; out->lv[l].keys = lvl[l].keys; out->lv[l].vals = lvl[l].vals;
-    out->lv[l].cap = lvl[l].cap; out->lv[l].n = lvl[l].rows;
-  }
-  out->first = dedup.first;
-  out->pts = pts;
-  out->header = hdr;
-  out->header_ints = hints;
-  out->compact = R ? 1 : 0;
-  out->compact_rows = R;
-  out->counters = counters;
-  out->n_counter_slots = 16;
+  publish();
   return APR_OK;
 }
 
diff --git a/apr_amd/csrc/hash.hip b/apr_amd/csrc/hash.hip
--- a/apr_amd/csrc/hash.hip
+++ b/apr_amd/csrc/hash.hip
@@ -1,3 +1,5 @@
+#include <limits.h>
+
 #include "common.h"
 
 namespace {
@@ -32,12 +34,10 @@
   return c;
 }
 
-__global__ void k_insert(const int4* __restrict__ coords, int64_t n, const int* __restrict__ n_dev,
-                         int floor_to, unsigned long long* __restrict__ keys, int* __restrict__ vals,
-                         uint32_t mask, int* __restrict__ slot_of, int* __restrict__ status) {
-  const int64_t i = (int64_t)blockIdx.x * blockDim.x + threadIdx.x;
+__device__ inline void insert_row(const int4* __restrict__ coords, int64_t i, int64_t n, int floor_to,
+                                  unsigned long long* __restrict__ keys, int* __restrict__ vals, uint32_t mask,
+                                  int* __restrict__ slot_of, int* __restrict__ status) {
   const int lane = threadIdx.x & 63;
-  if (n_dev) n = min((long long)n, (long long)*n_dev);
   const bool live = i < n;
   unsigned long long key = APR_KEY_EMPTY;
   bool ok = false;
@@ -77,12 +77,18 @@
   if (live) slot_of[i] = ok ? slot : -1;
 }
 
-__global__ void k_flag_count(const int* __restrict__ vals, const int* __restrict__ slot_of,
-                             int64_t n, const int* __restrict__ n_dev, uint8_t* __restrict__ flags,
-                             int* __restrict__ block_counts) {
+__global__ void k_insert(const int4* __restrict__ coords, int64_t n, const int* __restrict__ n_dev,
+                         int floor_to, unsigned long long* __restrict__ keys, int* __restrict__ vals,
+                         uint32_t mask, int* __restrict__ slot_of, int* __restrict__ status) {
+  const int64_t i = (int64_t)blockIdx.x * blockDim.x + threadIdx.x;
+  if (n_dev) n = min((long long)n, (long long)*n_dev);
+  insert_row(coords, i, n, floor_to, keys, vals, mask, slot_of, status);
+}
+
+__device__ inline void flag_count_block(const int* __restrict__ vals, const int* __restrict__ slot_of, int64_t n, int blk,
+                                        uint8_t* __restrict__ flags, int* __restrict__ block_counts) {
   __shared__ int wave_cnt[kBlock / 64];
-  int64_t i = (int64_t)blockIdx.x * blockDim.x + threadIdx.x;
-  if (n_dev) n = min((long long)n, (long long)*n_dev);
+  const int64_t i = (int64_t)blk * blockDim.x + threadIdx.x;
   bool f = false;
   if (i < n) {
     int s = slot_of[i];
@@ -95,12 +101,19 @@
   if (threadIdx.x == 0) {
     int s = 0;
     for (int w = 0; w < kBlock / 64; ++w) s += wave_cnt[w];
-    block_counts[blockIdx.x] = s;
-  }
-}
-
-__global__ void k_scan_blocks(const int* __restrict__ counts, int nblk, int* __restrict__ offsets,
-                              int* __restrict__ n_out) {
+    block_counts[blk] = s;
+  }
+}
+
+__global__ void k_flag_count(const int* __restrict__ vals, const int* __restrict__ slot_of,
+                             int64_t n, const int* __restrict__ n_dev, uint8_t* __restrict__ flags,
+                             int* __restrict__ block_counts) {
+  if (n_dev) n = min((long long)n, (long long)*n_dev);
+  flag_count_block(vals, slot_of, n, (int)blockIdx.x, flags, block_counts);
+}
+
+__device__ inline void scan_blocks(const int* __restrict__ counts, int nblk, int* __restrict__ offsets,
+                                   int* __restrict__ n_out) {
   __shared__ int wave_sum[16];
   __shared__ int carry_s;
   if (threadIdx.x == 0) carry_s = 0;
@@ -127,25 +140,38 @@
   if (threadIdx.x == 0) *n_out = carry_s;
 }
 
+__global__ void k_scan_blocks(const int* __restrict__ counts, int nblk, int* __restrict__ offsets,
+                              int* __restrict__ n_out) {
+  scan_blocks(counts, nblk, offsets, n_out);
+}
+
+__device__ inline int compact_block(const int4* __restrict__ coords, int64_t n, int blk, int floor_to,
+                                    const uint8_t* __restrict__ flags, const int* __restrict__ block_offsets,
+                                    const int* __restrict__ slot_of, int* __restrict__ vals, int4* __restrict__ out_coords,
+                                    long long* __restrict__ out_first) {
+  __shared__ int wave_cnt[kBlock / 64];
+  const int64_t i = (int64_t)blk * blockDim.x + threadIdx.x;
+  bool f = (i < n) && flags[i];
+  unsigned long long b = __ballot(f);
+  const int lane = threadIdx.x & 63, wave = threadIdx.x >> 6;
+  if (lane == 0) wave_cnt[wave] = __popcll(b);
+  __syncthreads();
+  if (!f) return -1;
+  int pos = block_offsets[blk] + __popcll(b & ((1ull << lane) - 1ull));
+  for (int w = 0; w < wave; ++w) pos += wave_cnt[w];
+  out_coords[pos] = load_coord(coords, i, floor_to);
+  if (out_first) out_first[pos] = (long long)i;
+  vals[slot_of[i]] = pos;
+  return pos;
+}
+
 __global__ void k_compact(const int4* __restrict__ coords, int64_t n, const int* __restrict__ n_dev,
                           int floor_to, const uint8_t* __restrict__ flags,
                           const int* __restrict__ block_offsets, const int* __restrict__ slot_of,
                           int* __restrict__ vals, int4* __restrict__ out_coords,
                           long long* __restrict__ out_first) {
-  __shared__ int wave_cnt[kBlock / 64];
-  int64_t i = (int64_t)blockIdx.x * blockDim.x + threadIdx.x;
   if (n_dev) n = min((long long)n, (long long)*n_dev);
-  bool f = (i < n) && flags[i];
-  unsigned long long b = __ballot(f);
-  const int lane = threadIdx.x & 63, wave = threadIdx.x >> 6;
-  if (lane == 0) wave_cnt[wave] = __popcll(b);
-  __syncthreads();
-  if (!f) return;
-  int pos = block_offsets[blockIdx.x] + __popcll(b & ((1ull << lane) - 1ull));
-  for (int w = 0; w < wave; ++w) pos += wave_cnt[w];
-  out_coords[pos] = load_coord(coords, i, floor_to);
-  if (out_first) out_first[pos] = (long long)i;
-  vals[slot_of[i]] = pos;
+  (void)compact_block(coords, n, (int)blockIdx.x, floor_to, flags, block_offsets, slot_of, vals, out_coords, out_first);
 }
 
 __device__ inline int table_lookup(const unsigned long long* __restrict__ keys,
@@ -249,6 +275,48 @@
   if (i >= 0) nbr_t[(int64_t)i * K + (int)(t % K)] = (int)(t / K);
 }
 
+__global__ void k_kernel_map_batch(AprKmapBatch b) {
+  const AprKmapOne m = apr_kmap_select(b, blockIdx.x);
+  const int ks = m.ks, K = ks * ks * ks, h = ks / 2;
+  const int64_t total = m.n_out * K;
+  for (int64_t t = (int64_t)m.lblk * blockDim.x + threadIdx.x; t < total; t += (int64_t)m.nblk * blockDim.x) {
+    const int64_t j = t / K;
+    const int o = (int)(t - j * K);
+    const int ox = o % ks - h, oy = (o / ks) % ks - h, oz = o / (ks * ks) - h;
+    const int4 c = m.coords[j];
+    const int x = c.y + ox * m.scale, y = c.z + oy * m.scale, z = c.w + oz * m.scale;
+    int r = -1;
+    if (apr_key_in_range(c.x, x, y, z)) r = table_lookup(m.keys, m.vals, m.mask, apr_pack_key(c.x, x, y, z));
+    m.nbr[t] = r;
+  }
+}
+
+constexpr int kTransposeBatchMax = 8;
+struct TransposeBatch {
+  const int* nbr[kTransposeBatchMax];
+  int* nbr_t[kTransposeBatchMax];
+  long long total[kTransposeBatchMax];
+  int K[kTransposeBatchMax];
+  unsigned blk0[kTransposeBatchMax + 1];
+  int n;
+};
+__global__ void k_map_transpose_batch(TransposeBatch b) {
+  const int* nbr = b.nbr[0];
+  int* nbr_t = b.nbr_t[0];
+  long long total = b.total[0];
+  int K = b.K[0];
+  unsigned b0 = 0;
+#pragma unroll
+  for (int a = 1; a < kTransposeBatchMax; ++a)
+    if (a < b.n && blockIdx.x >= b.blk0[a]) {
+      nbr = b.nbr[a]; nbr_t = b.nbr_t[a]; total = b.total[a]; K = b.K[a]; b0 = b.blk0[a];
+    }
+  const int64_t t = (int64_t)(blockIdx.x - b0) * blockDim.x + threadIdx.x;
+  if (t >= total) return;
+  const int i = nbr[t];
+  if (i >= 0) nbr_t[(int64_t)i * K + (int)(t % K)] = (int)(t / K);
+}
+
 constexpr int kMaxFrames = APR_MAX_FRAMES;
 struct FrameTable {
   const float* ptr[kMaxFrames];
@@ -298,6 +366,209 @@
   }
   for (long long e = (long long)blockIdx.x * blockDim.x + threadIdx.x; e < zero_words; e += (long long)gridDim.x * blockDim.x)
     zero_ptr[e] = 0;
+}
+
+
+constexpr int kFrontTables = 5;
+struct FrontInit {
+  unsigned long long* keys[kFrontTables];
+  int* vals[kFrontTables];
+  unsigned blk0[kFrontTables + 1];
+  int ntab;
+  int* zero;
+  long long zero_words;
+  long long bbox_word;
+};
+
+__global__ __launch_bounds__(kBlock) void k_front_init(FrontInit fi) {
+  int t = 0;
+#pragma unroll
+  for (int a = 1; a < kFrontTables; ++a)
+    if (a < fi.ntab && blockIdx.x >= fi.blk0[a]) t = a;
+  unsigned long long* keys = fi.keys[0];
+  int* vals = fi.vals[0];
+  unsigned b0 = 0;
+#pragma unroll
+  for (int a = 1; a < kFrontTables; ++a)
+    if (t == a) {
+      keys = fi.keys[a];
+      vals = fi.vals[a];
+      b0 = fi.blk0[a];
+    }
+  const int64_t q = ((int64_t)(blockIdx.x - b0) * kBlock + threadIdx.x) * 4;
+  const ulonglong2 e = make_ulonglong2(~0ull, ~0ull);
+  *(ulonglong2*)(keys + q) = e;
+  *(ulonglong2*)(keys + q + 2) = e;
+  *(int4*)(vals + q) = make_int4(0x7F7F7F7F, 0x7F7F7F7F, 0x7F7F7F7F, 0x7F7F7F7F);
+  for (long long w = (long long)blockIdx.x * kBlock + threadIdx.x; w < fi.zero_words; w += (long long)gridDim.x * kBlock) {
+    const long long b = w - fi.bbox_word;
+    fi.zero[w] = b >= 0 && b < 3 ? INT_MAX : b >= 3 && b < 7 ? INT_MIN : 0;
+  }
+}
+
+constexpr int kVoxBlocksMax = 2048;
+__global__ __launch_bounds__(kBlock) void k_voxelize_frames_bbox(FrameTable ft, int64_t n, float vs, int4* __restrict__ coords,
+                                                                 int* __restrict__ partial) {
+  __shared__ int s_red[kBlock / 64][8];
+  int lo[3] = {INT_MAX, INT_MAX, INT_MAX}, hi[4] = {INT_MIN, INT_MIN, INT_MIN, INT_MIN};
+  for (int64_t i = (int64_t)blockIdx.x * kBlock + threadIdx.x; i < n; i += (int64_t)gridDim.x * kBlock) {
+    const int b = frame_of(ft, i);
+    const float* p = ft.ptr[b] + 3 * (i - ft.off[b]);
+    const float x = p[0] / vs, y = p[1] / vs, z = p[2] / vs;
+    const int4 c = make_int4(b, (int)floorf(x), (int)floorf(y), (int)floorf(z));
+    coords[i] = c;
+    lo[0] = min(lo[0], c.y); lo[1] = min(lo[1], c.z); lo[2] = min(lo[2], c.w);
+    hi[0] = max(hi[0], c.y); hi[1] = max(hi[1], c.z); hi[2] = max(hi[2], c.w); hi[3] = max(hi[3], c.x);
+  }
+#pragma unroll
+  for (int d = 32; d >= 1; d >>= 1) {
+#pragma unroll
+    for (int a = 0; a < 3; ++a) lo[a] = min(lo[a], __shfl_xor(lo[a], d));
+#pragma unroll
+    for (int a = 0; a < 4; ++a) hi[a] = max(hi[a], __shfl_xor(hi[a], d));
+  }
+  const int wave = threadIdx.x >> 6;
+  if ((threadIdx.x & 63) == 0) {
+#pragma unroll
+    for (int a = 0; a < 3; ++a) s_red[wave][a] = lo[a];
+#pragma unroll
+    for (int a = 0; a < 4; ++a) s_red[wave][3 + a] = hi[a];
+  }
+  __syncthreads();
+  if (threadIdx.x < 7) {
+    const int a = threadIdx.x;
+    int v = s_red[0][a];
+    for (int w = 1; w < kBlock / 64; ++w) v = a < 3 ? min(v, s_red[w][a]) : max(v, s_red[w][a]);
+    partial[(int64_t)blockIdx.x * 8 + a] = v;
+  }
+}
+
+__global__ __launch_bounds__(1024) void k_scan_blocks_bbox(const int* __restrict__ counts, int nblk, int* __restrict__ offsets,
+                                                           int* __restrict__ n_out, const int* __restrict__ partial, int npart,
+                                                           int* __restrict__ bbox) {
+  __shared__ int s_box[128][8];
+  const int a = threadIdx.x & 7, r = threadIdx.x >> 3;
+  int v = a < 3 ? INT_MAX : INT_MIN;
+  if (a < 7)
+    for (int p = r; p < npart; p += 128) v = a < 3 ? min(v, partial[p * 8 + a]) : max(v, partial[p * 8 + a]);
+  s_box[r][a] = v;
+  __syncthreads();
+  if (threadIdx.x < 7) {
+    int w = s_box[0][a];
+    for (int q = 1; q < 128; ++q) w = a < 3 ? min(w, s_box[q][a]) : max(w, s_box[q][a]);
+    bbox[a] = w;
+  }
+  scan_blocks(counts, nblk, offsets, n_out);
+}
+
+__global__ void k_compact_pts(FrameTable ft, const int4* __restrict__ coords, int64_t n, const uint8_t* __restrict__ flags,
+                              const int* __restrict__ block_offsets, const int* __restrict__ slot_of, int* __restrict__ vals,
+                              int4* __restrict__ out_coords, long long* __restrict__ out_first, float* __restrict__ pts) {
+  const int pos = compact_block(coords, n, (int)blockIdx.x, 0, flags, block_offsets, slot_of, vals, out_coords, out_first);
+  if (pos < 0) return;
+  const int64_t i = (int64_t)blockIdx.x * blockDim.x + threadIdx.x;
+  const int b = frame_of(ft, i);
+  const float* p = ft.ptr[b] + 3 * (i - ft.off[b]);
+  pts[3 * (int64_t)pos + 0] = p[0];
+  pts[3 * (int64_t)pos + 1] = p[1];
+  pts[3 * (int64_t)pos + 2] = p[2];
+}
+
+struct LevelBuild {
+  unsigned long long* keys[4];
+  int* vals[4];
+  uint32_t mask[4];
+  int4* out_coords[4];
+  int* hdr;
+  int *slot_of, *blk_cnt, *blk_off;
+  uint8_t* flags;
+  long long rows;
+  int nb0, nbl;
+};
+struct SegOffsets {
+  long long off[kMaxFrames + 1];
+  int nseg;
+};
+
+__global__ __launch_bounds__(kBlock) void k_insert_levels(LevelBuild lb, const int4* __restrict__ coords,
+                                                          const int* __restrict__ n0_dev, SegOffsets so,
+                                                          const long long* __restrict__ first, int* __restrict__ seg_counts) {
+  const int n_all = *n0_dev;
+  const int64_t n = min(lb.rows, (long long)n_all);
+  if (blockIdx.x == 0) {
+    if (threadIdx.x < so.nseg) {
+      auto lower = [&](long long v) {
+        int lo = 0, hi = n_all;
+        while (lo < hi) {
+          const int mid = (lo + hi) >> 1;
+          if (first[mid] < v) lo = mid + 1; else hi = mid;
+        }
+        return lo;
+      };
+      seg_counts[threadIdx.x] = lower(so.off[threadIdx.x + 1]) - lower(so.off[threadIdx.x]);
+    }
+    if (lb.nb0 > 0 && threadIdx.x == 0) lb.hdr[0] = (int)n;
+  }
+  if ((int)blockIdx.x < lb.nb0) {
+    const int64_t i = (int64_t)blockIdx.x * kBlock + threadIdx.x;
+    if (i >= n) return;
+    const int4 c = coords[i];
+    if (!apr_key_in_range(c.x, c.y, c.z, c.w)) {
+      lb.hdr[1] = 1;
+      return;
+    }
+    const unsigned long long key = apr_pack_key(c.x, c.y, c.z, c.w);
+    const uint32_t mask = lb.mask[0];
+    uint32_t sl = apr_hash_u64(key) & mask;
+    bool done = false;
+    for (uint32_t probe = 0; probe <= mask; ++probe) {
+      if (lb.keys[0][sl] == APR_KEY_EMPTY && atomicCAS(&lb.keys[0][sl], APR_KEY_EMPTY, key) == APR_KEY_EMPTY) {
+        lb.vals[0][sl] = (int)i;
+        done = true;
+        break;
+      }
+      sl = (sl + 1) & mask;
+    }
+    if (!done) lb.hdr[1] = 2;
+    return;
+  }
+  const int q = (int)blockIdx.x - lb.nb0;
+  const int l = q / lb.nbl + 1, blk = q - (l - 1) * lb.nbl;
+  unsigned long long* keys = lb.keys[1];
+  int* vals = lb.vals[1];
+  uint32_t mask = lb.mask[1];
+#pragma unroll
+  for (int a = 2; a < 4; ++a)
+    if (l == a) {
+      keys = lb.keys[a];
+      vals = lb.vals[a];
+      mask = lb.mask[a];
+    }
+  insert_row(coords, (int64_t)blk * kBlock + threadIdx.x, n, 1 << l, keys, vals, mask, lb.slot_of + (int64_t)(l - 1) * lb.rows,
+             lb.hdr + 2 * l + 1);
+}
+
+__global__ __launch_bounds__(kBlock) void k_flag_count_levels(LevelBuild lb, const int* __restrict__ n0_dev) {
+  const int64_t n = min(lb.rows, (long long)*n0_dev);
+  const int l = (int)blockIdx.x / lb.nbl + 1, blk = (int)blockIdx.x - (l - 1) * lb.nbl;
+  const int* vals = l == 1 ? lb.vals[1] : l == 2 ? lb.vals[2] : lb.vals[3];
+  flag_count_block(vals, lb.slot_of + (int64_t)(l - 1) * lb.rows, n, blk, lb.flags + (int64_t)(l - 1) * lb.rows,
+                   lb.blk_cnt + (int64_t)(l - 1) * lb.nbl);
+}
+
+__global__ __launch_bounds__(1024) void k_scan_blocks_levels(LevelBuild lb) {
+  const int l = (int)blockIdx.x + 1;
+  scan_blocks(lb.blk_cnt + (int64_t)(l - 1) * lb.nbl, lb.nbl, lb.blk_off + (int64_t)(l - 1) * lb.nbl, lb.hdr + 2 * l);
+}
+
+__global__ __launch_bounds__(kBlock) void k_compact_levels(LevelBuild lb, const int4* __restrict__ coords,
+                                                           const int* __restrict__ n0_dev) {
+  const int64_t n = min(lb.rows, (long long)*n0_dev);
+  const int l = (int)blockIdx.x / lb.nbl + 1, blk = (int)blockIdx.x - (l - 1) * lb.nbl;
+  int* vals = l == 1 ? lb.vals[1] : l == 2 ? lb.vals[2] : lb.vals[3];
+  int4* out = l == 1 ? lb.out_coords[1] : l == 2 ? lb.out_coords[2] : lb.out_coords[3];
+  (void)compact_block(coords, n, blk, 1 << l, lb.flags + (int64_t)(l - 1) * lb.rows, lb.blk_off + (int64_t)(l - 1) * lb.nbl,
+                      lb.slot_of + (int64_t)(l - 1) * lb.rows, vals, out, nullptr);
 }
 
 }
@@ -398,6 +669,70 @@
   return map_transpose(nbr, n_out, K, n_in, nbr_t, true, stream);
 }
 
+int apr_internal_kmap_batch_fill(const apr_kmap_desc* maps, int32_t n, AprKmapBatch* b, const char* who) {
+  APR_CHECK_ARG(maps && n >= 1 && n <= APR_KMAP_BATCH_MAX, "%s: 1 .. %d maps", who, APR_KMAP_BATCH_MAX);
+  memset(b, 0, sizeof(*b));
+  int64_t blk = 0;
+  for (int a = 0; a < n; ++a) {
+    const apr_kmap_desc& d = maps[a];
+    APR_CHECK_ARG(d.kernel_size >= 1 && (d.kernel_size & 1) && d.kernel_size <= 7, "%s: kernel_size=%d must be odd and <= 7", who,
+                  d.kernel_size);
+    APR_CHECK_ARG((d.cap & (d.cap - 1)) == 0 && d.cap > 0, "%s: cap must be a power of two", who);
+    APR_CHECK_ARG(d.n_out >= 0 && (d.n_out == 0 || (d.out_coords && d.in_keys && d.in_vals && d.nbr)), "%s: bad map %d", who, a);
+    const int K = d.kernel_size * d.kernel_size * d.kernel_size;
+    int64_t nblk = cdiv64(d.n_out * K, kBlock);
+    if (nblk > 65536) nblk = 65536;
+    b->coords[a] = (const int4*)d.out_coords;
+    b->keys[a] = (const unsigned long long*)d.in_keys;
+    b->vals[a] = d.in_vals;
+    b->nbr[a] = d.nbr;
+    b->n_out[a] = d.n_out;
+    b->mask[a] = (uint32_t)(d.cap - 1);
+    b->ks[a] = d.kernel_size;
+    b->scale[a] = d.scale;
+    b->blk0[a] = (unsigned)blk;
+    blk += nblk;
+  }
+  for (int a = n; a <= APR_KMAP_BATCH_MAX; ++a) b->blk0[a] = (unsigned)blk;
+  b->n = n;
+  return APR_OK;
+}
+
+APR_API int apr_kernel_map_batch(const apr_kmap_desc* maps, int32_t n, void* stream) {
+  AprKmapBatch b;
+  if (int rc = apr_internal_kmap_batch_fill(maps, n, &b, "apr_kernel_map_batch")) return rc;
+  if (b.blk0[n] == 0) return APR_OK;
+  hipLaunchKernelGGL(k_kernel_map_batch, dim3(b.blk0[n]), dim3(kBlock), 0, (hipStream_t)stream, b);
+  APR_LAUNCH_CHECK();
+  return APR_OK;
+}
+
+APR_API int apr_kernel_map_transpose_batch(const apr_kmap_transpose_desc* maps, int32_t n, void* stream) {
+  APR_CHECK_ARG(maps && n >= 1 && n <= kTransposeBatchMax, "apr_kernel_map_transpose_batch: 1 .. %d tables", kTransposeBatchMax);
+  TransposeBatch b;
+  memset(&b, 0, sizeof(b));
+  int64_t blk = 0;
+  for (int a = 0; a < n; ++a) {
+    const apr_kmap_transpose_desc& d = maps[a];
+    APR_CHECK_ARG(d.n_out >= 0 && d.n_in >= 0 && d.K >= 1 && (d.nbr || d.n_out == 0) && (d.nbr_t || d.n_in == 0) &&
+                      d.n_out * (int64_t)d.K < (1ll << 38),
+                  "apr_kernel_map_transpose_batch: bad table %d", a);
+    b.nbr[a] = d.nbr;
+    b.nbr_t[a] = d.nbr_t;
+    b.total[a] = d.n_out * (int64_t)d.K;
+    b.K[a] = d.K;
+    b.blk0[a] = (unsigned)blk;
+    blk += cdiv64(b.total[a], kBlock);
+  }
+  APR_CHECK_ARG(blk < (1ll << 31), "apr_kernel_map_transpose_batch: too many rows");
+  for (int a = n; a <= kTransposeBatchMax; ++a) b.blk0[a] = (unsigned)blk;
+  b.n = n;
+  if (blk == 0) return APR_OK;
+  hipLaunchKernelGGL(k_map_transpose_batch, dim3((unsigned)blk), dim3(kBlock), 0, (hipStream_t)stream, b);
+  APR_LAUNCH_CHECK();
+  return APR_OK;
+}
+
 static __global__ __launch_bounds__(256) void k_fill_bytes(unsigned char* __restrict__ p, unsigned v32, unsigned long long head,
                                               unsigned long long n16, unsigned long long tail) {
   uint4* const q = (uint4*)(p + head);
@@ -457,6 +792,80 @@
   }
   ft.off[nseg] = offsets[nseg];
   ft.nseg = nseg;
+  return APR_OK;
+}
+
+int apr_internal_front_batched(const AprFrontEnd& fe, const float* const* frames, const int64_t* offs, int32_t nseg, float vs,
+                               hipStream_t st) {
+  FrameTable ft;
+  if (int rc = fill_frame_table(ft, frames, offs, nseg)) return rc;
+  const int64_t N = fe.N, R = fe.R, rows = R ? R : N;
+  APR_CHECK_ARG(N > 0 && N < (1ll << 31) && N == offs[nseg], "front end: 0 < points < 2^31");
+  const int nblk = (int)cdiv64(N, kBlock), nbl = (int)cdiv64(rows, kBlock), nb0 = R ? nbl : 0;
+  const int nvox = nblk < kVoxBlocksMax ? nblk : kVoxBlocksMax;
+
+  FrontInit fi;
+  memset(&fi, 0, sizeof(fi));
+  fi.ntab = R ? 5 : 4;
+  unsigned b = 0;
+  for (int t = 0; t < fi.ntab; ++t) {
+    const AprFrontMap& m = t == 0 ? fe.dedup : fe.lvl[R ? t - 1 : t];
+    APR_CHECK_ARG(m.cap >= 1024 && (m.cap & (m.cap - 1)) == 0 && m.cap >= 2 * (t == 0 ? N : rows), "front end: bad table");
+    fi.keys[t] = (unsigned long long*)m.keys;
+    fi.vals[t] = m.vals;
+    fi.blk0[t] = b;
+    b += (unsigned)(m.cap / (4 * kBlock));
+  }
+  for (int t = fi.ntab; t <= kFrontTables; ++t) fi.blk0[t] = b;
+  fi.zero = fe.hdr;
+  fi.zero_words = fe.clear_words;
+  fi.bbox_word = fe.bbox_word;
+  hipLaunchKernelGGL(k_front_init, dim3(b), dim3(kBlock), 0, st, fi);
+
+  APR_CHECK_ARG((size_t)nvox * 32 <= apr_align256((size_t)N * 12), "front end: partial boxes do not fit");
+  int* const partial = (int*)fe.pts;
+  hipLaunchKernelGGL(k_voxelize_frames_bbox, dim3(nvox), dim3(kBlock), 0, st, ft, N, vs, (int4*)fe.raw, partial);
+
+  AprArena a(fe.sc);
+  const MapScratch m = walk_map(a, N);
+  APR_CHECK_ARG(a.fits(fe.sc_bytes), "front end: scratch too small");
+  int* const n0_dev = fe.hdr + (R ? 8 : 0);
+  hipLaunchKernelGGL(k_insert, dim3(nblk), dim3(kBlock), 0, st, (const int4*)fe.raw, N, (const int*)nullptr, 0,
+                     (unsigned long long*)fe.dedup.keys, fe.dedup.vals, (uint32_t)(fe.dedup.cap - 1), m.slot_of, n0_dev + 1);
+  hipLaunchKernelGGL(k_flag_count, dim3(nblk), dim3(kBlock), 0, st, fe.dedup.vals, m.slot_of, N, (const int*)nullptr, m.flags,
+                     m.blk_cnt);
+  hipLaunchKernelGGL(k_scan_blocks_bbox, dim3(1), dim3(1024), 0, st, m.blk_cnt, nblk, m.blk_off, n0_dev, partial, nvox,
+                     fe.hdr + fe.bbox_word);
+  hipLaunchKernelGGL(k_compact_pts, dim3(nblk), dim3(kBlock), 0, st, ft, (const int4*)fe.raw, N, m.flags, m.blk_off, m.slot_of,
+                     fe.dedup.vals, (int4*)fe.dedup.coords, (long long*)fe.first, fe.pts);
+
+  LevelBuild lb;
+  memset(&lb, 0, sizeof(lb));
+  for (int l = 0; l < 4; ++l) {
+    lb.keys[l] = (unsigned long long*)fe.lvl[l].keys;
+    lb.vals[l] = fe.lvl[l].vals;
+    lb.mask[l] = (uint32_t)(fe.lvl[l].cap - 1);
+    lb.out_coords[l] = (int4*)fe.lvl[l].coords;
+  }
+  lb.hdr = fe.hdr;
+  lb.rows = rows;
+  lb.nb0 = nb0;
+  lb.nbl = nbl;
+  lb.slot_of = fe.raw;
+  const size_t flag_bytes = ((size_t)3 * rows + 3) & ~(size_t)3;
+  APR_CHECK_ARG(flag_bytes + (size_t)24 * nbl <= fe.sc_bytes && rows <= N, "front end: level scratch does not fit");
+  lb.flags = (uint8_t*)fe.sc;
+  lb.blk_cnt = (int*)((char*)fe.sc + flag_bytes);
+  lb.blk_off = lb.blk_cnt + (size_t)3 * nbl;
+  SegOffsets so;
+  memcpy(so.off, ft.off, sizeof(so.off));
+  so.nseg = nseg;
+  hipLaunchKernelGGL(k_insert_levels, dim3(nb0 + 3 * nbl), dim3(kBlock), 0, st, lb, (const int4*)fe.dedup.coords, n0_dev, so,
+                     (const long long*)fe.first, fe.hdr + 10);
+  hipLaunchKernelGGL(k_flag_count_levels, dim3(3 * nbl), dim3(kBlock), 0, st, lb, n0_dev);
+  hipLaunchKernelGGL(k_scan_blocks_levels, dim3(3), dim3(1024), 0, st, lb);
+  hipLaunchKernelGGL(k_compact_levels, dim3(3 * nbl), dim3(kBlock), 0, st, lb, (const int4*)fe.dedup.coords, n0_dev);
+  APR_LAUNCH_CHECK();
   return APR_OK;
 }
 
diff --git a/apr_amd/csrc/occ.hip b/apr_amd/csrc/occ.hip
--- a/apr_amd/csrc/occ.hip
+++ b/apr_amd/csrc/occ.hip
@@ -187,6 +187,27 @@
   }
 }
 
+
+__global__ void k_kernel_map_occ_batch(AprKmapBatch b, OccGrid g, int pad, const unsigned* __restrict__ bm) {
+  const AprKmapOne m = apr_kmap_select(b, blockIdx.x);
+  const int ks = m.ks, K = ks * ks * ks, h = ks / 2;
+  const int64_t total = m.n_out * K;
+  for (int64_t t = (int64_t)m.lblk * blockDim.x + threadIdx.x; t < total; t += (int64_t)m.nblk * blockDim.x) {
+    const int64_t j = t / K;
+    const int o = (int)(t - j * K);
+    const int ox = o % ks - h, oy = (o / ks) % ks - h, oz = o / (ks * ks) - h;
+    const int4 c = m.coords[j];
+    const int x = c.y + ox * m.scale, y = c.z + oy * m.scale, z = c.w + oz * m.scale;
+    int r = -1;
+    if (apr_key_in_range(c.x, x, y, z)) {
+      const int4 cell = make_int4(c.x, x, y, z);
+      const bool maybe = !occ_inside(g, cell, pad) || ((bm[occ_word(g, c.x, x, y, z)] >> ((x - g.minx) & 31)) & 1u);
+      if (maybe) r = apr_table_lookup(m.keys, m.vals, m.mask, apr_pack_key(c.x, x, y, z));
+    }
+    m.nbr[t] = r;
+  }
+}
+
 }
 
 APR_API int apr_kernel_map_occ(const int32_t* out_coords, int64_t n_out, const int32_t* n_out_dev, const uint64_t* in_keys,
@@ -207,6 +228,21 @@
   hipLaunchKernelGGL(k_kernel_map_occ, dim3((unsigned)nblk), dim3(256), 0, (hipStream_t)stream, (const int4*)out_coords, n_out,
                      n_out_dev, (const unsigned long long*)in_keys, in_vals, (uint32_t)(cap - 1), kernel_size, scale, L.g,
                      bitmap_kernel_size / 2, bm, nbr);
+  APR_LAUNCH_CHECK();
+  return APR_OK;
+}
+
+APR_API int apr_kernel_map_occ_batch(const apr_kmap_desc* maps, int32_t n, const int32_t* bbox_host, int32_t bitmap_kernel_size,
+                                     const void* occ_scratch, void* stream) {
+  AprKmapBatch b;
+  if (int rc = apr_internal_kmap_batch_fill(maps, n, &b, "apr_kernel_map_occ_batch")) return rc;
+  APR_CHECK_ARG(bbox_host && occ_scratch, "apr_kernel_map_occ_batch: bad arguments");
+  if (b.blk0[n] == 0) return APR_OK;
+  const OccLayout L = occ_layout(bbox_host, bitmap_kernel_size);
+  APR_CHECK_ARG(L.ok, "apr_kernel_map_occ_batch: empty or oversized bounding box");
+  const unsigned* bm = (const unsigned*)(((uintptr_t)occ_scratch + 255) & ~(uintptr_t)255);
+  hipLaunchKernelGGL(k_kernel_map_occ_batch, dim3(b.blk0[n]), dim3(256), 0, (hipStream_t)stream, b, L.g, bitmap_kernel_size / 2,
+                     bm);
   APR_LAUNCH_CHECK();
   return APR_OK;
 }
diff --git a/apr_amd/ops.py b/apr_amd/ops.py
--- a/apr_amd/ops.py
+++ b/apr_amd/ops.py
@@ -1343,6 +1343,47 @@
     return nbr
 
 
+def set_batched_builds(value):
+    check(_lib_().apr_set_batched_builds(-1 if value is None else int(bool(value))))
+
+
+def kernel_map_batch(items, kernel_size=3, occ=None):
+    descs = (_lib.KmapDesc * len(items))()
+    out = []
+    for d, (out_map, in_map, scale) in zip(descs, items):
+        nbr = torch.empty((out_map.n, kernel_size ** 3), dtype=torch.int32, device=out_map.coords.device)
+        d.out_coords, d.n_out = out_map.coords.data_ptr(), out_map.n
+        d.in_keys, d.in_vals, d.cap = in_map.keys.data_ptr(), in_map.vals.data_ptr(), in_map.cap
+        d.kernel_size, d.scale, d.nbr = int(kernel_size), int(scale), nbr.data_ptr()
+        out.append(nbr)
+    if occ is None:
+        check(_lib_().apr_kernel_map_batch(descs, len(items), stream()))
+    else:
+        scratch, bbox, bks = occ[:3]
+        if any(in_map.n != occ[3] or in_map.coords.data_ptr() != occ[4] for _, in_map, _ in items):
+            raise _lib.AprHipError("kernel_map_batch: the bitmap was not built from every row of the input map")
+        check(_lib_().apr_kernel_map_occ_batch(descs, len(items), (C.c_int32 * 8)(*bbox), int(bks), ptr(scratch), stream()))
+    return out
+
+
+def kernel_map_transpose_batch(items):
+    dev = items[0][0].device
+    pool = torch.empty(sum(n_in * nbr.shape[1] for nbr, n_in in items), dtype=torch.int32, device=dev)
+    fill_bytes(pool, 0xFF)
+    descs = (_lib.KmapTransposeDesc * len(items))()
+    out, pos = [], 0
+    for d, (nbr, n_in) in zip(descs, items):
+        if nbr.dtype != torch.int32 or not nbr.is_contiguous() or nbr.dim() != 2:
+            raise _lib.AprHipError("kernel_map_transpose_batch: nbr must be a contiguous int32 [n_out, K] tensor")
+        K = nbr.shape[1]
+        t = pool[pos:pos + n_in * K].view(n_in, K)
+        pos += n_in * K
+        d.nbr, d.n_out, d.K, d.n_in, d.nbr_t = nbr.data_ptr(), nbr.shape[0], K, n_in, t.data_ptr()
+        out.append(t)
+    check(_lib_().apr_kernel_map_transpose_batch(descs, len(items), stream()))
+    return out
+
+
 def set_ransac_screen(mode):
     check(_lib_().apr_ransac_set_screen(-1 if mode is None else int(bool(mode))))
 
diff --git a/include/apr_hip.h b/include/apr_hip.h
--- a/include/apr_hip.h
+++ b/include/apr_hip.h
@@ -71,6 +71,20 @@
                        const int32_t* in_vals, int64_t cap, int32_t kernel_size, int32_t scale,
                        const int32_t* bbox_host, int32_t bitmap_kernel_size, const void* occ_scratch, int32_t* nbr,
                        void* stream);
+
+typedef struct apr_kmap_desc {
+  const int32_t* out_coords; int64_t n_out;
+  const uint64_t* in_keys; const int32_t* in_vals; int64_t cap;
+  int32_t kernel_size, scale;
+  int32_t* nbr;
+} apr_kmap_desc;
+typedef struct apr_kmap_transpose_desc {
+  const int32_t* nbr; int64_t n_out; int32_t K; int64_t n_in; int32_t* nbr_t;
+} apr_kmap_transpose_desc;
+int apr_kernel_map_batch(const apr_kmap_desc* maps, int32_t n, void* stream);
+int apr_kernel_map_occ_batch(const apr_kmap_desc* maps, int32_t n, const int32_t* bbox_host, int32_t bitmap_kernel_size,
+                             const void* occ_scratch, void* stream);
+int apr_kernel_map_transpose_batch(const apr_kmap_transpose_desc* maps, int32_t n, void* stream);
 
 
 int64_t apr_spconv_packed_size(int32_t K, int32_t cin, int32_t cout);
@@ -185,6 +199,7 @@
 size_t apr_voxel_pyramid_scratch_bytes(int64_t n_points, int32_t nseg);
 int apr_voxel_pyramid(const float* const* frames_host, const int64_t* offsets_host, int32_t nseg, float voxel_size,
                       void* arena, size_t arena_bytes, apr_pyramid* out, void* stream);
+int apr_set_batched_builds(int32_t value);
 
 
 int apr_bn_stats(const float* x, int64_t ld, int64_t n, int32_t c,
```

After: 2709. No clear change (-0.8%).
